# 21cmfast/21cmFAST

Measured on AMD Instinct MI355X. Metric: IonizeBox cells/sec (512^3 HII_DIM, 40 filter radii), higher is better.
Workload: dtype f32; 1 GPU; ComputeIonizedBox single-z, HII_DIM=512, 40 filter steps, G=2 (delta tophat + n_ion exp-MFP), first snapshot, device-resident inputs; hii_dim=512, n_radii=40, filtered_grids=2, parallelism=single GPU, fft=native

## Files before the change

21cmfast_amd/csrc/hip/c21hip.h:

```cpp
#ifndef C21HIP_H
#define C21HIP_H

#include <stddef.h>

#include "ws_slots.h"

#ifdef __cplusplus
extern "C" {
#endif

int c21hip_device_count(void);
int c21hip_current_device(void);
int c21hip_use_device(int device);
int c21hip_is_device_ptr(const void *p);
void *c21hip_ws(int slot, size_t bytes);
__attribute__((visibility("hidden"))) const void *c21_stage_in(int slot, const void *p, size_t bytes, void *stream, int *status);
void *c21hip_ws_peek(int slot, size_t *bytes);
int c21hip_ws_adopt(int slot, void *ptr, size_t bytes);
void *c21hip_raw_alloc(size_t bytes);
void *c21hip_vmm_chunk(size_t phys_bytes, size_t map_bytes, void **va_out);
void c21hip_vmm_chunk_free(void *chunk);
int c21hip_ws_adopt_vmm(int slot, void *chunk, size_t bytes);
void c21hip_raw_free(void *p);
size_t c21hip_free_bytes(void);
// ... 23 lines not shown
float c21hip_event_elapsed_ms(void *start, void *stop);
void c21hip_set_error(const char *fmt, ...);
const char *c21hip_get_error(void);

int c21hip_fft_r2c(float *padded, int nx, int ny, int nz, void *stream);
int c21hip_fft_c2r(float *padded, int nx, int ny, int nz, void *stream);
int c21hip_fft_r2c_batched(float *padded, int nx, int ny, int nz, int n_batch, void *stream);
void c21hip_fft_release(void);
int c21hip_fft_is_native(int nx, int ny, int nz);
int c21hip_pair_sweep_supported(int nx);

size_t c21hip_split_floats(int nx, int ny, int nz);
int c21hip_padded_to_split(const float *padded_c, float *split, int nx, int ny, int nz,
                           void *stream);
int c21hip_split_filter_c2r(const float *split_src, float *split_work, float *real_out,
                            long out_zstride, int nx, int ny, int nz, double box_len,
                            double box_len_z, int filter_type, float R, float R_param, int apply,
                            void *stream);

int c21hip_split_r2c(const float *real_in, long in_zstride, float *split_out, int nx, int ny,
                     int nz, double factor, double lo, double hi, float out_scale, void *stream);
int c21hip_split_filter_xy(const float *split_src, float *split_work, int nx, int ny, int nz,
                           double box_len, double box_len_z, int filter_type, float R,
                           float R_param, int apply, void *stream);
int c21hip_split_filter_xy2(const float *src_a, float *work_a, int filter_a, float R_param_a,
                            const float *src_b, float *work_b, int filter_b, float R_param_b,
                            int nx, int ny, int nz, double box_len, double box_len_z, float R,
                            int apply, int table_slot, int tables_ready, void *stream);
int c21hip_split_filter_shell(const float *src_a, float *work_a, int filter_a, const float *src_b,
                              float *work_b, int filter_b, int n_grids, int nx, int ny, int nz,
                              double box_len, double box_len_z, float R_inner, float R_outer,
                              float R_star, int apply, void *stream);
int c21hip_split_filter_xy2_pair(const float *src_a, float *work_a, float *work_a2, int filter_a,
                                 float R_param_a, const float *src_b, float *work_b,
                                 float *work_b2, int filter_b, float R_param_b, int nx, int ny,
                                 int nz, double box_len, double box_len_z, float R, float R2,
                                 int table_slot, int table_slot2, int phases, void *stream);
int c21hip_split_filter_x_pair1(const float *src, float *work, float *work2, int filter_type, int nx, int ny,
                                int nz, double box_len, double box_len_z, float R, float R2, int phases,
                                void *stream);
int c21hip_split_filter_xy2_pair_eval(const float *src_a, float *work_a, float *work_a2, int filter_a,
                                      const float *src_b, float *work_b, float *work_b2, int filter_b, int nx,
                                      int ny, int nz, double box_len, double box_len_z, float R, float R2,
                                      int phases, void *stream);
int c21hip_split_filter_xy_shared_pair(const float *src, float *work, float *work2,
                                       int filter_type, int nx, int ny, int nz, double box_len,
                                       double box_len_z, float R, float R2, int table_slot,
                                       int table_slot2, int phases, void *stream);
int c21hip_wev_prepare(int filter_a, float R_param_a, int filter_b, float R_param_b, int n_grids,
                       const float *R, int n_R, int nx, int ny, int nz, double box_len,
                       double box_len_z, int pair, int *enabled, void *stream);
void c21hip_wev_release(void);
int c21hip_wev_applicable(int filter_a, int filter_b, int n_grids, int nx, int ny, int nz);
int c21hip_split_filter_xy_single_pair(const float *src, float *work, float *work2, int filter_type,
                                       float R_param, int nx, int ny, int nz, double box_len,
                                       double box_len_z, float R, float R2, int phases, void *stream);
int c21hip_z_ionise_recomb_xe_supported(int nx, int ny, int nz);
int c21hip_split_z_ionise_recomb_xe(const float *delta_work, const float *stars_work, const float *xe_work,
                                    const float *nrec, double rec0, float *g12, unsigned char *first_cross,
                                    double *partials, int nx, int ny, int nz, int r_index,
                                    double rhocrit_omb, double ion_eff, int mass_dep_zeta, double f_limit,
                                    void *stream);
int c21hip_split_z_ionise_recomb_nrec(const float *delta_work, const float *stars_work, const float *nrec_work,
                                      float *g12, unsigned char *first_cross, double *partials, int nx,
                                      int ny, int nz, int r_index, double rhocrit_omb, double ion_eff,
                                      int mass_dep_zeta, double f_limit, void *stream);
int c21hip_z_ionise_recomb_xe_nrec_supported(int nx, int ny, int nz);
int c21hip_split_z_ionise_recomb_xe_nrec(const float *delta_work, const float *stars_work, const float *xe_work,
                                         const float *nrec_work, float *g12, unsigned char *first_cross,
                                         double *partials, int nx, int ny, int nz, int r_index,
                                         double rhocrit_omb, double ion_eff, int mass_dep_zeta, double f_limit,
                                         void *stream);
int c21hip_split_z_ionise_recomb(const float *delta_work, const float *stars_work, const float *nrec,
                                 double rec0, float *g12, unsigned char *first_cross,
                                 double *partials, int nx, int ny, int nz, int r_index,
                                 double rhocrit_omb, double ion_eff, int mass_dep_zeta,
                                 double f_limit, void *stream);
int c21hip_split_z_sfr_gamma12(const float *sfr_work, const unsigned char *first_cross, float *g12,
                               int nx, int ny, int nz, int r_index, double g12_scale, void *stream);
int c21hip_z_ionise_recomb_supported(int nx, int ny, int nz);
int c21hip_z_xe_mask_supported(int nx, int ny, int nz);
int c21hip_split_z_xe_mask(const float *xe_work, const float *nion_dense, const double *mean_dev,
                           unsigned char *first_cross, int nx, int ny, int nz, int r_index,
                           double mean_f_coll, int fix_mean, int mass_dep_zeta, double f_limit,
                           double ion_eff, void *stream);
int c21hip_apply_first_cross_recomb(const unsigned char *first_cross, const float *R_dev,
                                    const float *prev_z_reion, int first_snapshot, double redshift,
                                    float *xH, float *z_reion, float *mfp, size_t ntot, void *stream);
int c21hip_window_tables(int table_slot, int filter_a, float R_param_a, int filter_b,
                         float R_param_b, int nx, int ny, int nz, double box_len,
                         double box_len_z, float R, void *stream);
int c21hip_split_z_c2r_minmax(const float *split_work, float *real_out, long out_zstride, int nx,
                              int ny, int nz, double *partials, double *minmax_out, void *stream);
int c21hip_z_table_band_supported(int nx, int ny, int nz);
int c21hip_split_z_minmax_only(const float *split_work, int nx, int ny, int nz, double *partials,
                               double *minmax_out, void *stream);
int c21hip_split_z_fcoll_table_band(const float *split_work, float *f_pend, const double *band_dev,
                                    const double *thr_prev_dev, unsigned char *first_cross, int r_index,
                                    int r_prev, int nx, int ny, int nz, int mode, double tab_min, double tab_width,
                                    const float *table_dev, double *partials, void *stream);
int c21hip_split_z_fcoll_erfc(const float *split_work, float *nion_dense, int nx, int ny, int nz,
                              double growthf, double sigma_min, double sigma_max, double delta_c,
                              double *partials, double *sum_out, void *stream);
int c21hip_split_z_c2r_stats(const float *split_work, float *real_out, long out_zstride, int nx,
                             int ny, int nz, double min_value, double const_factor,
                             double *partials, double *stats_out, void *stream);
int c21hip_batched_stats(const double *partials, long stride, int nb, int count,
                         double *stats_out, void *stream);
int c21hip_floor_scale_stats(const float *in, long in_zstride, float *out, int nx, int ny, int nz,
                             double min_value, double const_factor, double *partials,
                             double *stats_out, void *stream);
int c21hip_split_z_c2r_div(const float *split_work, float *real_out, long out_zstride, int nx,
                           int ny, int nz, float divisor, void *stream);
int c21hip_split_z_c2r_out(const float *split_work, float *real_out, long out_zstride, int nx,
                           int ny, int nz, float scale, float divisor, int floor_density,
                           void *stream);
int c21hip_split_xblock_log2(int nx);
int c21hip_split_kop(const float *in_split, float *out_split, int nx, int ny, int nz,
                     double box_len, double box_len_z, int axis0, int axis1, void *stream);
int c21hip_split_sepop_xy(const float *split_src, float *split_work, int nx, int ny, int nz,
                          double box_len, double box_len_z, int axis0, int axis1, void *stream);
int c21hip_split_fold(const float *hi_split, float *lo_split, int nx, int ny, int nz, int f,
                      double box_len, double box_len_z, int axis0, int axis1, void *stream);
int c21hip_split_fold_multi(const float *hi_split, float *const lo_split[4], const int ops[4], int n_out, int nx,
                            int ny, int nz, int f, double box_len, double box_len_z, float tophat_R, void *stream);
int c21hip_lpt2_source(const float *const diag[3], const float *const off[3], float *out, size_t n,
                       float norm, void *stream);
int c21hip_copy_filter_split(const float *src_split, float *dst_split, int nx, int ny, int nz,
                             double box_len, double box_len_z, int filter_type, float R,
                             float R_param, int apply, void *stream);
int c21hip_split_z_c2r(const float *split_work, float *real_out, long out_zstride, int nx, int ny,
                       int nz, void *stream);
int c21hip_split_z_ionise_stars(const float *delta_work, const float *stars_work,
                                unsigned char *first_cross, double *partials, double *sum_out,
                                int nx, int ny, int nz, int r_index, double rhocrit_omb,
                                double ion_eff, int mass_dep_zeta, double f_limit, void *stream);
int c21hip_z_ionise_partials(int nx, int ny, int nz);
int c21hip_batched_means(const double *partials, long stride, int n_partials, int first, int step,
                         int count, double ntot, int mass_dep_zeta, double f_limit, double *sums,
                         double *means, void *stream);
int c21hip_split_z_ionise_stars_xe(const float *delta_work, const float *stars_work,
                                   const float *xe_work, unsigned char *first_cross,
                                   double *partials, double *sum_out, int nx, int ny, int nz,
                                   int r_index, double rhocrit_omb, double ion_eff,
                                   int mass_dep_zeta, double f_limit, void *stream);
int c21hip_z_ionise_xe_supported(int nx, int ny, int nz);
int c21hip_z_cross_bits_supported(int nx, int ny, int nz);
int c21hip_split_z_ionise_stars_bits(const float *delta_work, const float *stars_work,
                                     unsigned *cross_plane, double *partials, double *sum_out, int nx,
                                     int ny, int nz, int r_index, double rhocrit_omb, double ion_eff,
                                     int mass_dep_zeta, double f_limit, void *stream);
int c21hip_resolve_crossings(const unsigned *bits, int r_hi, int r_lo, unsigned char *first_cross,
                             size_t nlines, void *stream);
int c21hip_split_filter_xy_shared(const float *src, float *work, int filter_type, int nx, int ny,
                                  int nz, double box_len, double box_len_z, float R, int apply,
                                  int table_slot, void *stream);
int c21hip_bench_pass(int kind, int n, int filter_a, int filter_b, float R, float R_param_b,
                      double box_len, int reps, void *stream, float *ms_out);
int c21hip_reduce_sum(const double *partials, int n, double *out, void *stream);
int c21hip_reduce_op(const double *partials, int n, int op, double *stage, double *out,
                     void *stream);

int c21hip_pack_clip(const float *dense, float *padded, int nx, int ny, int nz, double factor,
                     double lo, double hi, void *stream);
int c21hip_unpack_scale(const float *padded, float *dense, int nx, int ny, int nz, float scale,
                        void *stream);
int c21hip_divide_inplace(float *buf, size_t n, float divisor, void *stream);
int c21hip_divide_inplace_f64(float *buf, size_t n, double divisor, void *stream);
int c21hip_fill(float *buf, size_t n, float value, void *stream);
int c21hip_add_scalar(float *buf, size_t n, float value, void *stream);
int c21hip_widen(const float *in, double *out, size_t n, void *stream);

int c21hip_copy_filter(const float *src_c, float *dst_c, int nx, int ny, int nz, double box_len,
                       double box_len_z, int filter_type, float R, float R_param, int apply,
                       void *stream);
int c21hip_copy_filter_star(const float *src_c, float *dst_c, int nx, int ny, int nz,
                            double box_len, double box_len_z, int filter_type, float R,
                            float R_param, float R_star, int apply, void *stream);

int c21hip_gsl_words_to_deviates(void *buf, size_t n_deviates, const unsigned char *row_kind_dev,
                                 size_t deviates_per_row, void *stream);

int c21hip_cic_scatter(const float *hires_density, const int dens_dim[3], const float *const vel[3],
                       const float *const vel2[3], const int vel_dim[3], double *out,
                       const int out_dim[3], double box_len, double box_len_z, double growth,
                       double init_growth, int lpt2, int *fixed_out, void *stream);
int c21hip_cic_fixed_status(int *bad, void *stream);
int c21hip_cic_last_path(void);
int c21hip_halobox_scatter(const float *src_density, const int dens_dim[3],
                           const float *const vel[3], const float *const vel2[3],
                           const int vel_dim[3], double *out_nion, double *out_sfr,
                           double *out_xray , const int out_dim[3],
                           double box_len, double box_len_z, double growth, double init_growth,
                           int lpt2, const float *tables_dev ,
                           double tab_min, double tab_width, double pref_nion, double pref_sfr,
                           double pref_xray, void *stream);
int c21hip_halobox_turnovers(size_t ntot, int n_chunks, int below_z_heat_max, double redshift,
                             double mturn_a_nofb, double m_turn, double vcb_const, double A_LW,
                             double BETA_LW, double A_VCB, double BETA_VCB, double sigma_vcb,
                             const float *prev_G12, const float *prev_z_reion, const float *J_21_LW,
                             const float *vcb, float *out_a, float *out_m, double *sums_dev,
                             void *stream);
int c21hip_halobox_scatter_mini(const float *src_density, const int dim[3],
                                const float *const vel[3], const float *const vel2[3],
                                const float *mturn_a, const float *mturn_m, double *out_nion,
                                double *out_sfr, double *out_sfr_mini, double *out_xray,
                                double box_len, double box_len_z, double growth, double init_growth,
                                int lpt2, const float *tab_sfrd, const float *tab_nion_a,
                                const float *tab_nion_m, const float *tab_sfrd_m,
                                const float *tab_xray, const double *ranges,
                                const double *prefactors, void *stream);
struct c21cm_halo_consts;
size_t c21hip_halo_deposit_scratch_ints(unsigned long long n_halos, const int out_dim[3]);
int c21hip_halo_props(const struct c21cm_halo_consts *consts, unsigned long long n_halos,
                      const float *masses, const float *coords, const float *star_rng,
                      const float *sfr_rng, const float *xray_rng, const int dim[3],
                      double cell_length, double redshift, int below_z_heat_max, int vcb_flucts,
                      const double lw[7], const float *vcb, const float *J21, const float *z_re,
                      const float *G12, float *out, void *stream);
int c21hip_halo_deposit(const struct c21cm_halo_consts *consts, unsigned long long n_halos,
                        const float *masses, const float *coords, const float *star_rng,
                        const float *sfr_rng, const float *xray_rng, const float *const vel[3],
                        const float *const vel2[3], const int vel_dim[3], const int out_dim[3],
                        double box_len, double box_len_z, double growth, double init_growth, int lpt2,
                        const float *mturn_a, const float *mturn_m, double *out_nion, double *out_sfr,
                        double *out_sfr_mini, double *out_xray, double *out_wsfr, int *scratch,
                        void *stream);
int c21hip_halo_catalog(const struct c21cm_halo_consts *consts, unsigned long long n_halos,
                        const float *masses, const float *coords, const float *star_rng,
                        const float *sfr_rng, const float *xray_rng, const float *const vel[3],
                        const float *const vel2[3], const int vel_dim[3], const int lo_dim[3],
                        double box_len, double box_len_z, double vdf, double vdf2, int lpt2,
                        double box_to_lores, const float *mturn_a, const float *mturn_m,
                        float *const out[9], void *stream);
int c21hip_narrow(const double *in, float *out, float *out_scaled, double scale, size_t n,
                  void *stream);
int c21hip_minmax_dense(const float *a, size_t n, double *partials, double *out2, void *stream);
int c21hip_widen_normalise(const double *in, float *padded, int nx, int ny, int nz, int normalise,
                           double mass_factor, int fixed, void *stream);
int c21hip_scale_pack(const float *dense, float *padded, int nx, int ny, int nz, double factor,
                      void *stream);
int c21hip_gather(const float *src_padded, const int src_dim[3], float *dst, const int lo_dim[3],
                  int dst_padded, float divisor, int clip, void *stream);
int c21hip_velocity_kspace(const float *saved_c, float *grid_c, int nx, int ny, int nz,
                           double box_len, double box_len_z, int axis, double dDdt_over_D,
                           void *stream);

int c21hip_vcb_op(const float *in_c, float *out_c, int nx, int ny, int nz, double box_len,
                  double box_len_z, int axis, const double *h_by_m_dev, void *stream);
int c21hip_vcb_accumulate(const float *src_padded, const int hi_dim[3], float *dst,
                          const int lo_dim[3], int first, int last, float volume, void *stream);
int c21hip_sample_modes(float *cbox, int nx, int ny, int nz, const double *pk_by_m_dev,
                        float volume, unsigned long long seed, const double *deviates_dev,
                        void *stream);
int c21hip_sample_modes_split(float *split, int nx, int ny, int nz, const double *pk_by_m_dev, float volume,
                              unsigned long long seed, const double *deviates_dev, void *stream);
int c21hip_kspace_op(const float *in_c, float *out_c, int nx, int ny, int nz, double box_len,
                     double box_len_z, int axis0, int axis1, void *stream);
int c21hip_pack_density(const float *dense, float *padded, int nx, int ny, int nz, float volume,
                        void *stream);
int c21hip_lpt2_accumulate(float *box, const float *phi_ij_padded, const float *diag_i,
                           const float *diag_j, int nx, int ny, int nz, void *stream);

typedef struct c21hip_ionize_args {
    int nx, ny, nz;
    int r_index;
    int lagrangian;
    int mass_dep_zeta;
    int use_ts_fluct;
    int minimize_memory;
    int first_snapshot;
    int fix_mean;
    double mean_f_coll;
    double f_limit;
    double ion_eff_factor;
    double rhocrit_omb;
    double photoncons_factor;
    double redshift;
    double TK_nofluct, adia_TK_term, T_re;
} c21hip_ionize_args;

#define C21HIP_PARTIALS 4096

int c21hip_clip_minmax(float *delta_fil, int nx, int ny, int nz, double *partials,
                       double *minmax_out, void *stream);
int c21hip_fcoll_eulerian(const float *delta_fil, float *nion_dense, int nx, int ny, int nz,
                          int mode, double growthf, double sigma_min, double sigma_max,
                          double delta_c, double tab_min, double tab_width,
                          const float *table_dev, double *partials, double *sum_out,
                          void *stream);
int c21hip_fcoll_eulerian_zs(const float *delta_fil, long zstride, float *nion_dense, int nx, int ny, int nz,
                             int mode, double growthf, double sigma_min, double sigma_max, double delta_c,
                             double tab_min, double tab_width, const float *table_dev, double *partials,
                             double *sum_out, void *stream);
int c21hip_ionise_stars(const c21hip_ionize_args *a, const float *delta_fil,
                        const float *stars_fil, const float *xe_fil, const float *density,
                        const float *prev_z_reion, const float *kinetic_temp_neutral, float *xH,
                        float *z_reion, float *kinetic_temperature, unsigned char *first_cross,
                        double *partials, double *sum_out, void *stream);
int c21hip_ionise_eulerian(const c21hip_ionize_args *a, const float *nion_dense,
                           const float *xe_fil, const float *density, const float *prev_z_reion,
                           const float *kinetic_temp_neutral, const double *mean_dev, float *xH,
                           float *z_reion, float *kinetic_temperature,
                           unsigned char *first_cross, void *stream);
int c21hip_finish_mean(const double *sum_dev, double ntot, int mass_dep_zeta, double f_limit,
                       double *mean_dev, void *stream);
// ... 247 lines not shown
```

21cmfast_amd/csrc/hip/fft_native.hip:

```cpp
#include <hip/hip_runtime.h>

#include <cmath>
#include <map>
#include <mutex>
#include <vector>

#include "c21hip.h"
#include "fcoll_device.h"
#include "ms_window.h"
#include "c21cm_abi.h"
#include "c21cm_grid.h"

#ifndef C21X_XPAIR_THREADS
#define C21X_XPAIR_THREADS 512
#endif
#ifndef C21X_FUSE512
#define C21X_FUSE512 1
#endif
#ifndef C21X_FUSE1024
#define C21X_FUSE1024 1
#endif
#ifndef C21X_F512_MERGE
#define C21X_F512_MERGE 1
#endif
// ... 301 lines not shown
        const float ksq = __fadd_rn(__fadd_rn(__fmul_rn(kx[i], kx[i]), __fmul_rn(ky[i], ky[i])),
                                    __fmul_rn(kz[i], kz[i]));
        const double k = sqrt((double)ksq);
        x0[i] = (double)(float)(k * (double)pa.R);
        x3[i] = k * pb.mfp.R;
    }
#pragma unroll
    for (int i = 0; i < NE; i++) fast_sincos(x0[i], &sn[i], &cs[i]);
#pragma unroll
    for (int i = 0; i < NE; i++) {
        wa[i] = w_tophat(x0[i], sn[i], cs[i]);
        const double d = x3[i] - x0[i], d3 = d * (1.0 / 3.0);
        const double s3 = sn[i] + d * (cs[i] - 0.5 * d * (sn[i] + d3 * cs[i]));
        const double c3 = cs[i] - d * (sn[i] + 0.5 * d * (cs[i] - d3 * sn[i]));
        wb[i] = w_expmfp(pb.mfp, x3[i], s3, c3);
    }
}

using wtab_t = float;
struct WTableArgs {
    FilterParams pa, pb;
    int dual;
    int nx, ny, nz;
    wtab_t *main_a, *nyq_a, *main_b, *nyq_b;
    MsConsts ms_a, ms_b;
};

template <int NE>
__device__ __forceinline__ void window_batch_ms(const FilterParams &p, const MsConsts &ms,
                                                const float (&kx)[NE], const float (&ky)[NE],
                                                const float (&kz)[NE], double (&w)[NE]) {
    if (p.type != 5) {
        window_batch<NE>(p, kx, ky, kz, w);
        return;
    }
#pragma unroll
    for (int i = 0; i < NE; i++) {
        const float ksq = __fadd_rn(__fadd_rn(__fmul_rn(kx[i], kx[i]), __fmul_rn(ky[i], ky[i])),
                                    __fmul_rn(kz[i], kz[i]));
        w[i] = ms_window(sqrt((double)ksq), ms);
    }
}

template <bool MS>
__global__ void __launch_bounds__(kBlock)
window_table_kernel(WTableArgs t) {
    const int nxh = t.nx / 2 + 1, nyh = t.ny / 2 + 1, H = t.nz / 2, H4 = H / 4;
    const long n4 = (long)nyh * nxh * H4;
    const long id = (long)blockIdx.x * kBlock + threadIdx.x;
    const bool sym = (t.nx == t.ny);
    if (id < n4) {
        const int l4 = (int)(id % H4);
        const long r = id / H4;
        const int i = (int)(r % nxh), j = (int)(r / nxh);
        if (sym && i > j) return;
        const long rT = (long)i * nxh + j;
        float kx[4], ky[4], kz[4];
#pragma unroll
        for (int e = 0; e < 4; e++) {
            kx[e] = k_of(i, t.nx, t.pa.dkx);
            ky[e] = k_of(j, t.ny, t.pa.dky);
            kz[e] = (float)((double)(4 * l4 + e) * t.pa.dkz);
        }
        double wa[4], wb[4];
        if (MS) {
            window_batch_ms<4>(t.pa, t.ms_a, kx, ky, kz, wa);
            if (t.dual) window_batch_ms<4>(t.pb, t.ms_b, kx, ky, kz, wb);
        } else if (t.dual)
            window_batch_dual<4>(t.pa, t.pb, kx, ky, kz, wa, wb);
        else
            window_batch<4>(t.pa, kx, ky, kz, wa);
        for (int rep = 0; rep < ((sym && i != j) ? 2 : 1); rep++) {
            const long rr = rep ? rT : r;
            *reinterpret_cast<float4 *>(t.main_a + rr * H + 4 * l4) =
                make_float4((float)wa[0], (float)wa[1], (float)wa[2], (float)wa[3]);
            if (t.dual)
                *reinterpret_cast<float4 *>(t.main_b + rr * H + 4 * l4) =
                    make_float4((float)wb[0], (float)wb[1], (float)wb[2], (float)wb[3]);
        }
    } else if (id - n4 < (long)nxh * nyh) {
        const long q = id - n4;
        const int i = (int)(q / nyh), j = (int)(q % nyh);
        if (sym && i > j) return;
        float kx[1] = {k_of(i, t.nx, t.pa.dkx)}, ky[1] = {k_of(j, t.ny, t.pa.dky)};
        float kz[1] = {(float)((double)(t.nz / 2) * t.pa.dkz)};
        double wa[1], wb[1];
        if (MS) {
            window_batch_ms<1>(t.pa, t.ms_a, kx, ky, kz, wa);
            if (t.dual) window_batch_ms<1>(t.pb, t.ms_b, kx, ky, kz, wb);
        } else if (t.dual)
            window_batch_dual<1>(t.pa, t.pb, kx, ky, kz, wa, wb);
        else
            window_batch<1>(t.pa, kx, ky, kz, wa);
        t.nyq_a[q] = (wtab_t)wa[0];
        if (t.dual) t.nyq_b[q] = (wtab_t)wb[0];
        if (sym && i != j) {
            t.nyq_a[(long)j * nyh + i] = (wtab_t)wa[0];
            if (t.dual) t.nyq_b[(long)j * nyh + i] = (wtab_t)wb[0];
        }
    }
}

struct WNodeArgs {
    float *out;
    int n_nodes, n_tabs;
    int first_type;
    const ExpMfpConsts *mfp;
};
__device__ __forceinline__ double wnode_value(int type, const ExpMfpConsts &c, double x) {
    x = fabs(x);
    double sn, cs;
    sincos(x, &sn, &cs);
    return type == 0 ? w_tophat(x, sn, cs) : w_expmfp(c, x, sn, cs);
}
__global__ void __launch_bounds__(kBlock)
window_nodes_kernel(WNodeArgs a) {
    const int id = blockIdx.x * kBlock + threadIdx.x;
    if (id >= a.n_nodes * a.n_tabs) return;
    const int tab = id / a.n_nodes, n = id - tab * a.n_nodes;
    const int type = (tab == 0) ? a.first_type : 3;
    ExpMfpConsts c{};
    if (type == 3) c = a.mfp[a.first_type == 3 ? tab : tab - 1];
    const double h = 0.25, s = h / 16., x = h * (double)n;
    const double c1[4] = {4. / 5., -1. / 5., 4. / 105., -1. / 280.};
    const double c2[4] = {8. / 5., -1. / 5., 8. / 315., -1. / 560.};
    const double f0 = wnode_value(type, c, x);
    double d1 = 0., d2 = -205. / 72. * f0;
#pragma unroll
    for (int k = 1; k <= 4; k++) {
        const double fp = wnode_value(type, c, x + k * s), fm = wnode_value(type, c, x - k * s);
        d1 += c1[k - 1] * (fp - fm);
        d2 += c2[k - 1] * (fp + fm);
    }
    float *o = a.out + 3 * (size_t)id;
    o[0] = (float)f0;
    o[1] = (float)(d1 / s * h);
    o[2] = (float)(d2 / (s * s) * h * h * 0.5);
}

struct LineGeo {
    const float2 *src[2];
    float2 *dst[2];
    float2 *dst2[2];
    long line_stride, line_bstride;
    long outer_stride, outer_bstride;
    int line_lb, outer_lb;
    long col_stride;
    int n_outer;
    int n_ctiles;
    int pair_outer;
    int filter_axis;
};

struct LinePassArgs {
    LineGeo g0, g1;
    int n_geo;
    int g1_strided;
    int n_grids;
    int n_y, n_z;
    float out_scale;
    const wtab_t *wt_main[2];
    const wtab_t *wt_nyq[2];
    int dual;
    const wtab_t *wt2_main[2];
    const wtab_t *wt2_nyq[2];
    FilterParams fp;
    int op_ex, op_ey, op_ez, op_imag;
    double op_sign, op_dkx, op_dky, op_dkz;
    const float *wev_src[3];
    int wev_n_tabs, wev_n_nodes;
    int wev_tab[2][2];
    int wev_type[2];
    float wev_R[2];
    float wev_mfp[2][4];
    double wev_dkx, wev_dky, wev_dkz;
    int item_order;
};

static inline int geo_items(const LineGeo &g) {
    return (g.pair_outer ? (g.n_outer / 2 + 1) : g.n_outer) * g.n_ctiles;
}

template <int N>
__device__ __forceinline__ int mirror_row(int row_a) {
    return row_a == 0 ? N / 2 : N - row_a;
}

template <int N, int FMODE = 0>
struct LineThreads {
    static constexpr int value =
        ((FMODE == 5 || FMODE == 7 || FMODE == 9) && N == 512) ? C21X_XPAIR_THREADS
                                                 : ((N >= 128 && N != 192) ? 512 : 256);
};

struct LineItemSecond {
    float2 *dst0b, *dst1b;
    const wtab_t *wt0b, *wt1b;
};
struct LineItemNone {};
template <bool PAIR>
struct LineItemT : std::conditional_t<PAIR, LineItemSecond, LineItemNone> {
    const float2 *src0, *src1;
    float2 *dst0, *dst1;
    long line_stride, line_bstride, outer_stride, outer_bstride, col_stride;
    int line_lb, outer_lb;
    int n_outer, filter_axis;
    int og, ct, npair;
    const wtab_t *wt0, *wt1;
};

template <int N, int SIGN, int FMODE>
__global__ void __launch_bounds__((LineThreads<N, FMODE>::value), (LineThreads<N, FMODE>::value / 256))
line_pass_kernel(LinePassArgs a, const float2 *__restrict__ tw_global) {
    static_assert(N >= 64, "tile loader needs N >= 64");
    constexpr int kBlock = LineThreads<N, FMODE>::value;
    constexpr int TZ = line_tile_cols(N);
    constexpr int CPAIR = TZ / 2;
    constexpr int RSTEP = kBlock / CPAIR;
    constexpr bool WEVAL = (FMODE >= 6 && FMODE <= 9);
    constexpr bool WDIRECT = (FMODE == 8 || FMODE == 9);
    constexpr bool WIN = (FMODE == 3 || (FMODE == 5 && !C21X_XPAIR_NOWIN) || WEVAL);
    constexpr bool PAIR = (FMODE == 5 || FMODE == 7 || FMODE == 9);
    constexpr int NR = PAIR ? 2 : 1;
    using LineItem = LineItemT<PAIR>;
    extern __shared__ float4 lds_raw[];
    float2 *tile = reinterpret_cast<float2 *>(lds_raw);
    float2 *tw = tile + NR * N * TZ;
    float2 *tw_half = tw + N;
    float *wnodes = reinterpret_cast<float *>(tw_half + (N >= 1024 ? N / 2 : 0));
    for (int t = threadIdx.x; t < N; t += kBlock) tw[t] = tw_global[t];
    if (N >= 1024)
        for (int t = threadIdx.x; t < N / 2; t += kBlock) tw_half[t] = tw_global[2 * t];
    if constexpr (WEVAL) {
        const int per = 3 * a.wev_n_nodes;
        for (int t = threadIdx.x; t < per; t += kBlock) {
            wnodes[t] = a.wev_src[0][t];
            if (a.wev_n_tabs > 1) wnodes[per + t] = a.wev_src[1][t];
            if (a.wev_n_tabs > 2) wnodes[2 * per + t] = a.wev_src[2][t];
        }
    }
#ifndef C21X_NO_TW_BARRIER
#define C21X_NO_TW_BARRIER 0
#endif
    if (!C21X_NO_TW_BARRIER || WEVAL) __syncthreads();

    constexpr int NP = (N / 2) / RSTEP;
    const int r0 = threadIdx.x / CPAIR, c4 = threadIdx.x % CPAIR;
    constexpr bool F512_ = C21X_FUSE512 && N == 512 && kBlock == 512 && (FMODE == 0 || WEVAL);
    float2 twd1[F512_ ? 8 : 1], twd2[F512_ ? 8 : 1];
    if constexpr (F512_) {
        __syncthreads();
        auto fill = [&](float2(&t)[8], int ps) {
            t[0] = make_float2(1.f, 0.f);
            t[1] = tw[ps];
            t[2] = tw[2 * ps];
            t[4] = tw[4 * ps];
            t[3] = cmul(t[1], t[2]);
            t[5] = cmul(t[1], t[4]);
            t[6] = cmul(t[2], t[4]);
            t[7] = cmul(t[3], t[4]);
            if (SIGN > 0)
#pragma unroll
                for (int j = 1; j < 8; j++) t[j].y = -t[j].y;
        };
        fill(twd1, r0);
        if (C21X_F512_HOIST2) fill(twd2, r0 & ~7);
    }
    const int n_work0 = (a.g0.pair_outer ? (a.g0.n_outer / 2 + 1) : a.g0.n_outer) * a.g0.n_ctiles;
    const int n_work1 =
        (a.n_geo > 1) ? (a.g1.pair_outer ? (a.g1.n_outer / 2 + 1) : a.g1.n_outer) * a.g1.n_ctiles : 0;
    const int n_work = n_work0 + (a.g1_strided ? 0 : n_work1);

    auto decode = [&](int w) {
        LineItem it;
        const bool s = w >= n_work0;
        int ww = s ? w - n_work0 : w;
        if (WIN && !s && ww < (n_work0 & ~15) && a.item_order == 0) {
            const int r = ww & 15;
            ww = (ww & ~15) + 2 * (r & 7) + (r >> 3);
        }
        it.src0 = s ? a.g1.src[0] : a.g0.src[0];
        it.src1 = s ? a.g1.src[1] : a.g0.src[1];
        it.dst0 = s ? a.g1.dst[0] : a.g0.dst[0];
        it.dst1 = s ? a.g1.dst[1] : a.g0.dst[1];
        it.line_stride = s ? a.g1.line_stride : a.g0.line_stride;
        it.line_bstride = s ? a.g1.line_bstride : a.g0.line_bstride;
        it.line_lb = s ? a.g1.line_lb : a.g0.line_lb;
        it.outer_stride = s ? a.g1.outer_stride : a.g0.outer_stride;
        it.outer_bstride = s ? a.g1.outer_bstride : a.g0.outer_bstride;
        it.outer_lb = s ? a.g1.outer_lb : a.g0.outer_lb;
        it.col_stride = s ? a.g1.col_stride : a.g0.col_stride;
        it.n_outer = s ? a.g1.n_outer : a.g0.n_outer;
        it.filter_axis = s ? a.g1.filter_axis : a.g0.filter_axis;
        it.wt0 = (it.filter_axis == 1) ? a.wt_nyq[0] : a.wt_main[0];
        it.wt1 = (it.filter_axis == 1) ? a.wt_nyq[1] : a.wt_main[1];
        if constexpr (PAIR) {
            it.dst0b = s ? a.g1.dst2[0] : a.g0.dst2[0];
            it.dst1b = s ? a.g1.dst2[1] : a.g0.dst2[1];
            it.wt0b = (it.filter_axis == 1) ? a.wt2_nyq[0] : a.wt2_main[0];
            it.wt1b = (it.filter_axis == 1) ? a.wt2_nyq[1] : a.wt2_main[1];
        }
        const int nct = s ? a.g1.n_ctiles : a.g0.n_ctiles;
        const int po = s ? a.g1.pair_outer : a.g0.pair_outer;
        it.og = ww / nct;
        it.ct = ww - it.og * nct;
        if (a.item_order == 3 || a.item_order == -1) {
            if (!s && (int)gridDim.x % nct == 0)
                it.ct = (it.ct + w / (int)gridDim.x) % nct;
        } else if (a.item_order != 0 && !s) {
            const int nog = n_work0 / nct;
            if (FMODE != 0) {
                it.ct = ww / nog;
                it.og = ww - it.ct * nog;
            } else {
                const int k = a.item_order < nct ? a.item_order : nct;
                const int head = k * nog;
                if (ww < head) {
                    const int c = ww / nog;
                    it.ct = nct - 1 - c;
                    it.og = ww - c * nog;
                } else {
                    const int v = ww - head, m = nct - k;
                    it.og = v / m;
                    it.ct = v - it.og * m;
                }
            }
        }
        it.npair = (po && it.og != 0 && 2 * it.og != it.n_outer) ? 2 : 1;
        return it;
    };
    auto member_grid = [](const LineItem &it, int m) { return it.npair == 2 ? (m >> 1) : m; };
    auto member_base = [](const LineItem &it, int m) {
        const int mi = it.npair == 2 ? (m & 1) : 0;
        const int outer = mi == 0 ? it.og : it.n_outer - it.og;
        return (long)(outer >> it.outer_lb) * it.outer_bstride +
               (long)(outer & ((1 << it.outer_lb) - 1)) * it.outer_stride +
               (long)it.ct * TZ * it.col_stride;
    };
    auto row_off = [](const LineItem &it, int r) {
        return (unsigned)(r >> it.line_lb) * (unsigned)it.line_bstride +
               (unsigned)(r & ((1 << it.line_lb) - 1)) * (unsigned)it.line_stride;
    };

    constexpr bool TWO_SETS = (N < 1024) && (!PAIR || C21X_XPAIR_TWO_SETS);
    float4 reg_a[2 * NP], reg_b[2 * NP];
    constexpr bool F512 = C21X_FUSE512 && N == 512 && kBlock == 512 && (FMODE == 0 || WEVAL);
    constexpr bool F1024 = C21X_FUSE1024 && N == 1024 && kBlock == 512 && (FMODE == 0 || FMODE == 3 || WEVAL);
    constexpr bool FUSED = F512 || F1024;
    constexpr int NW = FUSED ? 2 * NP : NP;
    constexpr bool WPRE = (N >= 512) && !FUSED;
    float2 wpre[NR][WPRE ? NP : 1], wcur[NR][NW], wpre_half[NR], wcur_half[NR];
    auto w_reload = [&](const LineItem &it, int m) {
        const int mi = it.npair == 2 ? (m & 1) : 0;
        return m == 0 || (a.dual && mi == 0);
    };
    struct KAbs {
        float kh, kl;
    };
    auto k_abs = [](float kx, float ky, float kz) -> KAbs {
        const float ksq = __fadd_rn(__fadd_rn(__fmul_rn(kx, kx), __fmul_rn(ky, ky)), __fmul_rn(kz, kz));
        KAbs k;
        k.kh = __builtin_amdgcn_sqrtf(ksq);
        const float r = __fmaf_rn(-k.kh, k.kh, ksq);
        k.kl = (k.kh > 0.f) ? __fmul_rn(r, __fmul_rn(0.5f, __builtin_amdgcn_rcpf(k.kh))) : 0.f;
        return k;
    };
    auto weval_direct = [&](float x0, float d, int type, int rr) -> float {
        const float n = rintf(x0 * 0.6366197723675814f);
        float r = __fmaf_rn(-n, 1.5707963705062866f, x0);
        r = __fmaf_rn(-n, -4.371138828673793e-08f, r);
        const float z = r * r;
        const float s = fmaf(fmaf(fmaf(-1.9515295891e-4f, z, 8.3321608736e-3f), z, -1.6666654611e-1f) * z, r, r);
        const float c = fmaf(fmaf(fmaf(2.443315711809948e-5f, z, -1.388731625493765e-3f), z,
                                  4.166664568298827e-2f) * z, z, fmaf(-0.5f, z, 1.0f));
        const int q = (int)n & 3;
        const float ss = (q & 1) ? c : s, cc = (q & 1) ? s : c;
        float sn = (q & 2) ? -ss : ss, cs = ((q + 1) & 2) ? -cc : cc;
        const float inv = __builtin_amdgcn_rcpf(x0);
        if (type == 0) return 3.f * (sn - x0 * cs) * (inv * inv) * inv;
        const float s0 = sn, c0 = cs;
        sn = fmaf(d, c0, s0);
        cs = fmaf(-d, s0, c0);
        const float ra = rr ? a.wev_mfp[1][0] : a.wev_mfp[0][0], r2 = rr ? a.wev_mfp[1][1] : a.wev_mfp[0][1],
                    r3 = rr ? a.wev_mfp[1][2] : a.wev_mfp[0][2], et = rr ? a.wev_mfp[1][3] : a.wev_mfp[0][3];
        const float xx = fmaf(2.f * x0, d, x0 * x0);
        float f = fmaf(xx, r2, fmaf(2.f, ra, 1.f)) * ra * cs;
        f = fmaf(fmaf(xx, r2 - r3, ra + 1.f) * sn, __builtin_amdgcn_rcpf(x0 + d), f);
        f = fmaf(f, et, -2.f * r2);
        const float dd = fmaf(xx, r2, 1.f);
        return f * (-3.f * ra * __builtin_amdgcn_rcpf(dd * dd));
    };
    auto weval_one = [&](const KAbs &k, float R, int type, const float *tab, int rr) -> float {
        const float ph = __fmul_rn(k.kh, R);
        const float e = __fmaf_rn(k.kl, R, __fmaf_rn(k.kh, R, -ph));
        const float x0 = __fadd_rn(ph, e);
        if (type == 1) return ((double)x0 * 0.413566994 > 1) ? 0.f : 1.f;
        const float u = x0 * 4.0f;
        if constexpr (WDIRECT)
            if (u >= (float)(a.wev_n_nodes - 2))
                return weval_direct(x0, __fadd_rn(__fsub_rn(ph, x0), e), type, rr);
        const int n = WDIRECT ? (int)u : min((int)u, a.wev_n_nodes - 2);
        const float t = u - (float)n;
        const float *nd = tab + 3 * n;
        const float f0 = nd[0], g0 = nd[1], q0 = nd[2], f1 = nd[3], g1 = nd[4], q1 = nd[5];
        const float A = ((f1 - f0) - g0) - q0, B = (g1 - g0) - 2.f * q0, C = q1 - q0;
        const float a3 = 10.f * A - 4.f * B + C, a4 = -15.f * A + 7.f * B - 2.f * C,
                    a5 = 6.f * A - 3.f * B + C;
        float p = fmaf(fmaf(fmaf(fmaf(fmaf(a5, t, a4), t, a3), t, q0), t, g0), t, f0);
        if (type == 3) {
            const float d = __fadd_rn(__fsub_rn(ph, x0), e);
            const float dp = fmaf(fmaf(fmaf(fmaf(5.f * a5, t, 4.f * a4), t, 3.f * a3), t, 2.f * q0), t, g0);
            p = fmaf(d * 4.0f, dp, p);
        }
        return p;
    };
    float wev_kx[WEVAL ? NW : 1];
    float wev_kx_half = 0.f;
    if constexpr (WEVAL) {
#pragma unroll
        for (int u = 0; u < NW; u++) {
            const int row = r0 + RSTEP * u;
            wev_kx[u] = (float)((double)(FUSED ? min(row, N - row) : row) * a.wev_dkx);
        }
        wev_kx_half = (float)((double)(N / 2) * a.wev_dkx);
    }
    auto eval_windows = [&](const LineItem &it, int m) {
        const int wsel = (a.dual && member_grid(it, m)) ? 1 : 0;
        const int type = wsel ? a.wev_type[1] : a.wev_type[0];
        const int per = 3 * a.wev_n_nodes;
        float kyc[2], kzc[2];
        if (it.filter_axis == 0) {
            kyc[0] = kyc[1] = (float)((double)it.og * a.wev_dky);
            const int l0 = it.ct * TZ + 2 * c4;
            kzc[0] = (float)((double)l0 * a.wev_dkz);
            kzc[1] = (float)((double)(l0 + 1) * a.wev_dkz);
        } else {
            const int c0 = it.ct * TZ + 2 * c4;
            kyc[0] = (float)((double)min(c0, a.n_y - c0) * a.wev_dky);
            kyc[1] = (float)((double)min(c0 + 1, a.n_y - c0 - 1) * a.wev_dky);
            kzc[0] = kzc[1] = (float)((double)(a.n_z / 2) * a.wev_dkz);
        }
        const float *tab0 = wnodes + max(wsel ? a.wev_tab[0][1] : a.wev_tab[0][0], 0) * per;
        const float *tab1 = wnodes + max(wsel ? a.wev_tab[1][1] : a.wev_tab[1][0], 0) * per;
#pragma unroll
        for (int u = 0; u < NW; u++) {
            if (FUSED && u >= NP && !(u == NP && r0 == 0)) continue;
            const KAbs k0 = k_abs(wev_kx[WEVAL ? u : 0], kyc[0], kzc[0]);
            const KAbs k1 = k_abs(wev_kx[WEVAL ? u : 0], kyc[1], kzc[1]);
#pragma unroll
            for (int rr = 0; rr < NR; rr++) {
                const float R = rr ? a.wev_R[1] : a.wev_R[0];
                const float *tab = rr ? tab1 : tab0;
                (WPRE ? wpre[rr][WPRE ? u : 0] : wcur[rr][u]) =
                    make_float2(weval_one(k0, R, type, tab, rr), weval_one(k1, R, type, tab, rr));
            }
        }
        if (!FUSED && r0 == 0) {
            const KAbs k0 = k_abs(wev_kx_half, kyc[0], kzc[0]), k1 = k_abs(wev_kx_half, kyc[1], kzc[1]);
#pragma unroll
            for (int rr = 0; rr < NR; rr++) {
                const float R = rr ? a.wev_R[1] : a.wev_R[0];
                const float *tab = rr ? tab1 : tab0;
                (WPRE ? wpre_half[rr] : wcur_half[rr]) =
                    make_float2(weval_one(k0, R, type, tab, rr), weval_one(k1, R, type, tab, rr));
            }
        }
        if constexpr (FUSED) {
            float2 *const exch = tile;
            __syncthreads();
#pragma unroll
            for (int rr = 0; rr < NR; rr++)
#pragma unroll
                for (int u = 0; u < NP; u++) exch[((int)threadIdx.x * NP + u) * NR + rr] = wcur[rr][u];
            __syncthreads();
            const int src = (((RSTEP - r0) & (RSTEP - 1)) * CPAIR + c4) * NP;
#pragma unroll
            for (int rr = 0; rr < NR; rr++)
#pragma unroll
                for (int u = NP; u < NW; u++)
                    if (!(u == NP && r0 == 0))
                        wcur[rr][u] = exch[(src + (NW - (r0 == 0 ? 0 : 1) - u)) * NR + rr];
            __syncthreads();
        }
    };
    auto issue_wloads = [&](const LineItem &it, int m) {
        if constexpr (WEVAL) {
            eval_windows(it, m);
            return;
        }
        const bool second = a.dual && member_grid(it, m);
#pragma unroll
        for (int rr = 0; rr < NR; rr++) {
            const wtab_t *t = second ? it.wt1 : it.wt0;
            if constexpr (PAIR)
                if (rr) t = second ? it.wt1b : it.wt0b;
            if (it.filter_axis == 0) {
                const unsigned wc = (unsigned)(a.n_z / 2);
                const wtab_t *b = t + (long)it.og * (N / 2 + 1) * wc + (it.ct * TZ + 2 * c4);
                if constexpr (FUSED) {
#pragma unroll
                    for (int u = 0; u < NW; u++) {
                        const int row = r0 + RSTEP * u;
                        wcur[rr][u] = *reinterpret_cast<const float2 *>(b + (unsigned)min(row, N - row) * wc);
                    }
                    continue;
                }
#pragma unroll
                for (int u = 0; u < NP; u++)
                    (WPRE ? wpre[rr][WPRE ? u : 0] : wcur[rr][u]) =
                        *reinterpret_cast<const float2 *>(b + (unsigned)(r0 + RSTEP * u) * wc);
                (WPRE ? wpre_half[rr] : wcur_half[rr]) =
                    *reinterpret_cast<const float2 *>(b + (unsigned)(N / 2) * wc);
            } else {
                const int c0 = it.ct * TZ + 2 * c4;
                const unsigned nyh = (unsigned)(a.n_y / 2 + 1);
                const unsigned j0 = (unsigned)min(c0, a.n_y - c0),
                               j1 = (unsigned)min(c0 + 1, a.n_y - c0 - 1);
                if constexpr (FUSED) {
#pragma unroll
                    for (int u = 0; u < NW; u++) {
                        const int row = r0 + RSTEP * u;
                        const wtab_t *r = t + (unsigned)min(row, N - row) * nyh;
                        wcur[rr][u] = make_float2(r[j0], r[j1]);
                    }
                    continue;
                }
#pragma unroll
                for (int u = 0; u < NP; u++) {
                    const wtab_t *r = t + (unsigned)(r0 + RSTEP * u) * nyh;
                    (WPRE ? wpre[rr][WPRE ? u : 0] : wcur[rr][u]) = make_float2(r[j0], r[j1]);
                }
                {
                    const wtab_t *r = t + (unsigned)(N / 2) * nyh;
                    (WPRE ? wpre_half[rr] : wcur_half[rr]) = make_float2(r[j0], r[j1]);
                }
            }
        }
    };
    auto issue_loads = [&](float4(&reg)[2 * NP], const LineItem &it, int m) {
        const float2 *lo = (member_grid(it, m) ? it.src1 : it.src0) + member_base(it, m);
        const float2 *hi = lo + (long)((N / 2) >> it.line_lb) * it.line_bstride;
#pragma unroll
        for (int u = 0; u < 2 * NP; u++) {
            if constexpr (FUSED) {
                const int row = r0 + RSTEP * u;
                const unsigned roff = row_off(it, row < N / 2 ? row : row - N / 2);
                reg[u] = *reinterpret_cast<const float4 *>((row < N / 2 ? lo : hi) + (roff + 2u * c4));
                continue;
            }
            const int row_a = r0 + RSTEP * (u >> 1);
            const unsigned roff = (u & 1) ? (row_a == 0 ? 0u : row_off(it, N / 2 - row_a))
                                          : row_off(it, row_a);
            const float2 *p = (u & 1) ? hi : lo;
            reg[u] = *reinterpret_cast<const float4 *>(p + (roff + 2u * c4));
        }
    };

    struct TileRef {
        LineItem it;
        int m, work, valid;
    };
    auto next_tile = [&](const TileRef &t) {
        TileRef n = t;
        if (!t.valid) return n;
        if (t.m + 1 < t.it.npair * a.n_grids) {
            n.m = t.m + 1;
        } else {
            n.work = t.work + (int)gridDim.x;
            n.valid = n.work < n_work;
            if (n.valid) {
                n.m = 0;
                n.it = decode(n.work);
            }
        }
        return n;
    };

    bool first = true;
    auto process = [&](float4(&reg)[2 * NP], const TileRef &cur, const TileRef &nxt,
                       const TileRef &refill) {
        const LineItem &it = cur.it;
        const int m = cur.m;
        const long st_half = (long)((N / 2) >> it.line_lb) * it.line_bstride;
        if (!first) __syncthreads();
        first = false;
        if (WIN && WPRE && w_reload(it, m)) {
#pragma unroll
            for (int rr = 0; rr < NR; rr++) {
#pragma unroll
                for (int u = 0; u < NP; u++) wcur[rr][u] = wpre[rr][WPRE ? u : 0];
                wcur_half[rr] = wpre_half[rr];
            }
        }
        double op_c0 = 1., op_c1 = 1.;
        if (FMODE == 4) {
            const int c0 = it.ct * TZ + 2 * c4;
            int kyi0, kyi1, kzi0, kzi1;
            if (it.filter_axis == 0) {
                const int mi = it.npair == 2 ? (m & 1) : 0;
                const int outer = mi == 0 ? it.og : it.n_outer - it.og;
                kyi0 = kyi1 = (outer <= a.n_y / 2) ? outer : outer - a.n_y;
                kzi0 = c0;
                kzi1 = c0 + 1;
            } else {
                kyi0 = (c0 <= a.n_y / 2) ? c0 : c0 - a.n_y;
                kyi1 = (c0 + 1 <= a.n_y / 2) ? c0 + 1 : c0 + 1 - a.n_y;
                kzi0 = kzi1 = a.n_z / 2;
            }
            const double ky0 = (double)kyi0 * a.op_dky, ky1 = (double)kyi1 * a.op_dky;
            const double kz0 = (double)kzi0 * a.op_dkz, kz1 = (double)kzi1 * a.op_dkz;
            const double fy0 = a.op_ey == 0 ? 1. : (a.op_ey == 1 ? ky0 : ky0 * ky0);
            const double fy1 = a.op_ey == 0 ? 1. : (a.op_ey == 1 ? ky1 : ky1 * ky1);
            const double fz0 = a.op_ez == 0 ? 1. : (a.op_ez == 1 ? kz0 : kz0 * kz0);
            const double fz1 = a.op_ez == 0 ? 1. : (a.op_ez == 1 ? kz1 : kz1 * kz1);
// ... 85 lines not shown
                }
                continue;
            }
            if (!(PAIR && C21X_XPAIR_SKIP_FFT)) {
                Dft<8, SIGN>::run(c0);
                Dft<8, SIGN>::run(c1);
            }
#pragma unroll
            for (int j = 0; j < 8; j++) {
                float2 o0 = c0[j], o1 = c1[j];
                if (j > 0 && !(PAIR && C21X_XPAIR_SKIP_FFT)) {
                    o0 = cmul(o0, twd1[F512_ ? j : 0]);
                    o1 = cmul(o1, twd1[F512_ ? j : 0]);
                }
                *reinterpret_cast<float4 *>(tile_r + (8 * r0 + j) * TZ + 2 * c4) =
                    make_float4(o0.x, o0.y, o1.x, o1.y);
            }
            continue;
        }
#pragma unroll
        for (int u = 0; u < 2 * NP; u++) {
            const int row_a = r0 + RSTEP * (u >> 1);
            const int row = (u & 1) ? mirror_row<N>(row_a) : row_a;
            const bool half = (u & 1) && row_a == 0;
            float4 v = reg[u];
            if (FMODE == 4) {
                const int kxi = (row <= N / 2) ? row : row - N;
                const double kx = (double)kxi * a.op_dkx;
                const double fr = a.op_ex == 0 ? 1. : (a.op_ex == 1 ? kx : kx * kx);
                const double f0 = fr * op_c0, f1 = fr * op_c1;
                if (a.op_imag) {
                    const float4 t = v;
                    v.x = (float)(-(double)t.y * f0);
                    v.y = (float)((double)t.x * f0);
                    v.z = (float)(-(double)t.w * f1);
                    v.w = (float)((double)t.z * f1);
                } else {
                    v.x = (float)((double)v.x * f0);
                    v.y = (float)((double)v.y * f0);
                    v.z = (float)((double)v.z * f1);
                    v.w = (float)((double)v.w * f1);
                }
            }
            if (WIN) {
                const float2 wv = half ? wcur_half[rr] : wcur[rr][u >> 1];
                v.x = __fmul_rn(v.x, wv.x);
                v.y = __fmul_rn(v.y, wv.x);
                v.z = __fmul_rn(v.z, wv.y);
                v.w = __fmul_rn(v.w, wv.y);
            }
            *reinterpret_cast<float4 *>(tile_r + row * TZ + 2 * c4) = v;
        }
      }
        __syncthreads();
        if (WIN && !WEVAL && w_reload(nxt.it, nxt.m)) issue_wloads(nxt.it, nxt.m);
        issue_loads(reg, refill.it, refill.m);
        if (WEVAL && !FUSED && w_reload(nxt.it, nxt.m)) issue_wloads(nxt.it, nxt.m);

        if constexpr (F1024) {
            const int obase = (r0 & 7) + 64 * (r0 >> 3);
            float2 s0[2][8], s1[2][8];
#pragma unroll
            for (int h = 0; h < 2; h++)
#pragma unroll
                for (int k = 0; k < 8; k++) {
                    const float4 t = *reinterpret_cast<const float4 *>(tile + (h * (N / 2) + r0 + RSTEP * k) * TZ + 2 * c4);
                    s0[h][k] = make_float2(t.x, t.y);
                    s1[h][k] = make_float2(t.z, t.w);
                }
            __syncthreads();
            float2 w2[8];
            {
                const int ps = r0 & ~7;
                w2[1] = tw_half[ps];
                w2[2] = tw_half[2 * ps];
                w2[4] = tw_half[4 * ps];
                w2[3] = cmul(w2[1], w2[2]);
                w2[5] = cmul(w2[1], w2[4]);
                w2[6] = cmul(w2[2], w2[4]);
                w2[7] = cmul(w2[3], w2[4]);
                if (SIGN > 0)
#pragma unroll
                    for (int j = 1; j < 8; j++) w2[j].y = -w2[j].y;
            }
#pragma unroll
            for (int h = 0; h < 2; h++) {
                Dft<8, SIGN>::run(s0[h]);
                Dft<8, SIGN>::run(s1[h]);
#pragma unroll
                for (int j = 0; j < 8; j++) {
                    float2 o0 = s0[h][j], o1 = s1[h][j];
                    if (j > 0) {
                        o0 = cmul(o0, w2[j]);
                        o1 = cmul(o1, w2[j]);
                    }
                    *reinterpret_cast<float4 *>(tile + (h * (N / 2) + obase + 8 * j) * TZ + 2 * c4) =
                        make_float4(o0.x, o0.y, o1.x, o1.y);
                }
            }
            __syncthreads();
        }
        if constexpr (F512 && !(PAIR && C21X_XPAIR_SKIP_FFT)) {
            constexpr int GRP = C21X_F512_MERGE ? NR : 1;
            const int obase = (r0 & 7) + 64 * (r0 >> 3);
#pragma unroll
            for (int g = 0; g < NR; g += GRP) {
                float2 s0[GRP][8], s1[GRP][8];
#pragma unroll
                for (int rr = 0; rr < GRP; rr++)
#pragma unroll
                    for (int k = 0; k < 8; k++) {
                        const float4 t = *reinterpret_cast<const float4 *>(tile + (g + rr) * N * TZ +
                                                                           (r0 + RSTEP * k) * TZ + 2 * c4);
                        s0[rr][k] = make_float2(t.x, t.y);
                        s1[rr][k] = make_float2(t.z, t.w);
                    }
                __syncthreads();
                float2 w2[8];
                if (!C21X_F512_HOIST2) {
                    const int ps = r0 & ~7;
                    w2[1] = tw[ps];
                    w2[2] = tw[2 * ps];
                    w2[4] = tw[4 * ps];
                    w2[3] = cmul(w2[1], w2[2]);
                    w2[5] = cmul(w2[1], w2[4]);
                    w2[6] = cmul(w2[2], w2[4]);
                    w2[7] = cmul(w2[3], w2[4]);
                    if (SIGN > 0)
#pragma unroll
                        for (int j = 1; j < 8; j++) w2[j].y = -w2[j].y;
                }
#pragma unroll
                for (int rr = 0; rr < GRP; rr++) {
                    Dft<8, SIGN>::run(s0[rr]);
                    Dft<8, SIGN>::run(s1[rr]);
#pragma unroll
                    for (int j = 0; j < 8; j++) {
                        float2 o0 = s0[rr][j], o1 = s1[rr][j];
                        if (j > 0) {
                            const float2 w = C21X_F512_HOIST2 ? twd2[F512_ ? j : 0] : w2[j];
                            o0 = cmul(o0, w);
                            o1 = cmul(o1, w);
                        }
                        *reinterpret_cast<float4 *>(tile + (g + rr) * N * TZ + (obase + 8 * j) * TZ + 2 * c4) =
                            make_float4(o0.x, o0.y, o1.x, o1.y);
                    }
                }
                __syncthreads();
            }
        }
#pragma unroll
      for (int rr = 0; rr < NR; rr++) {
        float2 *const tile_r = tile + rr * N * TZ;
        float2 *st_lo = member_grid(it, m) ? it.dst1 : it.dst0;
        if constexpr (PAIR)
            if (rr) st_lo = member_grid(it, m) ? it.dst1b : it.dst0b;
        st_lo += member_base(it, m);
        if constexpr (F1024) {
#pragma unroll
            for (int h = 0; h < 2; h++) {
                float2 c0[8], c1[8];
#pragma unroll
                for (int k = 0; k < 8; k++) {
                    const float4 t = *reinterpret_cast<const float4 *>(tile_r + (h * (N / 2) + r0 + RSTEP * k) * TZ + 2 * c4);
                    c0[k] = make_float2(t.x, t.y);
                    c1[k] = make_float2(t.z, t.w);
                }
                Dft<8, SIGN>::run(c0);
                Dft<8, SIGN>::run(c1);
#pragma unroll
                for (int j = 0; j < 8; j++) {
                    float4 v = make_float4(c0[j].x, c0[j].y, c1[j].x, c1[j].y);
                    if (a.out_scale != 1.0f) {
                        v.x *= a.out_scale;
                        v.y *= a.out_scale;
                        v.z *= a.out_scale;
                        v.w *= a.out_scale;
                    }
                    const int row = 2 * (r0 + RSTEP * j) + h;
                    const unsigned roff = row_off(it, row < N / 2 ? row : row - N / 2);
                    float2 *p = st_lo + (row < N / 2 ? 0 : st_half);
                    *reinterpret_cast<float4 *>(p + (roff + 2u * c4)) = v;
                }
            }
            continue;
        }
        if constexpr (F512) {
            if constexpr (PAIR && C21X_XPAIR_SKIP_FFT == 3) continue;
            float2 c0[8], c1[8];
#pragma unroll
            for (int k = 0; k < 8; k++) {
                const float4 t = *reinterpret_cast<const float4 *>(tile_r + (r0 + RSTEP * k) * TZ + 2 * c4);
                c0[k] = make_float2(t.x, t.y);
                c1[k] = make_float2(t.z, t.w);
            }
            if (!(PAIR && C21X_XPAIR_SKIP_FFT)) {
                Dft<8, SIGN>::run(c0);
                Dft<8, SIGN>::run(c1);
            }
#pragma unroll
            for (int j = 0; j < 8; j++) {
                float4 v = make_float4(c0[j].x, c0[j].y, c1[j].x, c1[j].y);
                if (a.out_scale != 1.0f) {
                    v.x *= a.out_scale;
                    v.y *= a.out_scale;
                    v.z *= a.out_scale;
                    v.w *= a.out_scale;
                }
                const int row = r0 + RSTEP * j;
                const unsigned roff = row_off(it, row < N / 2 ? row : row - N / 2);
                float2 *p = st_lo + (row < N / 2 ? 0 : st_half);
                *reinterpret_cast<float4 *>(p + (roff + 2u * c4)) = v;
            }
            continue;
        }
        if (!(PAIR && C21X_XPAIR_SKIP_FFT)) line_fft<N, TZ, SIGN, kBlock>(tile_r, tw, tw_half);
        if (PAIR && C21X_XPAIR_SKIP_FFT == 2 && rr == 1) continue;
#pragma unroll
        for (int u = 0; u < 2 * NP; u++) {
            const int row_a = r0 + RSTEP * (u >> 1);
            const int row = (u & 1) ? mirror_row<N>(row_a) : row_a;
            float4 v = *reinterpret_cast<const float4 *>(tile_r + fft_out_row<N>(row) * TZ + 2 * c4);
            if (a.out_scale != 1.0f) {
                v.x *= a.out_scale;
                v.y *= a.out_scale;
                v.z *= a.out_scale;
                v.w *= a.out_scale;
            }
            const unsigned roff = (u & 1) ? (row_a == 0 ? 0u : row_off(it, N / 2 - row_a))
                                          : row_off(it, row_a);
            float2 *p = st_lo + ((u & 1) ? st_half : 0);
            *reinterpret_cast<float4 *>(p + (roff + 2u * c4)) = v;
        }
      }
        if (WEVAL && FUSED && w_reload(nxt.it, nxt.m)) issue_wloads(nxt.it, nxt.m);
    };

    if ((int)blockIdx.x < n_work) {
        TileRef ta;
        ta.work = blockIdx.x;
        ta.valid = 1;
        ta.m = 0;
        ta.it = decode(ta.work);
        if (WIN && !WEVAL) issue_wloads(ta.it, 0);
        issue_loads(reg_a, ta.it, 0);
        if (WEVAL) issue_wloads(ta.it, 0);
        TileRef tb = next_tile(ta);
        if (!TWO_SETS) {
            process(reg_a, ta, tb, tb);
            while (tb.valid) {
                ta = tb;
                tb = next_tile(ta);
                process(reg_a, ta, tb, tb);
            }
            goto main_done;
        }
        issue_loads(reg_b, tb.it, tb.m);
        TileRef tc = next_tile(tb);
        process(reg_a, ta, tb, tc);
        while (tb.valid) {
            const TileRef td = next_tile(tc);
            process(reg_b, tb, tc, td);
            if (!tc.valid) break;
            const TileRef te = next_tile(td);
            process(reg_a, tc, td, te);
            tb = td;
            tc = te;
        }
    }
main_done:
    if (!(a.n_geo > 1 && a.g1_strided)) return;
    for (int w = (int)(gridDim.x - 1 - blockIdx.x); w < n_work1; w += (int)gridDim.x) {
        const unsigned ls = (unsigned)a.g1.line_bstride, cs = (unsigned)a.g1.col_stride;
        const int nct = a.g1.n_ctiles;
        const int og = w / nct, ct = w - og * nct;
        const long base = (long)og * a.g1.outer_bstride + (long)ct * TZ * a.g1.col_stride;
        for (int g = 0; g < a.n_grids; g++) {
            const float2 *src = (g ? a.g1.src[1] : a.g1.src[0]) + base;
            float2 *dst = (g ? a.g1.dst[1] : a.g1.dst[0]) + base;
            __syncthreads();
#pragma unroll
            for (int u = 0; u < 2 * NP; u++) {
                const int row_a = r0 + RSTEP * (u >> 1);
                const int row = (u & 1) ? mirror_row<N>(row_a) : row_a;
                const float2 e0 = src[(unsigned)row * ls + (unsigned)(2 * c4) * cs];
                const float2 e1 = src[(unsigned)row * ls + (unsigned)(2 * c4 + 1) * cs];
                *reinterpret_cast<float4 *>(tile + row * TZ + 2 * c4) =
                    make_float4(e0.x, e0.y, e1.x, e1.y);
            }
            __syncthreads();
            line_fft<N, TZ, SIGN, kBlock>(tile, tw, tw_half);
#pragma unroll
            for (int u = 0; u < 2 * NP; u++) {
                const int row_a = r0 + RSTEP * (u >> 1);
                const int row = (u & 1) ? mirror_row<N>(row_a) : row_a;
                float4 v = *reinterpret_cast<const float4 *>(tile + fft_out_row<N>(row) * TZ + 2 * c4);
                if (a.out_scale != 1.0f) {
                    v.x *= a.out_scale;
                    v.y *= a.out_scale;
                    v.z *= a.out_scale;
                    v.w *= a.out_scale;
                }
                dst[(unsigned)row * ls + (unsigned)(2 * c4) * cs] = make_float2(v.x, v.y);
                dst[(unsigned)row * ls + (unsigned)(2 * c4 + 1) * cs] = make_float2(v.z, v.w);
            }
        }
// ... 304 lines not shown
    const float dmin = (float)(-1. + 1e-7);
    double acc = 0.;
#pragma unroll
    for (int u = 0; u < NOUT; u++) {
        const int f = threadIdx.x + kBlock * u;
        const int li = f / H, j = f % H;
        const float2 st = tile[j * ZROW + li];
        const float s0 = fmaxf(st.x, 0.f), s1 = fmaxf(st.y, 0.f);
        acc += (double)s0;
        acc += (double)s1;
        const double D0 = a.rhocrit_omb * (1. + (double)fmaxf(dens[u].x, dmin));
        const double D1 = a.rhocrit_omb * (1. + (double)fmaxf(dens[u].y, dmin));
        const bool i0 = floor_ionises || ((double)s0 * a.ion_eff > D0);
        const bool i1 = floor_ionises || ((double)s1 * a.ion_eff > D1);
        uchar2 m = old[u];
        const bool n0 = i0 && m.x == 0, n1 = i1 && m.y == 0;
        if (n0) m.x = (unsigned char)a.r_index;
        if (n1) m.y = (unsigned char)a.r_index;
        if (n0 || n1 || a.store_all)
            reinterpret_cast<uchar2 *>(a.first_cross + logical_line(l0 + li, a.ny, a.lb) * NZ)[j] = m;
    }
    __shared__ double red[kBlock / 64];
#pragma unroll
    for (int off = 32; off > 0; off >>= 1) acc += __shfl_down(acc, off, 64);
    if ((threadIdx.x & 63) == 0) red[threadIdx.x >> 6] = acc;
    __syncthreads();
    if (threadIdx.x == 0) {
        double sum = 0.;
#pragma unroll
        for (int w = 0; w < kBlock / 64; w++) sum += red[w];
        a.partials[blockIdx.x] = sum;
    }
}

__global__ void __launch_bounds__(kBlock)
padded_to_split_kernel(const float2 *__restrict__ padded, float2 *__restrict__ main,
                       float2 *__restrict__ nyq, long nlines, int H, int ny, int lb) {
    const long total = nlines * (long)(H + 1);
    for (long i = (long)blockIdx.x * kBlock + threadIdx.x; i < total;
         i += (long)gridDim.x * kBlock) {
        const long line = i / (H + 1);
        const int k = (int)(i - line * (H + 1));
        const float2 v = padded[i];
        if (k < H) {
            const long x = line / ny, y = line - x * ny;
            const long m = lb ? (((x >> lb) * ny + y) << lb) + (x & ((1 << lb) - 1)) : line;
            main[m * H + k] = v;
        } else {
            nyq[line] = v;
        }
    }
}

struct Twiddles {
    float2 *dev = nullptr;
};
std::map<int, Twiddles> g_tw;
std::mutex g_tw_mutex;

const float2 *twiddles(int n) {
    std::lock_guard<std::mutex> lock(g_tw_mutex);
    auto it = g_tw.find(n);
    if (it != g_tw.end()) return it->second.dev;
    std::vector<float2> host(n);
    for (int t = 0; t < n; t++) {
        const double ang = -2.0 * M_PI * (double)t / (double)n;
        host[t] = make_float2((float)cos(ang), (float)sin(ang));
    }
    Twiddles tw;
    if (hipMalloc(&tw.dev, sizeof(float2) * n) != hipSuccess) return nullptr;
    if (hipMemcpy(tw.dev, host.data(), sizeof(float2) * n, hipMemcpyHostToDevice) != hipSuccess)
        return nullptr;
    g_tw[n] = tw;
    return tw.dev;
}

bool pow2(int n) { return n > 0 && (n & (n - 1)) == 0; }

void geo_ptrs(LineGeo &g, int grid, const float2 *src, float2 *dst) {
    g.src[grid] = src;
    g.dst[grid] = dst;
}
void geo_axes(LineGeo &g, int line_lb, long line_stride, long line_bstride, int outer_lb,
              long outer_stride, long outer_bstride) {
    g.line_lb = line_lb;
    g.line_stride = line_stride;
    g.line_bstride = line_bstride;
    g.outer_lb = outer_lb;
    g.outer_stride = outer_stride;
    g.outer_bstride = outer_bstride;
}
LineGeo geo_x_main(int ny, int H, int tz, int lb) {
    LineGeo g{};
    const long xb = 1L << lb;
    geo_axes(g, lb, H, (long)ny * xb * H, 0, 0, xb * H);
    g.col_stride = 1;
    g.n_outer = ny;
    g.n_ctiles = H / tz;
    g.pair_outer = 1;
    g.filter_axis = 0;
    return g;
}
LineGeo geo_x_nyq(int ny, int tz) {
    LineGeo g{};
    geo_axes(g, 0, 0, ny, 0, 0, 0);
    g.col_stride = 1;
    g.n_outer = 1;
    g.n_ctiles = ny / tz;
    g.pair_outer = 0;
    g.filter_axis = 1;
    return g;
}
LineGeo geo_y_main(int nx, int ny, int H, int tz, int lb) {
    LineGeo g{};
    const long xb = 1L << lb;
    geo_axes(g, 0, 0, xb * H, lb, H, (long)ny * xb * H);
    g.col_stride = 1;
    g.n_outer = nx;
    g.n_ctiles = H / tz;
    return g;
}
LineGeo geo_y_nyq(int nx, int ny, int tz) {
    LineGeo g{};
    geo_axes(g, 0, 0, 1, 0, 0, 0);
    g.col_stride = ny;
    g.n_outer = 1;
    g.n_ctiles = nx / tz;
    return g;
}

struct KTimeRec {
    int kind;
    hipEvent_t e0, e1;
};
std::vector<KTimeRec> g_ktime;
int g_ktime_on = 0;
struct KTimeScope {
    KTimeRec r{-1, nullptr, nullptr};
    hipStream_t stream;
    KTimeScope(int kind, hipStream_t s) : stream(s) {
        if (!g_ktime_on) return;
        if (hipEventCreate(&r.e0) != hipSuccess || hipEventCreate(&r.e1) != hipSuccess) return;
        r.kind = kind;
        (void)hipEventRecord(r.e0, stream);
    }
    ~KTimeScope() {
        if (r.kind < 0) return;
        (void)hipEventRecord(r.e1, stream);
        g_ktime.push_back(r);
    }
};
constexpr int ktime_kind(int sign, int fmode) {
    return sign < 0 ? 9 : (fmode == 0 ? 1 : fmode == 3 ? 0 : fmode == 5 ? 6 : (fmode == 6 || fmode == 8) ? 7
                                                              : (fmode == 7 || fmode == 9) ? 8 : 10);
}

#ifndef C21X_XORDER_DEFAULT
#define C21X_XORDER_DEFAULT 3
#endif
template <int N, int SIGN, int FMODE>
int launch_line_pass_mode(const LinePassArgs &a, hipStream_t stream) {
    const float2 *tw = twiddles(N);
    if (!tw) {
        c21hip_set_error("native FFT: twiddle table allocation failed");
        return C21CM_MEMORY_ALLOC_ERROR;
    }
    const size_t lds = sizeof(float2) * ((size_t)((FMODE == 5 || FMODE == 7 || FMODE == 9) ? 2 : 1) * N *
                                             line_tile_cols(N) + N + (N >= 1024 ? N / 2 : 0)) +
                       ((FMODE >= 6 && FMODE <= 9) ? sizeof(float) * 3 * (size_t)a.wev_n_nodes * a.wev_n_tabs : 0);
    if (lds > 160 * 1024) {
        c21hip_set_error("native FFT: %zu bytes of LDS for a %d-point line pass (mode %d)", lds, N, FMODE);
        return C21CM_VALUE_ERROR;
    }
    const int n_work = geo_items(a.g0) + (a.n_geo > 1 ? geo_items(a.g1) : 0);
    int per_cu = (int)((160 * 1024) / lds) > 0 ? (int)((160 * 1024) / lds) : 1;
    const int by_waves = (LineThreads<N, FMODE>::value >= 512 && N > 256) ? 1 : 2;
    if (per_cu > by_waves) per_cu = by_waves;
    int nblocks = 256 * per_cu;
    if (nblocks > n_work) nblocks = n_work;
    static size_t attr_lds = 0;
    if (lds > attr_lds) {
        (void)hipFuncSetAttribute((const void *)line_pass_kernel<N, SIGN, FMODE>,
                                  hipFuncAttributeMaxDynamicSharedMemorySize, (int)lds);
        attr_lds = lds;
    }
    LinePassArgs ao = a;
    {
        static int xo = -99, yo = -99;
        if (xo == -99) {
            const char *ex = getenv("C21CM_XORDER"), *ey = getenv("C21CM_YORDER");
            xo = ex ? atoi(ex) : C21X_XORDER_DEFAULT;
            yo = ey ? atoi(ey) : -1;
        }
        ao.item_order = (FMODE == 0) ? yo : xo;
    }
    KTimeScope kt(ktime_kind(SIGN, FMODE), stream);
    hipLaunchKernelGGL((line_pass_kernel<N, SIGN, FMODE>), dim3((unsigned)nblocks),
                       dim3(LineThreads<N, FMODE>::value), lds, stream, ao, tw);
    LAUNCH_CHECK();
    return 0;
}

template <int N, int SIGN>
int launch_line_pass(const LinePassArgs &a, int fmode, hipStream_t stream) {
    if (SIGN > 0 && fmode == 3) return launch_line_pass_mode<N, +1, 3>(a, stream);
    if (SIGN > 0 && fmode == 4) return launch_line_pass_mode<N, +1, 4>(a, stream);
    if constexpr (N <= 512)
        if (SIGN > 0 && fmode == 5) return launch_line_pass_mode<N, +1, 5>(a, stream);
    if constexpr (N >= 128 && (N & (N - 1)) == 0) {
        if (SIGN > 0 && fmode == 6) return launch_line_pass_mode<N, +1, 6>(a, stream);
        if (SIGN > 0 && fmode == 8) return launch_line_pass_mode<N, +1, 8>(a, stream);
        if constexpr (N <= 512) {
            if (SIGN > 0 && fmode == 7) return launch_line_pass_mode<N, +1, 7>(a, stream);
            if (SIGN > 0 && fmode == 9) return launch_line_pass_mode<N, +1, 9>(a, stream);
        }
    }
    if (fmode >= 6 && fmode <= 9) {
        c21hip_set_error("native FFT: evaluated windows are not built for %d-point lines", N);
        return C21CM_VALUE_ERROR;
    }
    return launch_line_pass_mode<N, SIGN, 0>(a, stream);
}

template <int SIGN>
int dispatch_line_pass(int n, const LinePassArgs &a, int fmode, hipStream_t stream) {
    switch (n) {
        case 64: return launch_line_pass<64, SIGN>(a, fmode, stream);
        case 128: return launch_line_pass<128, SIGN>(a, fmode, stream);
        case 192: return launch_line_pass<192, SIGN>(a, fmode, stream);
        case 256: return launch_line_pass<256, SIGN>(a, fmode, stream);
        case 384: return launch_line_pass<384, SIGN>(a, fmode, stream);
        case 512: return launch_line_pass<512, SIGN>(a, fmode, stream);
        case 768: return launch_line_pass<768, SIGN>(a, fmode, stream);
        case 1024: return launch_line_pass<1024, SIGN>(a, fmode, stream);
        case 1536: return launch_line_pass<1536, SIGN>(a, fmode, stream);
        default:
            c21hip_set_error("native FFT: unsupported line length %d", n);
            return C21CM_VALUE_ERROR;
    }
}

template <int NZ, int EPI = 0>
int launch_z_c2r(const ZPassArgs &a, long nlines, hipStream_t stream) {
    constexpr int H = NZ / 2;
    const float2 *twH = twiddles(H);
    const float2 *twN = twiddles(NZ);
    if (!twH || !twN) return C21CM_MEMORY_ALLOC_ERROR;
    const size_t lds = sizeof(float2) * ((size_t)H * (LZ_PLAIN + 1) + H + H / 2 + 1);
    static bool attr_done = false;
    if (!attr_done) {
        (void)hipFuncSetAttribute((const void *)z_c2r_kernel<NZ, EPI>,
                                  hipFuncAttributeMaxDynamicSharedMemorySize, (int)lds);
        attr_done = true;
    }
    hipLaunchKernelGGL((z_c2r_kernel<NZ, EPI>), dim3((unsigned)(nlines / LZ_PLAIN)), dim3(kBlock),
                       lds, stream, a, twH, twN);
    LAUNCH_CHECK();
    return 0;
}

constexpr int ZW_LINES = 16;
constexpr int zw_lines(int P) { return kBlock / P; }

template <int A, bool TS, int P = 16, bool RC = false, bool CB = false>
__global__ void
#if C21X_ZW_OCC
__launch_bounds__(kBlock, (A == 16 && !TS) ? C21X_ZW_OCC : 1)
#else
__launch_bounds__((A == 16 && P == 16) ? C21X_ZW_BLOCK : kBlock, (TS && RC && A == 16 && P == 16) ? C21X_ZW_TSRC_OCC : 1)
#endif
zw_ionise_kernel(ZFusedArgs a, const float2 *__restrict__ twH_global,
                 const float2 *__restrict__ twN_global) {
    constexpr int ZBLK = (A == 16 && P == 16) ? C21X_ZW_BLOCK : kBlock;
    constexpr int H = P * A, NZ = 2 * H, ZWL = ZBLK / P;
    constexpr int LINE_LDS = A * (P + 1) + 4;
    static_assert(LINE_LDS % 2 == 0, "16-byte aligned line regions (mask rows)");
    __shared__ __attribute__((aligned(16))) float2 lines[ZWL * LINE_LDS];
    __shared__ float2 twH[H], twN[H];
    __shared__ double red[ZBLK / 64];
    for (int t = threadIdx.x; t < H; t += ZBLK) {
        twH[t] = twH_global[t];
        twN[t] = twN_global[t];
    }
    const int lane = threadIdx.x & 63, wave = threadIdx.x >> 6;
    const int g = lane / P, b = lane % P;
    const int lw = wave * (64 / P) + g;
    const unsigned blk = a.reverse ? gridDim.x - 1 - blockIdx.x : blockIdx.x;
    const long line = (long)blk * ZWL + lw;
    float2 *L = lines + lw * LINE_LDS;
    const float2 *dm = a.d_main + line * H, *sm = a.s_main + line * H;
    constexpr bool EARLY = (A == 16) && !C21X_ZW_LATE;
    static_assert(!CB || (A == 16 && P == 16 && !TS && !RC), "crossing bits: the two-grid kernel on 512-point lines");
    float2 xd[A], xs[A];
#pragma unroll
    for (int q = 0; q < A; q++) xd[q] = dm[P * q + b];
    if (EARLY) {
#pragma unroll
        for (int q = 0; q < A; q++) xs[q] = sm[P * q + b];
    }
    const long lline = logical_line(line, a.ny, a.lb);
    const float dh = a.d_nyq[lline].x, sh = a.s_nyq[lline].x;
    unsigned char *mrow = nullptr;
    if constexpr (!CB) mrow = a.first_cross + lline * NZ;
    constexpr bool MASK16 = !CB && EARLY && (C21X_ZW_MASK16 || (TS && RC && C21X_ZW_TSRC_LEAN));
    constexpr int MV = MASK16 ? A / 8 : 1;
    uint4 mreg[MV];
    uchar2 old[(EARLY && !MASK16) ? A : 1];
    if constexpr (MASK16) {
#pragma unroll
        for (int v = 0; v < MV; v++) mreg[v] = reinterpret_cast<const uint4 *>(mrow)[b * MV + v];
    } else if (EARLY && !CB) {
#pragma unroll
        for (int q = 0; q < A; q++)
            old[q] = reinterpret_cast<const uchar2 *>(mrow)[(b + P * (q / P)) + A * (q % P)];
    }
    constexpr bool STASH = TS && RC && A == 16 && P == 16 && C21X_ZW_TSRC_LEAN;
    constexpr int NRH = (RC && A == 16 && !STASH) ? A / 2 : 1;
    float2 nr_lo[NRH], nr_hi[NRH];
    __shared__ __attribute__((aligned(16))) float nstash[STASH ? ZWL * NZ : 4];
    uint4 nreg[STASH ? NZ / (4 * P) : 1];
    if constexpr (STASH) {
#pragma unroll
        for (int v = 0; v < NZ / (4 * P); v++) nreg[v] = make_uint4(0u, 0u, 0u, 0u);
        if (a.nrec) {
#pragma unroll
            for (int v = 0; v < NZ / (4 * P); v++)
                nreg[v] = reinterpret_cast<const uint4 *>(a.nrec + lline * NZ)[v * P + b];
        }
    } else if constexpr (RC && A == 16) {
        if (a.nrec) {
#pragma unroll
            for (int q = 0; q < NRH; q++)
                nr_lo[q] = reinterpret_cast<const float2 *>(a.nrec + lline * NZ)[(b + P * (q / P)) + A * (q % P)];
        }
    }
    __syncthreads();
    if constexpr (STASH) {
        if (a.n_main) {
            float2 xn[A];
            const float2 *nm = a.n_main + line * H;
#pragma unroll
            for (int q = 0; q < A; q++) xn[q] = nm[P * q + b];
            wave_c2r<A, P>(xn, a.n_nyq[lline].x, L, twH, twN, b);
#pragma unroll
            for (int q = 0; q < A; q++) {
                const int j = (b + P * (q / P)) + A * (q % P);
                reinterpret_cast<float2 *>(nstash + lw * NZ)[j] =
                    make_float2(fmaxf(xn[q].x, 0.f), fmaxf(xn[q].y, 0.f));
            }
            wave_fence();
        }
    }
    wave_c2r<A, P>(xd, dh, L, twH, twN, b);
    if constexpr (STASH) {
        if (a.nrec) {
#pragma unroll
            for (int v = 0; v < NZ / (4 * P); v++)
                reinterpret_cast<uint4 *>(nstash + lw * NZ)[v * P + b] = nreg[v];
        }
    }
    if (!EARLY) {
#pragma unroll
        for (int q = 0; q < A; q++) xs[q] = sm[P * q + b];
    }
    wave_fence();
    wave_c2r<A, P>(xs, sh, L, twH, twN, b);
    static_assert(!(TS && RC) || A == 16, "x_e + recombinations: 16 points per lane only (registers)");
    float2 xx[TS ? A : 1];
    if constexpr (TS) {
        const float2 *xm = a.x_main + line * H;
// ... 1204 lines not shown
        const dim3 tgrid((unsigned)((n_threads + kBlock - 1) / kBlock));
        if (ms)
            hipLaunchKernelGGL(window_table_kernel<true>, tgrid, dim3(kBlock), 0, stream, t);
        else
            hipLaunchKernelGGL(window_table_kernel<false>, tgrid, dim3(kBlock), 0, stream, t);
        LAUNCH_CHECK();
    }
    w.main[0] = t.main_a;
    w.nyq[0] = t.nyq_a;
    w.main[1] = t.main_b;
    w.nyq[1] = t.nyq_b;
    w.dual = t.dual;
    return 0;
}

struct WevSet {
    bool active = false;
    int filter[2] = {-1, -1};
    float R_param[2] = {0.f, 0.f};
    int nx = 0, ny = 0, nz = 0;
    double box_len = 0, box_len_z = 0;
    std::vector<float> R;
    float *nodes = nullptr;
    int n_nodes = 0, n_tabs = 0;
    bool covers = true;
    int first_type = 0;
    int table(int w, int r) const {
        const int t = filter[w];
        if (t == 1) return -1;
        if (t == 0) return 0;
        int base = (first_type == 0) ? 1 : 0;
        if (w == 1 && filter[0] == 3) base += (int)R.size();
        return base + r;
    }
    int find(float radius) const {
        for (size_t i = 0; i < R.size(); i++)
            if (R[i] == radius) return (int)i;
        return -1;
    }
};
WevSet g_wev;

static bool wev_type_ok(int t) { return t == 0 || t == 1 || t == 3; }
static size_t wev_lds(int n, bool pair, int n_tabs, int n_nodes) {
    return sizeof(float2) * ((size_t)(pair ? 2 : 1) * n * TZ + n + (n >= 1024 ? n / 2 : 0)) +
           sizeof(float) * 3 * (size_t)n_nodes * n_tabs;
}
static bool wev_use(LinePassArgs &a, int n_grids, const int filter_type[2], const float R_param[2],
                    float R, float R2, bool pair, int nx, int ny, int nz, double box_len,
                    double box_len_z) {
    const WevSet &w = g_wev;
    if (!w.active || w.nx != nx || w.ny != ny || w.nz != nz || w.box_len != box_len ||
        w.box_len_z != box_len_z)
        return false;
    int win0 = 0;
    auto matches = [&](int g, int win) {
        return filter_type[g] == w.filter[win] && (filter_type[g] != 3 || R_param[g] == w.R_param[win]);
    };
    if (n_grids == 2) {
        if (!matches(0, 0) || !matches(1, 1)) return false;
    } else if (!matches(0, 0)) {
        if (!matches(0, 1)) return false;
        win0 = 1;
    }
    const int ra = w.find(R), rb = pair ? w.find(R2) : ra;
    if (ra < 0 || rb < 0) return false;
    int ids[4], n_ids = 0;
    auto slot = [&](int id) {
        if (id < 0) return -1;
        for (int i = 0; i < n_ids; i++)
            if (ids[i] == id) return i;
        ids[n_ids] = id;
        return n_ids++;
    };
    const int rr[2] = {ra, rb};
    for (int m = 0; m < 2; m++)
        for (int win = 0; win < 2; win++)
            a.wev_tab[m][win] =
                (win < n_grids && (m == 0 || pair)) ? slot(w.table(win == 0 ? win0 : win, rr[m])) : -1;
    if (n_ids > 3) return false;
    if (wev_lds(nx, pair, n_ids, w.n_nodes) > 160 * 1024) return false;
    for (int i = 0; i < 3; i++)
        a.wev_src[i] = w.nodes + 3 * (size_t)w.n_nodes * (i < n_ids ? ids[i] : ids[0 < n_ids ? 0 : 0]);
    a.wev_n_tabs = n_ids > 0 ? n_ids : 1;
    if (n_ids == 0) a.wev_src[0] = a.wev_src[1] = a.wev_src[2] = w.nodes;
    a.wev_n_nodes = w.n_nodes;
    a.wev_type[0] = filter_type[0];
    a.wev_type[1] = n_grids == 2 ? filter_type[1] : filter_type[0];
    a.wev_R[0] = R;
    a.wev_R[1] = pair ? R2 : R;
    for (int m = 0; m < 2; m++) {
        const int win = (filter_type[0] == 3) ? 0 : ((n_grids == 2 && filter_type[1] == 3) ? 1 : -1);
        if (win < 0) break;
        const float Rm = m ? a.wev_R[1] : a.wev_R[0];
        const double ratio = (double)R_param[win] / (double)Rm;
        a.wev_mfp[m][0] = (float)ratio;
        a.wev_mfp[m][1] = (float)(ratio * ratio);
        a.wev_mfp[m][2] = (float)(ratio * ratio * ratio);
        a.wev_mfp[m][3] = (float)exp((double)(-Rm / R_param[win]));
    }
    a.wev_dkx = 2.0 * M_PI / box_len;
    a.wev_dky = 2.0 * M_PI / box_len;
    a.wev_dkz = 2.0 * M_PI / box_len_z;
    a.dual = (n_grids == 2 && (filter_type[0] != filter_type[1] ||
                               (filter_type[0] >= 3 && R_param[0] != R_param[1])))
                 ? 1 : 0;
    return true;
}

static int check_filter_request(int n_grids, int nx, int ny, int nz, const int filter_type[2],
                                int apply) {
    if (!c21hip_native_fft_supported(nx, ny, nz)) {
        c21hip_set_error("native FFT does not support %dx%dx%d", nx, ny, nz);
        return C21CM_VALUE_ERROR;
    }
    for (int g = 0; g < n_grids; g++)
        if (apply && (filter_type[g] < 0 || filter_type[g] > 5)) {
            c21hip_set_error("filter type %d is not implemented on the device", filter_type[g]);
            return C21CM_VALUE_ERROR;
        }
    return 0;
}

static int filter_xy(const float *const split_src[2], float *const split_work[2], int n_grids,
                     int nx, int ny, int nz, double box_len, double box_len_z,
                     const int filter_type[2], float R, const float R_param[2], int apply,
                     void *stream_, int phases = 7, int table_slot = 0, float R_star = 0.f) {
    int st = check_filter_request(n_grids, nx, ny, nz, filter_type, apply);
    if (st) return st;
    hipStream_t stream = (hipStream_t)stream_;
    const int H = nz / 2;
    const long nlines = (long)nx * ny;
    LinePassArgs a{};
    fill_filter(a.fp, apply ? filter_type[0] : -1, R, R_param[0], box_len, box_len_z);
    a.n_y = ny;
    a.n_z = nz;
    a.out_scale = 1.0f;
    int fmode = apply ? 3 : 0;
    if (fmode == 3 && filter_type[0] != 5 && wev_use(a, n_grids, filter_type, R_param, R, R, false, nx,
                                                      ny, nz, box_len, box_len_z))
        fmode = g_wev.covers ? 6 : 8;
    if (fmode == 3) {
        WinTables w;
        if ((st = win_tables(table_slot, n_grids, filter_type, R, R_param, R_star, nx, ny, nz,
                             box_len, box_len_z, (phases & 1) != 0, stream, w)))
            return st;
        for (int i = 0; i < 2; i++) {
            a.wt_main[i] = w.main[i];
            a.wt_nyq[i] = w.nyq[i];
        }
        a.dual = w.dual;
    }
    if (!(phases & 6)) return 0;
    a.n_geo = 2;
    a.n_grids = n_grids;
    a.g0 = geo_x_main(ny, H, line_tile_cols(nx), split_xb_log2(nx));
    a.g1 = geo_x_nyq(ny, line_tile_cols(nx));
    for (int g = 0; g < n_grids; g++) {
        const float2 *src = reinterpret_cast<const float2 *>(split_src[g]);
        float2 *work = reinterpret_cast<float2 *>(split_work[g]);
        geo_ptrs(a.g0, g, src, work);
        geo_ptrs(a.g1, g, src + nlines * H, work + nlines * H);
    }
    if ((phases & 2) && (st = dispatch_line_pass<+1>(nx, a, fmode, stream))) return st;
    if (!(phases & 4)) return 0;
    a.fp.type = -1;
    a.g0 = geo_y_main(nx, ny, H, line_tile_cols(ny), split_xb_log2(nx));
    a.g1 = geo_y_nyq(nx, ny, line_tile_cols(ny));
    a.g1_strided = 1;
    for (int g = 0; g < n_grids; g++) {
        float2 *work = reinterpret_cast<float2 *>(split_work[g]);
        geo_ptrs(a.g0, g, work, work);
        geo_ptrs(a.g1, g, work + nlines * H, work + nlines * H);
    }
    return dispatch_line_pass<+1>(ny, a, 0, stream);
}

extern "C" int c21hip_split_filter_xy(const float *split_src, float *split_work, int nx, int ny,
                                      int nz, double box_len, double box_len_z, int filter_type,
                                      float R, float R_param, int apply, void *stream_) {
    const float *src[2] = {split_src, nullptr};
    float *work[2] = {split_work, nullptr};
    const int ft[2] = {filter_type, 0};
    const float rp[2] = {R_param, 0.f};
    return filter_xy(src, work, 1, nx, ny, nz, box_len, box_len_z, ft, R, rp, apply, stream_);
}

extern "C" int c21hip_split_filter_xy2(const float *src_a, float *work_a, int filter_a,
                                       float R_param_a, const float *src_b, float *work_b,
                                       int filter_b, float R_param_b, int nx, int ny, int nz,
                                       double box_len, double box_len_z, float R, int apply,
                                       int table_slot, int tables_ready, void *stream_) {
    const float *src[2] = {src_a, src_b};
    float *work[2] = {work_a, work_b};
    const int ft[2] = {filter_a, filter_b};
    const float rp[2] = {R_param_a, R_param_b};
    return filter_xy(src, work, 2, nx, ny, nz, box_len, box_len_z, ft, R, rp, apply, stream_,
                     tables_ready ? 6 : 7, table_slot);
}

static int filter_xy_pair(const float *src_a, float *work_a, float *work_a2, int filter_a,
                          float R_param_a, const float *src_b, float *work_b, float *work_b2,
                          int filter_b, float R_param_b, int nx, int ny, int nz, double box_len,
                          double box_len_z, float R, float R2, int table_slot, int table_slot2,
                          int phases, void *stream_, int n_grids = 2, bool must_eval = false) {
    const int tables_ready = !(phases & 1);
    const int ft[2] = {filter_a, filter_b};
    const float rp[2] = {R_param_a, R_param_b};
    int st = check_filter_request(n_grids, nx, ny, nz, ft, 1);
    if (st) return st;
    if (nx >= 1024 || table_slot == table_slot2 || (n_grids != 2 && !tables_ready)) {
        c21hip_set_error("two-radius sweep: nx = %d / table slots %d, %d not supported", nx,
                         table_slot, table_slot2);
        return C21CM_VALUE_ERROR;
    }
    hipStream_t stream = (hipStream_t)stream_;
    const int H = nz / 2;
    const long nlines = (long)nx * ny;
    LinePassArgs a{};
    a.fp.type = -1;
    a.n_y = ny;
    a.n_z = nz;
    a.out_scale = 1.0f;
    const bool evaluated = (must_eval && !(phases & 2))
                               ? true
                               : wev_use(a, n_grids, ft, rp, R, R2, true, nx, ny, nz, box_len, box_len_z);
    if (must_eval && !evaluated) {
        c21hip_set_error("two-radius sweep of one grid: the evaluated windows do not cover radii %g, %g", (double)R,
                         (double)R2);
        return C21CM_VALUE_ERROR;
    }
    if (!evaluated) {
        WinTables w, w2;
        if ((st = win_tables(table_slot, n_grids, ft, R, rp, 0.f, nx, ny, nz, box_len, box_len_z,
                             !tables_ready, stream, w)))
            return st;
        if ((st = win_tables(table_slot2, n_grids, ft, R2, rp, 0.f, nx, ny, nz, box_len, box_len_z,
                             !tables_ready, stream, w2)))
            return st;
        for (int i = 0; i < 2; i++) {
            a.wt_main[i] = w.main[i];
            a.wt_nyq[i] = w.nyq[i];
            a.wt2_main[i] = w2.main[i];
            a.wt2_nyq[i] = w2.nyq[i];
        }
        a.dual = w.dual;
    }
    a.n_geo = 2;
    a.n_grids = n_grids;
    a.g0 = geo_x_main(ny, H, line_tile_cols(nx), split_xb_log2(nx));
    a.g1 = geo_x_nyq(ny, line_tile_cols(nx));
    const float2 *src[2] = {reinterpret_cast<const float2 *>(src_a),
                            reinterpret_cast<const float2 *>(src_b)};
    float2 *work[2] = {reinterpret_cast<float2 *>(work_a), reinterpret_cast<float2 *>(work_b)};
    float2 *work2[2] = {reinterpret_cast<float2 *>(work_a2), reinterpret_cast<float2 *>(work_b2)};
    for (int g = 0; g < n_grids && (phases & 2); g++) {
        geo_ptrs(a.g0, g, src[g], work[g]);
        geo_ptrs(a.g1, g, src[g] + nlines * H, work[g] + nlines * H);
        a.g0.dst2[g] = work2[g];
        a.g1.dst2[g] = work2[g] + nlines * H;
    }
    if ((phases & 2) &&
        (st = dispatch_line_pass<+1>(nx, a, evaluated ? (g_wev.covers ? 7 : 9) : 5, stream)))
        return st;
    if (!(phases & 12)) return 0;
    for (int r = 0; r < 2; r++) {
        if (!(phases & (4 << r))) continue;
        float2 *const *wk = r ? work2 : work;
        a.g0 = geo_y_main(nx, ny, H, line_tile_cols(ny), split_xb_log2(nx));
        a.g1 = geo_y_nyq(nx, ny, line_tile_cols(ny));
        a.g1_strided = 1;
        for (int g = 0; g < n_grids; g++) {
            geo_ptrs(a.g0, g, wk[g], wk[g]);
            geo_ptrs(a.g1, g, wk[g] + nlines * H, wk[g] + nlines * H);
        }
        if ((st = dispatch_line_pass<+1>(ny, a, 0, stream))) return st;
    }
    return 0;
}

extern "C" int c21hip_split_filter_xy2_pair(const float *src_a, float *work_a, float *work_a2,
                                            int filter_a, float R_param_a, const float *src_b,
                                            float *work_b, float *work_b2, int filter_b,
                                            float R_param_b, int nx, int ny, int nz,
                                            double box_len, double box_len_z, float R, float R2,
                                            int table_slot, int table_slot2, int phases,
                                            void *stream_) {
    return filter_xy_pair(src_a, work_a, work_a2, filter_a, R_param_a, src_b, work_b, work_b2,
                          filter_b, R_param_b, nx, ny, nz, box_len, box_len_z, R, R2, table_slot,
                          table_slot2, phases, stream_);
}

extern "C" int c21hip_split_filter_xy_shared_pair(const float *src, float *work, float *work2,
                                                  int filter_type, int nx, int ny, int nz,
                                                  double box_len, double box_len_z, float R,
                                                  float R2, int table_slot, int table_slot2,
                                                  int phases, void *stream_) {
    return filter_xy_pair(src, work, work2, filter_type, 0.f, nullptr, nullptr, nullptr, 0, 0.f,
                          nx, ny, nz, box_len, box_len_z, R, R2, table_slot, table_slot2, phases,
                          stream_, 1);
}

extern "C" int c21hip_split_filter_x_pair1(const float *src, float *work, float *work2, int filter_type,
                                           int nx, int ny, int nz, double box_len, double box_len_z, float R,
                                           float R2, int phases, void *stream_) {
    return filter_xy_pair(src, work, work2, filter_type, 0.f, nullptr, nullptr, nullptr, 0, 0.f, nx, ny, nz,
                          box_len, box_len_z, R, R2, 0, 1, phases & ~1, stream_, 1, true);
}

extern "C" int c21hip_split_filter_xy2_pair_eval(const float *src_a, float *work_a, float *work_a2, int filter_a,
                                                 const float *src_b, float *work_b, float *work_b2, int filter_b,
                                                 int nx, int ny, int nz, double box_len, double box_len_z, float R,
                                                 float R2, int phases, void *stream_) {
    return filter_xy_pair(src_a, work_a, work_a2, filter_a, 0.f, src_b, work_b, work_b2, filter_b, 0.f, nx, ny, nz,
                          box_len, box_len_z, R, R2, 0, 1, phases & ~1, stream_, 2, true);
}

extern "C" int c21hip_split_filter_shell(const float *src_a, float *work_a, int filter_a,
                                         const float *src_b, float *work_b, int filter_b,
                                         int n_grids, int nx, int ny, int nz, double box_len,
                                         double box_len_z, float R_inner, float R_outer,
                                         float R_star, int apply, void *stream_) {
    const float *src[2] = {src_a, src_b};
    float *work[2] = {work_a, work_b};
    const int ft[2] = {filter_a, filter_b};
    const float rp[2] = {R_outer, R_outer};
    return filter_xy(src, work, n_grids, nx, ny, nz, box_len, box_len_z, ft, R_inner, rp, apply,
                     stream_, 7, 0, R_star);
}

extern "C" int c21hip_split_sepop_xy(const float *split_src, float *split_work, int nx, int ny,
                                     int nz, double box_len, double box_len_z, int axis0,
                                     int axis1, void *stream_) {
    if (!c21hip_native_fft_supported(nx, ny, nz)) {
        c21hip_set_error("native FFT does not support %dx%dx%d", nx, ny, nz);
        return C21CM_VALUE_ERROR;
    }
    if (axis0 < 0 || axis0 > 2 || axis1 > 2) return C21CM_VALUE_ERROR;
    hipStream_t stream = (hipStream_t)stream_;
    const int H = nz / 2;
    const long nlines = (long)nx * ny;
    LinePassArgs a{};
    a.fp.type = -1;
    a.n_y = ny;
    a.n_z = nz;
    a.out_scale = 1.0f;
    int e[3] = {0, 0, 0};
    e[axis0]++;
    if (axis1 >= 0) e[axis1]++;
    a.op_ex = e[0];
    a.op_ey = e[1];
    a.op_ez = e[2];
    a.op_imag = axis1 < 0;
    a.op_sign = axis1 < 0 ? 1. : -1.;
    a.op_dkx = 2.0 * M_PI / box_len;
    a.op_dky = 2.0 * M_PI / box_len;
    a.op_dkz = 2.0 * M_PI / box_len_z;
    a.n_geo = 2;
    a.n_grids = 1;
    a.g0 = geo_x_main(ny, H, line_tile_cols(nx), split_xb_log2(nx));
    a.g1 = geo_x_nyq(ny, line_tile_cols(nx));
    const float2 *src = reinterpret_cast<const float2 *>(split_src);
    float2 *work = reinterpret_cast<float2 *>(split_work);
    geo_ptrs(a.g0, 0, src, work);
    geo_ptrs(a.g1, 0, src + nlines * H, work + nlines * H);
    int st = dispatch_line_pass<+1>(nx, a, 4, stream);
    if (st) return st;
    a.g0 = geo_y_main(nx, ny, H, line_tile_cols(ny), split_xb_log2(nx));
    a.g1 = geo_y_nyq(nx, ny, line_tile_cols(ny));
    a.g1_strided = 1;
    geo_ptrs(a.g0, 0, work, work);
    geo_ptrs(a.g1, 0, work + nlines * H, work + nlines * H);
    return dispatch_line_pass<+1>(ny, a, 0, stream);
}

extern "C" int c21hip_window_tables(int table_slot, int filter_a, float R_param_a, int filter_b,
                                    float R_param_b, int nx, int ny, int nz, double box_len,
                                    double box_len_z, float R, void *stream_) {
    const float *src[2] = {nullptr, nullptr};
    float *work[2] = {nullptr, nullptr};
    const int ft[2] = {filter_a, filter_b};
    const float rp[2] = {R_param_a, R_param_b};
    return filter_xy(src, work, 2, nx, ny, nz, box_len, box_len_z, ft, R, rp, 1, stream_, 1,
                     table_slot);
}

static bool wev_static_ok(int filter_a, int filter_b, int n_grids, int nx, int ny, int nz, int pair,
                          int *worst_out, int *cap_out) {
    if (!wev_type_ok(filter_a) || (n_grids == 2 && !wev_type_ok(filter_b))) return false;
    if (nx < 128 || (nx & (nx - 1)) || nx > 1024 || !c21hip_native_fft_supported(nx, ny, nz))
        return false;
    const int f1 = n_grids == 2 ? filter_b : filter_a;
    const bool any_tophat = (filter_a == 0) || (n_grids == 2 && f1 == 0);
    const int n_mfp_windows = (filter_a == 3 ? 1 : 0) + (n_grids == 2 && f1 == 3 ? 1 : 0);
    const int worst = (any_tophat ? 1 : 0) + n_mfp_windows * (pair && nx <= 512 ? 2 : 1);
    if (worst > 3 || n_mfp_windows > 1) return false;
    const size_t fixed = wev_lds(nx, pair && nx <= 512, 0, 0);
    const size_t room = fixed < 158 * 1024 ? 158 * 1024 - fixed : 0;
    const int cap = (int)(room / (sizeof(float) * 3 * (size_t)(worst > 0 ? worst : 1)));
    if (cap < 32 * 4 + 3) return false;
    if (worst_out) *worst_out = worst;
    if (cap_out) *cap_out = cap;
    return true;
}

extern "C" int c21hip_wev_prepare(int filter_a, float R_param_a, int filter_b, float R_param_b,
                                  int n_grids, const float *R, int n_R, int nx, int ny, int nz,
                                  double box_len, double box_len_z, int pair, int *enabled,
                                  void *stream_) {
    *enabled = 0;
    g_wev.active = false;
    const char *env = getenv("C21CM_WINDOWS");
    const int by_table = (env && env[0] == 't') ? 1 : 0;
    int worst = 0, cap = 0;
    if (by_table || n_R < 1 || !wev_static_ok(filter_a, filter_b, n_grids, nx, ny, nz, pair, &worst, &cap))
        return 0;
    WevSet &w = g_wev;
    w.filter[0] = filter_a;
    w.filter[1] = n_grids == 2 ? filter_b : filter_a;
    w.R_param[0] = R_param_a;
    w.R_param[1] = n_grids == 2 ? R_param_b : R_param_a;
    w.nx = nx, w.ny = ny, w.nz = nz;
    w.box_len = box_len, w.box_len_z = box_len_z;
    w.R.assign(R, R + n_R);
    float R_max = 0.f;
    for (int i = 0; i < n_R; i++) R_max = R[i] > R_max ? R[i] : R_max;
    const double kx = M_PI * nx / box_len, ky = M_PI * ny / box_len, kz = M_PI * nz / box_len_z;
    const double x_max = sqrt(kx * kx + ky * ky + kz * kz) * R_max * (1. + 1e-6);
    w.n_nodes = (int)(x_max * 4.) + 3;
    const bool any_tophat = (w.filter[0] == 0) || (n_grids == 2 && w.filter[1] == 0);
    const int n_mfp_windows = (w.filter[0] == 3 ? 1 : 0) + (n_grids == 2 && w.filter[1] == 3 ? 1 : 0);
    w.first_type = any_tophat ? 0 : 3;
    w.n_tabs = (any_tophat ? 1 : 0) + n_mfp_windows * n_R;
    {
        const int need = w.n_nodes;
        if (w.n_nodes > cap) w.n_nodes = cap;
        if (w.n_nodes > 4096) w.n_nodes = 4096;
        w.covers = (w.n_nodes == need);
    }
    if (w.n_tabs == 0) {
        w.n_tabs = 1;
        w.first_type = 0;
    }
// ... 251 lines not shown
}

extern "C" int c21hip_split_z_fcoll_erfc(const float *split_work, float *nion_dense, int nx,
                                         int ny, int nz, double growthf, double sigma_min,
                                         double sigma_max, double delta_c, double *partials,
                                         double *sum_out, void *stream) {
    const long nlines = (long)nx * ny;
    ZPassArgs z{};
    z.ny = ny;
    z.lb = split_xb_log2(nx);
    z.main = reinterpret_cast<const float2 *>(split_work);
    z.nyq = z.main + nlines * (nz / 2);
    z.out_scale = 1.0f;
    z.f_out = nion_dense;
    z.p0 = partials;
    z.delta_c = delta_c;
    z.sig = -1.;
    {
        const float ss = (float)sigma_min, sl = (float)sigma_max;
        if (sl > ss) {
            c21hip_set_error("FgtrM requested in a region where M_min > M_max (sigma %g > %g)",
                             (double)sl, (double)ss);
            return C21CM_VALUE_ERROR;
        }
        if (sl != ss)
            z.sig = 1.0 / ((double)(float)growthf * (sqrt(2.) * sqrt((double)(ss * ss - sl * sl))));
    }
    int st;
    {
        KTimeScope kt(12, (hipStream_t)stream);
        st = dispatch_z_c2r<2>(nz, z, nlines, (hipStream_t)stream);
    }
    if (st || !sum_out) return st;
    return c21hip_reduce_sum(partials, (int)(nlines / LZ_PLAIN), sum_out, stream);
}

extern "C" int c21hip_z_fcoll_erfc_mask_supported(int nx, int ny, int nz) {
    return (nz == 512 || nz == 1024) && zw_lines_of(nz, (long)nx * ny) != 0;
}
extern "C" int c21hip_split_z_fcoll_erfc_mask(const float *split_work, float *nion_dense,
                                              const float *nion_prev, const double *mean_prev_dev,
                                              unsigned char *first_cross, int r_index_prev, int fix_mean,
                                              double mean_f_coll, int mass_dep_zeta, double f_limit,
                                              double ion_eff, int nx, int ny, int nz, double growthf,
                                              double sigma_min, double sigma_max, double delta_c,
                                              double *partials, double *sum_out, void *stream) {
    if (!c21hip_z_fcoll_erfc_mask_supported(nx, ny, nz) || nion_prev == nion_dense) {
        c21hip_set_error("pass Z with the deferred barrier: unsupported box or aliased f_coll grids");
        return C21CM_VALUE_ERROR;
    }
    const long nlines = (long)nx * ny;
    ZPassArgs z{};
    z.ny = ny;
    z.lb = split_xb_log2(nx);
    z.main = reinterpret_cast<const float2 *>(split_work);
    z.nyq = z.main + nlines * (nz / 2);
    z.out_scale = 1.0f;
    z.f_out = nion_dense;
    z.f_prev = nion_prev;
    z.mean_dev = mean_prev_dev;
    z.mask_rw = first_cross;
    z.r_index = r_index_prev;
    z.fix_mean = fix_mean;
    z.mean_f_coll = mean_f_coll;
    z.mass_dep_zeta = mass_dep_zeta;
    z.f_limit = f_limit;
    z.ion_eff = ion_eff;
    z.p0 = partials;
    z.delta_c = delta_c;
    z.sig = -1.;
    {
        const float ss = (float)sigma_min, sl = (float)sigma_max;
        if (sl > ss) {
            c21hip_set_error("FgtrM requested in a region where M_min > M_max (sigma %g > %g)",
                             (double)sl, (double)ss);
            return C21CM_VALUE_ERROR;
        }
        if (sl != ss)
            z.sig = 1.0 / ((double)(float)growthf * (sqrt(2.) * sqrt((double)(ss * ss - sl * sl))));
    }
    int st = dispatch_z_c2r<6>(nz, z, nlines, (hipStream_t)stream);
    if (st) return st;
    return c21hip_reduce_sum(partials, (int)(nlines / LZ_PLAIN), sum_out, stream);
}

extern "C" int c21hip_split_z_fcoll_erfc_band(const float *split_work, float *f_pend,
                                              const double *band_dev, const double *thr_prev_dev,
                                              unsigned char *first_cross, int r_index, int r_prev, int nx,
                                              int ny, int nz, double growthf, double sigma_min,
                                              double sigma_max, double delta_c, double *partials,
                                              double *sum_out, void *stream) {
    if (!c21hip_z_fcoll_erfc_mask_supported(nx, ny, nz) || r_index <= 0 || r_index >= 255 || r_prev >= 255) {
        c21hip_set_error("pass Z with the banded barrier: unsupported box or radius index");
        return C21CM_VALUE_ERROR;
    }
    const long nlines = (long)nx * ny;
    ZPassArgs z{};
    z.ny = ny;
    z.lb = split_xb_log2(nx);
    z.main = reinterpret_cast<const float2 *>(split_work);
    z.nyq = z.main + nlines * (nz / 2);
    z.out_scale = 1.0f;
    z.f_out = f_pend;
    z.band = band_dev;
    z.mean_dev = thr_prev_dev;
    z.mask_rw = first_cross;
    z.r_index = r_index;
    z.r_prev = r_prev;
    z.p0 = partials;
    z.delta_c = delta_c;
    z.sig = -1.;
    {
        const float ss = (float)sigma_min, sl = (float)sigma_max;
        if (sl > ss) {
            c21hip_set_error("FgtrM requested in a region where M_min > M_max (sigma %g > %g)",
                             (double)sl, (double)ss);
            return C21CM_VALUE_ERROR;
        }
        if (sl != ss)
            z.sig = 1.0 / ((double)(float)growthf * (sqrt(2.) * sqrt((double)(ss * ss - sl * sl))));
    }
    int st;
    {
        KTimeScope kt(12, (hipStream_t)stream);
        st = dispatch_z_c2r<7>(nz, z, nlines, (hipStream_t)stream);
    }
    if (st || !sum_out) return st;
    return c21hip_reduce_sum(partials, (int)(nlines / LZ_PLAIN), sum_out, stream);
}

extern "C" int c21hip_split_filter_c2r(const float *split_src, float *split_work, float *real_out,
                                       long out_zstride, int nx, int ny, int nz, double box_len,
                                       double box_len_z, int filter_type, float R, float R_param,
                                       int apply, void *stream) {
    int st = c21hip_split_filter_xy(split_src, split_work, nx, ny, nz, box_len, box_len_z,
                                    filter_type, R, R_param, apply, stream);
    if (st) return st;
    return c21hip_split_z_c2r(split_work, real_out, out_zstride, nx, ny, nz, stream);
}

extern "C" int c21hip_split_z_ionise_stars(const float *delta_work, const float *stars_work,
                                           unsigned char *first_cross, double *partials,
                                           double *sum_out, int nx, int ny, int nz, int r_index,
                                           double rhocrit_omb, double ion_eff, int mass_dep_zeta,
                                           double f_limit, void *stream) {
    return c21hip_split_z_ionise_stars_xe(delta_work, stars_work, NULL, first_cross, partials,
                                          sum_out, nx, ny, nz, r_index, rhocrit_omb, ion_eff,
                                          mass_dep_zeta, f_limit, stream);
}

static int z_ionise_stars(const float *delta_work, const float *stars_work, const float *xe_work,
                          unsigned char *first_cross, unsigned *cross_bits, double *partials,
                          double *sum_out, int nx, int ny, int nz, int r_index, double rhocrit_omb,
                          double ion_eff, int mass_dep_zeta, double f_limit, void *stream) {
    const long nlines = (long)nx * ny;
    ZFusedArgs a{};
    a.ny = ny;
    a.lb = split_xb_log2(nx);
    a.d_main = reinterpret_cast<const float2 *>(delta_work);
    a.d_nyq = a.d_main + nlines * (nz / 2);
    a.s_main = reinterpret_cast<const float2 *>(stars_work);
    a.s_nyq = a.s_main + nlines * (nz / 2);
    if (xe_work) {
        a.x_main = reinterpret_cast<const float2 *>(xe_work);
        a.x_nyq = a.x_main + nlines * (nz / 2);
    }
    a.first_cross = first_cross;
    a.cross_bits = cross_bits;
    a.partials = partials;
    a.rhocrit_omb = rhocrit_omb;
    a.ion_eff = ion_eff;
    a.f_limit = f_limit;
    a.mass_dep_zeta = mass_dep_zeta;
    a.r_index = r_index;
    static const int store_all = [] {
        const char *e = getenv("C21CM_MASK_STORE_ALL");
        return (e && e[0] == '1') ? 1 : 0;
    }();
    a.store_all = store_all;
    static const int reverse = [] {
        const char *e = getenv("C21CM_ZREV");
        return (e && e[0] == '0') ? 0 : 1;
    }();
    a.reverse = reverse;
    int n_partials = 0;
    int st = dispatch_z_fused(nz, a, nlines, (hipStream_t)stream, &n_partials);
    if (st) return st;
    if (!sum_out) return 0;
    return c21hip_reduce_sum(partials, n_partials, sum_out, stream);
}

extern "C" int c21hip_split_z_ionise_stars_xe(const float *delta_work, const float *stars_work,
                                              const float *xe_work, unsigned char *first_cross,
                                              double *partials, double *sum_out, int nx, int ny,
                                              int nz, int r_index, double rhocrit_omb,
                                              double ion_eff, int mass_dep_zeta, double f_limit,
                                              void *stream) {
    return z_ionise_stars(delta_work, stars_work, xe_work, first_cross, nullptr, partials, sum_out, nx,
                          ny, nz, r_index, rhocrit_omb, ion_eff, mass_dep_zeta, f_limit, stream);
}

extern "C" int c21hip_z_cross_bits_supported(int nx, int ny, int nz) {
    static const int on = [] {
        const char *e = getenv("C21CM_CROSS_BITS");
        return (e && e[0] == '0') ? 0 : 1;
    }();
    return on && nz == 512 && zw_lines_of(nz, (long)nx * ny) != 0;
}

extern "C" int c21hip_split_z_ionise_stars_bits(const float *delta_work, const float *stars_work,
                                                unsigned *cross_plane, double *partials,
                                                double *sum_out, int nx, int ny, int nz, int r_index,
                                                double rhocrit_omb, double ion_eff,
                                                int mass_dep_zeta, double f_limit, void *stream) {
    if (!cross_plane || !c21hip_z_cross_bits_supported(nx, ny, nz)) {
        c21hip_set_error("fused pass Z: crossing bits are not available for this grid");
        return C21CM_VALUE_ERROR;
    }
    return z_ionise_stars(delta_work, stars_work, nullptr, nullptr, cross_plane, partials, sum_out, nx,
                          ny, nz, r_index, rhocrit_omb, ion_eff, mass_dep_zeta, f_limit, stream);
}

extern "C" int c21hip_split_z_ionise_recomb_xe(const float *delta_work, const float *stars_work,
                                               const float *xe_work, const float *nrec, double rec0,
                                               float *g12, unsigned char *first_cross, double *partials,
                                               int nx, int ny, int nz, int r_index, double rhocrit_omb,
                                               double ion_eff, int mass_dep_zeta, double f_limit,
                                               void *stream);
extern "C" int c21hip_split_z_ionise_recomb(const float *delta_work, const float *stars_work,
                                            const float *nrec, double rec0, float *g12,
                                            unsigned char *first_cross,
                                            double *partials, int nx, int ny, int nz, int r_index,
                                            double rhocrit_omb, double ion_eff, int mass_dep_zeta,
                                            double f_limit, void *stream) {
    return c21hip_split_z_ionise_recomb_xe(delta_work, stars_work, nullptr, nrec, rec0, g12, first_cross,
                                           partials, nx, ny, nz, r_index, rhocrit_omb, ion_eff,
                                           mass_dep_zeta, f_limit, stream);
}
extern "C" int c21hip_split_z_ionise_recomb_xe(const float *delta_work, const float *stars_work,
                                               const float *xe_work, const float *nrec, double rec0,
                                               float *g12, unsigned char *first_cross, double *partials,
                                               int nx, int ny, int nz, int r_index, double rhocrit_omb,
                                               double ion_eff, int mass_dep_zeta, double f_limit,
                                               void *stream) {
    const long nlines = (long)nx * ny;
    ZFusedArgs a{};
    if (xe_work) {
        a.x_main = reinterpret_cast<const float2 *>(xe_work);
        a.x_nyq = a.x_main + nlines * (nz / 2);
    }
    a.ny = ny;
    a.lb = split_xb_log2(nx);
    a.d_main = reinterpret_cast<const float2 *>(delta_work);
    a.d_nyq = a.d_main + nlines * (nz / 2);
    a.s_main = reinterpret_cast<const float2 *>(stars_work);
    a.s_nyq = a.s_main + nlines * (nz / 2);
    a.first_cross = first_cross;
    a.partials = partials;
    a.rhocrit_omb = rhocrit_omb;
    a.ion_eff = ion_eff;
    a.f_limit = f_limit;
    a.mass_dep_zeta = mass_dep_zeta;
    a.r_index = r_index;
#ifdef C21CM_DIAG_BUILD
    a.rc = getenv("C21CM_DIAG_RC_NOSTORE") ? 2 : 1;
#else
    a.rc = 1;
#endif
    a.nrec = nrec;
    a.rec0 = rec0;
    a.g12 = g12;
    a.reverse = 1;
    int n_partials = 0;
    return dispatch_z_fused(nz, a, nlines, (hipStream_t)stream, &n_partials);
}
extern "C" int c21hip_split_z_ionise_recomb_nrec(const float *delta_work, const float *stars_work,
                                                 const float *nrec_work, float *g12,
                                                 unsigned char *first_cross, double *partials, int nx,
                                                 int ny, int nz, int r_index, double rhocrit_omb,
                                                 double ion_eff, int mass_dep_zeta, double f_limit,
                                                 void *stream) {
    const long nlines = (long)nx * ny;
    ZFusedArgs a{};
    a.x_main = reinterpret_cast<const float2 *>(nrec_work);
    a.x_nyq = a.x_main + nlines * (nz / 2);
    a.x_is_nrec = 1;
    a.ny = ny;
    a.lb = split_xb_log2(nx);
    a.d_main = reinterpret_cast<const float2 *>(delta_work);
    a.d_nyq = a.d_main + nlines * (nz / 2);
    a.s_main = reinterpret_cast<const float2 *>(stars_work);
    a.s_nyq = a.s_main + nlines * (nz / 2);
    a.first_cross = first_cross;
    a.partials = partials;
    a.rhocrit_omb = rhocrit_omb;
    a.ion_eff = ion_eff;
    a.f_limit = f_limit;
    a.mass_dep_zeta = mass_dep_zeta;
    a.r_index = r_index;
    a.rc = 1;
    a.g12 = g12;
    a.reverse = 1;
    int n_partials = 0;
    return dispatch_z_fused(nz, a, nlines, (hipStream_t)stream, &n_partials);
}
extern "C" int c21hip_split_z_sfr_gamma12(const float *sfr_work, const unsigned char *first_cross,
                                          float *g12, int nx, int ny, int nz, int r_index,
                                          double g12_scale, void *stream) {
    const long nlines = (long)nx * ny;
    const int zwl = zw_lines_of(nz, nlines);
    if (!zwl || zw3_selected(nz, nlines) || nz > 512) return C21CM_VALUE_ERROR;
    const float2 *twH = twiddles(nz / 2);
    const float2 *twN = twiddles(nz);
    if (!twH || !twN) return C21CM_MEMORY_ALLOC_ERROR;
    ZPassArgs z{};
    z.ny = ny;
    z.lb = split_xb_log2(nx);
    z.main = reinterpret_cast<const float2 *>(sfr_work);
    z.nyq = z.main + nlines * (nz / 2);
    z.out = g12;
    z.out_zstride = nz;
    z.out_scale = 1.0f;
    z.const_factor = g12_scale;
    z.mask = first_cross;
    z.r_index = r_index;
    const dim3 grid((unsigned)(nlines / zwl));
    if (nz == 256)
        hipLaunchKernelGGL((zw_c2r_kernel<16, 4, 8>), grid, dim3(kBlock), 0, (hipStream_t)stream, z, twH, twN);
    else
        hipLaunchKernelGGL((zw_c2r_kernel<16, 4, 16>), grid, dim3(kBlock), 0, (hipStream_t)stream, z, twH, twN);
    LAUNCH_CHECK();
    return 0;
}
extern "C" int c21hip_z_xe_mask_supported(int nx, int ny, int nz) {
    const long nlines = (long)nx * ny;
    return zw_lines_of(nz, nlines) != 0 && !zw3_selected(nz, nlines) && (nz == 256 || nz == 512);
}
extern "C" int c21hip_split_z_xe_mask(const float *xe_work, const float *nion_dense, const double *mean_dev,
                                      unsigned char *first_cross, int nx, int ny, int nz, int r_index,
                                      double mean_f_coll, int fix_mean, int mass_dep_zeta, double f_limit,
                                      double ion_eff, void *stream) {
    if (!c21hip_z_xe_mask_supported(nx, ny, nz)) return C21CM_VALUE_ERROR;
    const long nlines = (long)nx * ny;
    const int zwl = zw_lines_of(nz, nlines);
    const float2 *twH = twiddles(nz / 2);
    const float2 *twN = twiddles(nz);
    if (!twH || !twN) return C21CM_MEMORY_ALLOC_ERROR;
    ZPassArgs z{};
    z.ny = ny;
    z.lb = split_xb_log2(nx);
    z.main = reinterpret_cast<const float2 *>(xe_work);
    z.nyq = z.main + nlines * (nz / 2);
    z.out_zstride = nz;
    z.out_scale = 1.0f;
    z.f_out = const_cast<float *>(nion_dense);
    z.mask_rw = first_cross;
    z.mean_dev = mean_dev;
    z.mean_f_coll = mean_f_coll;
    z.fix_mean = fix_mean;
    z.mass_dep_zeta = mass_dep_zeta;
    z.f_limit = f_limit;
    z.ion_eff = ion_eff;
    z.r_index = r_index;
    KTimeScope kt(11, (hipStream_t)stream);
    const dim3 grid((unsigned)(nlines / zwl));
    if (nz == 256)
        hipLaunchKernelGGL((zw_c2r_kernel<16, 5, 8>), grid, dim3(kBlock), 0, (hipStream_t)stream, z, twH, twN);
    else if (nz == 512)
        hipLaunchKernelGGL((zw_c2r_kernel<16, 5, 16>), grid, dim3(kBlock), 0, (hipStream_t)stream, z, twH, twN);
    else
        return C21CM_VALUE_ERROR;
    LAUNCH_CHECK();
    return 0;
// ... 321 lines not shown
```

21cmfast_amd/csrc/hip/ws_slots.h:

```cpp
#ifndef C21_WS_SLOTS_H
#define C21_WS_SLOTS_H

enum c21_ws_slot {
    WS_DELTA_UNF,
    WS_DELTA_FIL,
    WS_STARS_UNF,
    WS_STARS_FIL,
    WS_XE_UNF,
    WS_XE_FIL,
    WS_DENSITY,
    WS_NION,
    WS_XE_DENSE,
    WS_TNEUTRAL,
    WS_PREV_ZRE,
    WS_XH,
    WS_ZRE,
    WS_TK,
    WS_NION_DENSE,
    WS_SCALARS,
    WS_TABLE,
    WS_FIRST_CROSS,
    WS_CROSS_BITS,
    WS_DELTA_WORK,
    WS_STARS_WORK,
// ... 102 lines not shown
    WS_WSFR,
    WS_PREV_NREC,
    WS_G12,
    WS_MFP,
    WS_NREC_OUT,
    WS_RR_TABLES,
    WS_SH_XH,
    WS_SH_ZRE,
    WS_SH_G12,
    WS_SH_MFP,

    WS_SHARD_GRID,
    WS_SHARD_STAGE,
    WS_SHARD_SCALARS,
    WS_SHARD_BITS,

    WS_TS_DENS,
    WS_TS_PTS,
    WS_TS_PTK,
    WS_TS_PXE,
    WS_TS_GRID_A,
    WS_TS_GRID_B,
    WS_TS_TAB,
    WS_TS_SFRDTAB,
    WS_TS_LYA_C,
    WS_TS_LYA_I,
    WS_TS_OTS,
    WS_TS_OTK,
    WS_TS_OXE,
    WS_TS_PART,
    WS_TS_SMALL,
    WS_TS_MEANSFR,
    WS_TS_SFRDTAB2,
    WS_TS_SUMS,

    WS_ABI_TS_FILTERED,
    WS_ABI_MEAN_PART,
    WS_ABI_TS_MCRIT,
    WS_ABI_TS_MCRIT_R,

    WS_MINI_PD_UNF,
    WS_MINI_PD_WORK,
    WS_MINI_PD_FIL,
    WS_MINI_MTA_UNF,
    WS_MINI_MTA_WORK,
    WS_MINI_MTA_FIL,
    WS_MINI_MTM_UNF,
    WS_MINI_MTM_WORK,
    WS_MINI_MTM_FIL,
    WS_MINI_PDENS,
    WS_MINI_MTA,
    WS_MINI_MTM,
    WS_MINI_TABLES,
    WS_MINI_HIST_A,
    WS_MINI_HIST_M,
    WS_MINI_OUT_A,
    WS_MINI_OUT_M,
    WS_MT_G12,
    WS_MT_ZRE,
    WS_MT_J21,
    WS_MT_VCB,
    WS_MT_OUT_A,
    WS_MT_OUT_M,
    WS_MT_SC,
    WS_MT_PART,

    WS_ABI_ION_MTA,
    WS_ABI_ION_MTM,

    WS_TS_MINI_TAB,
    WS_TS_MINI_MCRIT,
    WS_TS_MINI_SHELL,
    WS_TS_MINI_J21,
    WS_TS_MINI_MEAN,
    WS_TS_MCRIT_J21,
    WS_TS_MCRIT_VCB,
    WS_TS_MCRIT_OUT,

    WS_SPHERE_RSQ,

    WS_HBM_MTA,
    WS_HBM_MTM,
    WS_HBM_TAB,
    WS_HBM_ACC3,
    WS_HBM_OUT4,
    WS_HBM_G12,
    WS_HBM_ZRE,
    WS_HBM_J21,
    WS_HBM_VCB,
    WS_HBM_OUTA,
    WS_HBM_OUTM,
    WS_HBM_SUMS,
    WS_ABI_HB_MTA,
    WS_ABI_HB_MTM,
    WS_HC_MASS,
    WS_HC_COORD,
    WS_HC_RNG0,
    WS_HC_RNG1,
    WS_HC_RNG2,
    WS_HC_WSFR,
    WS_HC_BINS,

    WS_HP0,
    WS_HP_LAST = WS_HP0 + 9,
    WS_WEV_NODES = WS_HP0 + 2,
    WS_WEV_MFP = WS_HP0 + 3,
    WS_TSS_SUMS = WS_HP0 + 4,
    WS_TSS_SEND = WS_HP0 + 5,
    WS_TSS_RECV = WS_HP0 + 6,
    WS_TSS_SLAB = WS_HP0 + 7,
    WS_SFR_WORK2 = WS_HP0 + 8,
    WS_R_DEV = WS_HP_LAST,

    WS_SHARD_RC_MASK,
    WS_SHARD_RC_G12,

    WS_EUL_XEPEND,
    WS_NION_DENSE2,
    WS_GSL_ROW_KIND,
    WS_SHARD_STATUS,
    WS_SHARD_SLABBITS,
    WS_ARENA,
    WS_NREC_WORK2,
    WS_TSS_ROWMAX,
    WS_EUL_WORK3,
    WS_EUL_WORK4,

    WS_LC_TAB,
    WS_LC_BOXES,
    WS_LC_SLAB,
    WS_LC_HUBBLE,
    WS_LC_DVDR,
    WS_RSD_SCALE,
    WS_RSD_IN,
    WS_RSD_OUT,
    WS_RSD_FLAG,
    WS_RSD_VEL,
    WS_ANG_NHAT,
    WS_ANG_TAB,
    WS_ANG_BOXES,
    WS_ANG_SLAB,
    WS_ANG_FLAG,
    WS_PREFILTER_IN,
    WS_PREFILTER_OUT,
    WS_PW_TAB,
    WS_PW_IN,
    WS_PW_PAD,
    WS_PW_SUMS,
    WS_PW_FLAG,
    WS_PH_IN,
    WS_PH_OUT,
    WS_PH_GRIDS,

    WS_COUNT
};

#endif
```

21cmfast_amd/csrc/host/ionize_driver.c:

```c
#include <math.h>
#include <stdio.h>
#include <stdlib.h>
#include <string.h>

#include "../hip/c21hip.h"
#include "c21cm_grid.h"

#define MAX_COPYBACK 12
typedef struct {
    void *host[MAX_COPYBACK];
    void *dev[MAX_COPYBACK];
    size_t bytes[MAX_COPYBACK];
    int n;
} copyback_list;

#define SC_SUMS 0
#define SC_MEANS (SC_SUMS + C21CM_MAX_RADII)
#define SC_MINMAX (SC_MEANS + C21CM_MAX_RADII)
#define SC_XHSUM (SC_MINMAX + 4)
#define SC_FLAG (SC_XHSUM + 1)
#define SC_G12SUM (SC_FLAG + 1)
#define SC_SUMS_M (SC_G12SUM + 1)
#define SC_MEANS_M (SC_SUMS_M + C21CM_MAX_RADII)
#define SC_MINMAX_M (SC_MEANS_M + C21CM_MAX_RADII)
// ... 57 lines not shown
    if (s->recomb_model != C21CM_RECOMB_NONE) {
        if (s->recomb_model != C21CM_RECOMB_HOMOGENEOUS &&
            s->recomb_model != C21CM_RECOMB_INHOMOGENEOUS) {
            c21hip_set_error("ionize: unknown recomb_model %d", s->recomb_model);
            return C21CM_VALUE_ERROR;
        }
        if (!s->rr_y || !s->rr_c) {
            c21hip_set_error("ionize: a recombination model needs the rr_y / rr_c rate tables");
            return C21CM_VALUE_ERROR;
        }
        if (!box->ionisation_rate_G12 || !box->cumulative_recombinations) {
            c21hip_set_error("ionize: a recombination model needs ionisation_rate_G12 and "
                             "cumulative_recombinations");
            return C21CM_VALUE_ERROR;
        }
        if (s->recomb_model == C21CM_RECOMB_HOMOGENEOUS && !s->cell_recomb) {
            c21hip_set_error("ionize: RECOMB_MODEL = homogeneous needs CELL_RECOMB");
            return C21CM_VALUE_ERROR;
        }
        if (s->fcoll_mode == C21CM_FCOLL_STARS_GRID && (!halos || !halos->whalo_sfr)) {
            c21hip_set_error("ionize: Lagrangian sources with recombinations need HaloBox.whalo_sfr");
            return C21CM_VALUE_ERROR;
        }
    }
    if (s->fcoll_mode < C21CM_FCOLL_STARS_GRID || s->fcoll_mode > C21CM_FCOLL_NODES) {
        c21hip_set_error("ionize: unknown fcoll_mode %d", s->fcoll_mode);
        return C21CM_VALUE_ERROR;
    }
    if (s->use_mini_halos && s->fcoll_mode == C21CM_FCOLL_STARS_GRID) {
    } else if (s->use_mini_halos) {
        if (s->fcoll_mode != C21CM_FCOLL_TABLE_EXP || !s->table2d_fn) {
            c21hip_set_error("ionize: USE_MINI_HALOS runs on the E-INTEGRAL tables (fcoll_mode "
                             "TABLE_EXP) and needs table2d_fn");
            return C21CM_VALUE_ERROR;
        }
        if (!s->prev_density || !s->log10_mturn_acg || !s->log10_mturn_mcg ||
            !box->unnormalised_nion_mini) {
            c21hip_set_error("ionize: USE_MINI_HALOS needs prev_density, the two log10 M_turn "
                             "grids and IonizedBox.unnormalised_nion_mini");
            return C21CM_VALUE_ERROR;
        }
    } else if (s->fcoll_mode >= C21CM_FCOLL_TABLE_LINEAR && !s->table_fn) {
        c21hip_set_error("ionize: TABLE fcoll_mode needs table_fn");
        return C21CM_VALUE_ERROR;
    }
    if (s->ionise_entire_sphere) {
        if (s->recomb_model != C21CM_RECOMB_NONE || s->use_mini_halos) {
            c21hip_set_error("ionize: IONISE_ENTIRE_SPHERE with a recombination model or mini-halos "
                             "is not built (upstream's result depends on its thread order there)");
            return C21CM_VALUE_ERROR;
        }
        if (sphere_rsq(s, 0) > 1.f) {
            c21hip_set_error("ionize: IONISE_ENTIRE_SPHERE needs a cell-scale radius below one cell");
            return C21CM_VALUE_ERROR;
        }
    }
    if (!pf->density || !box->neutral_fraction || !box->z_reion) {
        c21hip_set_error("ionize: density / neutral_fraction / z_reion arrays are required");
        return C21CM_VALUE_ERROR;
    }
    if (s->fcoll_mode == C21CM_FCOLL_STARS_GRID && (!halos || !halos->n_ion)) {
        c21hip_set_error("ionize: Lagrangian source model needs HaloBox.n_ion");
        return C21CM_VALUE_ERROR;
    }
    if (s->fcoll_mode != C21CM_FCOLL_STARS_GRID && !box->unnormalised_nion) {
        c21hip_set_error("ionize: Eulerian source model needs IonizedBox.unnormalised_nion");
        return C21CM_VALUE_ERROR;
    }
    if (s->use_ts_fluct &&
        (!ts || !ts->xray_ionised_fraction || (!s->minimize_memory && !ts->kinetic_temp_neutral))) {
        c21hip_set_error("ionize: USE_TS_FLUCT needs the TsBox arrays");
        return C21CM_VALUE_ERROR;
    }
    if (!s->minimize_memory && !box->kinetic_temperature) {
        c21hip_set_error("ionize: kinetic_temperature is required unless MINIMIZE_MEMORY");
        return C21CM_VALUE_ERROR;
    }
    return 0;
}

static void fill_args(c21hip_ionize_args *a, const c21cm_ionize_spec *s, int r_index) {
    memset(a, 0, sizeof(*a));
    a->nx = s->hii_dim;
    a->ny = s->hii_dim;
    a->nz = s->hii_dim_z;
    a->r_index = r_index;
    a->lagrangian = (s->fcoll_mode == C21CM_FCOLL_STARS_GRID);
    a->mass_dep_zeta = s->mass_dep_zeta;
    a->use_ts_fluct = s->use_ts_fluct;
    a->minimize_memory = s->minimize_memory;
    a->first_snapshot = s->first_snapshot;
    a->fix_mean = s->fix_mean;
    a->mean_f_coll = s->mean_f_coll;
    a->f_limit = s->f_limit_acg;
    a->ion_eff_factor = s->ion_eff_factor;
    a->rhocrit_omb = s->rhocrit_omb;
    a->photoncons_factor = s->photoncons_adjustment_factor;
    a->redshift = s->redshift;
    a->TK_nofluct = s->TK_nofluct;
    a->adia_TK_term = s->adia_TK_term;
    a->T_re = s->T_re;
}

typedef struct {
    const c21cm_ionize_spec *s;
    void *stream;
    int nx, ny, nz;
    size_t ntot, npad;
    int lagrangian;
    int native;
    float *delta_unf, *delta_fil, *stars_unf, *stars_fil, *xe_unf, *xe_fil;
    float *delta_work, *stars_work, *xe_work;
    float *delta_work2, *stars_work2, *xe_work2;
    int recomb, inhomo, filter_rec;
    float *sfr_unf, *sfr_fil, *sfr_work, *nrec_unf, *nrec_fil, *nrec_work;
    const float *whalo_sfr, *prev_nrec;
    float *G12, *mfp, *nrec_out;
    double *rr_dev;
    int pair_radii;
    const float *density, *n_ion, *xe_dense, *Tneutral, *prev_zre;
    float *xH, *zre, *Tk, *nion_dense;
    double *scalars;
    double *partials;
    float *table_dev;
    int fused;
    double *def_partials;
    long def_stride;
    int def_first, def_step, def_count;
    int tab_seq;
    int wev;
    int fused_rc;
    int eul_pend, eul_pend_buf;
    unsigned char *eul_pend_mask;
    float *nion_dense2;
    int band_off;
    int band_used;
    int band_next;
    int band_pend;
    int band_h1, band_h2, band_hn;
    unsigned char *band_mask;
    const unsigned char *r0_mask;
    int r0_slab, r0_cb, r0_ce;
    int band_mf;
    int band_skip;
    short band_hist[C21CM_MAX_RADII][3];
    float *band_xe_pend;
    const float *cur_xe;
    int x3_on, x3_nrec;
    float *x3_unf, *x3_work, *x3_work2;
    int x4_on;
    float *x4_unf, *x4_work, *x4_work2;
    const float *cur_x4;
    unsigned *cross_bits;
    float *sfr_work2;
    double rec0;
    int finalised;
    float *eul_xe[2];
    int wev_pair, pairx_R;
    float *pairx_buf;
    int sphere;
    int mini, lag_mini;
    float *pd_unf, *pd_work, *pd_fil, *mta_unf, *mta_work, *mta_fil, *mtm_unf, *mtm_work, *mtm_fil;
    const float *prev_density, *mta_dense, *mtm_dense, *hist_a, *hist_m;
    float *mini_tables, *nion_all, *mini_all;
    int eul_mask;
    copyback_list cb;
    size_t cb_cell0, cb_ncell;
} ion_ctx;

static int r0_direct(void);

static int g_loop_flags;
int c21cm_ionize_last_loop_flags(void) { return g_loop_flags; }

static int ctx_setup(ion_ctx *c, const c21cm_ionize_spec *s, const PerturbedField *pf,
                     const IonizedBox *prev, const TsBox *ts, const HaloBox *halos,
                     IonizedBox *box, int need_outputs, int fused_rc_ok, void *stream) {
    int status = 0;
    memset(c, 0, sizeof(*c));
    c->s = s;
    c->stream = stream;
    c->nx = s->hii_dim;
    c->ny = s->hii_dim;
    c->nz = s->hii_dim_z;
    c->ntot = (size_t)c->nx * c->ny * c->nz;
    c->npad = (size_t)c->nx * c->ny * 2 * (size_t)(c->nz / 2 + 1);
    c->lagrangian = (s->fcoll_mode == C21CM_FCOLL_STARS_GRID);
    const size_t gbytes = c->npad * sizeof(float), dbytes = c->ntot * sizeof(float);

    c->native = c21hip_fft_is_native(c->nx, c->ny, c->nz);
    char *arena = NULL;
    size_t astep = 0;
    {
        const char *e = getenv("C21CM_ARENA");
        if (e && c->lagrangian) {
            const size_t skew = (size_t)atol(e);
            astep = ((gbytes + ((size_t)2 << 20) - 1) & ~(((size_t)2 << 20) - 1)) + skew;
            arena = (char *)c21hip_ws(WS_ARENA, 4 * astep);
            if (!arena) return C21CM_MEMORY_ALLOC_ERROR;
        }
    }
    c->delta_unf = arena ? (float *)arena : (float *)c21hip_ws(WS_DELTA_UNF, gbytes);
    c->delta_fil = (float *)c21hip_ws(WS_DELTA_FIL, gbytes);
    if (!c->delta_unf || !c->delta_fil) return C21CM_MEMORY_ALLOC_ERROR;
    if (c->native && !(c->delta_work = arena ? (float *)(arena + 2 * astep) : (float *)c21hip_ws(WS_DELTA_WORK, gbytes)))
        return C21CM_MEMORY_ALLOC_ERROR;
    if (c->lagrangian) {
        c->stars_unf = arena ? (float *)(arena + astep) : (float *)c21hip_ws(WS_STARS_UNF, gbytes);
        c->stars_fil = (float *)c21hip_ws(WS_STARS_FIL, gbytes);
        if (!c->stars_unf || !c->stars_fil) return C21CM_MEMORY_ALLOC_ERROR;
        if (c->native && !(c->stars_work = arena ? (float *)(arena + 3 * astep)
                                                 : c21_place_work_partner(WS_DELTA_WORK, WS_STARS_WORK, gbytes, c->nx, c->ny,
                                                                      c->nz, stream)))
            return C21CM_MEMORY_ALLOC_ERROR;
    }
    if (s->use_ts_fluct) {
        c->xe_unf = (float *)c21hip_ws(WS_XE_UNF, gbytes);
        c->xe_fil = (float *)c21hip_ws(WS_XE_FIL, gbytes);
        if (!c->xe_unf || !c->xe_fil) return C21CM_MEMORY_ALLOC_ERROR;
        if (c->native && !(c->xe_work = !c->lagrangian ? c21_place_work_partner(WS_DELTA_WORK, WS_XE_WORK, gbytes, c->nx,
                                                                                c->ny, c->nz, stream)
                                                       : (float *)c21hip_ws(WS_XE_WORK, gbytes)))
            return C21CM_MEMORY_ALLOC_ERROR;
    }
    {
        size_t np = (size_t)c->nx * c->ny / 4;
        np += np / 512 + 16;
        if (np < C21HIP_PARTIALS) np = C21HIP_PARTIALS;
        c->partials = (double *)c21hip_ws(WS_PARTIALS, np * sizeof(double));
        if (!c->partials) return C21CM_MEMORY_ALLOC_ERROR;
    }
    c->recomb = (s->recomb_model != C21CM_RECOMB_NONE);
    c->inhomo = (s->recomb_model == C21CM_RECOMB_INHOMOGENEOUS);
    c->filter_rec = c->recomb && !s->cell_recomb;
    c->fused = c->native && c->lagrangian && !c->recomb &&
               (!s->use_ts_fluct ||
                (c21hip_z_ionise_xe_supported(c->nx, c->ny, c->nz) && r0_direct()));
    c->fused_rc = 0;
    const char *e_nr = getenv("C21CM_RECOMB_FUSED_NREC");
    const int nrec_ok = s->cell_recomb ||
                        (c->inhomo && fused_rc_ok && !(e_nr && e_nr[0] == '0') &&
                         (s->use_ts_fluct ? c21hip_z_ionise_recomb_xe_nrec_supported(c->nx, c->ny, c->nz)
                                          : c21hip_z_ionise_recomb_xe_supported(c->nx, c->ny, c->nz)));
    c->x3_on = c->x3_nrec = 0;
    c->x3_unf = c->x3_work = c->x3_work2 = NULL;
    c->x4_on = 0;
    c->x4_unf = c->x4_work = c->x4_work2 = NULL;
    c->cur_x4 = NULL;
    if (c->native && c->lagrangian && c->recomb && nrec_ok &&
        !s->use_mini_halos && !s->ionise_entire_sphere && s->r_lowest == 0 &&
        fused_rc_ok) {
        const char *e = getenv("C21CM_RECOMB_FUSED"), *et = getenv("C21CM_RECOMB_FUSED_TS");
        const int ts_ok = !s->use_ts_fluct ||
                          (!(et && et[0] == '0') && r0_direct() &&
                           c21hip_z_ionise_recomb_xe_supported(c->nx, c->ny, c->nz));
        if (!(e && e[0] == '0') && ts_ok && c21hip_z_ionise_recomb_supported(c->nx, c->ny, c->nz) &&
            c21hip_wev_applicable(s->hii_filter, s->stars_filter, 2, c->nx, c->ny, c->nz))
            c->fused_rc = c->fused = 1;
    }
    c->eul_pend = -1;
    c->eul_pend_buf = 0;
    c->eul_pend_mask = NULL;
    c->wev_pair = 0;
    c->pairx_R = -1;
    c->pairx_buf = NULL;
    c->nion_dense2 = NULL;
    c->band_off = c->band_used = 0;
    c->band_next = c->band_pend = c->band_h1 = c->band_h2 = -1;
    c->band_hn = 0;
    c->band_mask = NULL;
    c->band_mf = 0;
    c->r0_mask = NULL;
    c->band_skip = -1;
    c->band_xe_pend = NULL;
    c->sphere = s->ionise_entire_sphere;
    c->mini = s->use_mini_halos && !c->lagrangian;
    c->lag_mini = s->use_mini_halos && c->lagrangian;
    if (c->lag_mini) c->fused = 0;
    c->eul_mask = c->native && !c->lagrangian && !c->recomb && !c->mini;
    if (c->mini) {
        const int slots[9] = {WS_MINI_PD_UNF, WS_MINI_PD_WORK, WS_MINI_PD_FIL,
                              WS_MINI_MTA_UNF, WS_MINI_MTA_WORK, WS_MINI_MTA_FIL,
                              WS_MINI_MTM_UNF, WS_MINI_MTM_WORK, WS_MINI_MTM_FIL};
        float **dst[9] = {&c->pd_unf, &c->pd_work, &c->pd_fil, &c->mta_unf, &c->mta_work,
                          &c->mta_fil, &c->mtm_unf, &c->mtm_work, &c->mtm_fil};
        for (int i = 0; i < 9; i++) {
            if (!c->native && i % 3 == 1) continue;
            if (!(*dst[i] = (float *)c21hip_ws(slots[i], gbytes))) return C21CM_MEMORY_ALLOC_ERROR;
        }
        c->mini_tables = (float *)c21hip_ws(
            WS_MINI_TABLES, 4 * sizeof(float) * C21CM_NDELTA_TABLE * C21CM_NMTURN_TABLE);
        if (!c->mini_tables) return C21CM_MEMORY_ALLOC_ERROR;
    }
    if (c->filter_rec) {
        c->nrec_unf = (float *)c21hip_ws(WS_NREC_UNF, gbytes);
        c->nrec_fil = (float *)c21hip_ws(WS_NREC_FIL, gbytes);
        if (!c->nrec_unf || !c->nrec_fil) return C21CM_MEMORY_ALLOC_ERROR;
        if (c->native && !(c->nrec_work = (float *)c21hip_ws(WS_NREC_WORK, gbytes)))
            return C21CM_MEMORY_ALLOC_ERROR;
    }
    if (c->recomb && c->lagrangian) {
        c->sfr_unf = (float *)c21hip_ws(WS_SFR_UNF, gbytes);
        c->sfr_fil = (float *)c21hip_ws(WS_SFR_FIL, gbytes);
        if (!c->sfr_unf || !c->sfr_fil) return C21CM_MEMORY_ALLOC_ERROR;
        const int x3_slot = s->use_ts_fluct ? WS_XE_WORK : (c->filter_rec ? WS_NREC_WORK : -1);
        if (c->native &&
// ... 127 lines not shown

static struct {
    int valid, nx, nz, ts;
    int stars_r0_ready;
    const void *density, *n_ion, *xe;
    double factor;
} g_spectra;

static int spectra_match(const ion_ctx *c, const PerturbedField *pf, const HaloBox *halos,
                         const TsBox *ts) {
    return g_spectra.valid && g_spectra.nx == c->nx && g_spectra.nz == c->nz &&
           g_spectra.ts == c->s->use_ts_fluct && g_spectra.density == (const void *)pf->density &&
           g_spectra.n_ion == (const void *)(c->lagrangian ? halos->n_ion : NULL) &&
           g_spectra.xe == (const void *)(c->s->use_ts_fluct ? ts->xray_ionised_fraction : NULL) &&
           g_spectra.factor == c->s->photoncons_adjustment_factor;
}

static void spectra_remember(const ion_ctx *c, const PerturbedField *pf, const HaloBox *halos,
                             const TsBox *ts) {
    g_spectra.valid = 1;
    g_spectra.stars_r0_ready = 0;
    g_spectra.nx = c->nx;
    g_spectra.nz = c->nz;
    g_spectra.ts = c->s->use_ts_fluct;
    g_spectra.density = pf->density;
    g_spectra.n_ion = c->lagrangian ? halos->n_ion : NULL;
    g_spectra.xe = c->s->use_ts_fluct ? ts->xray_ionised_fraction : NULL;
    g_spectra.factor = c->s->photoncons_adjustment_factor;
}

static int prepare_grid(ion_ctx *c, const float *dense, float *cgrid, float *scratch,
                        double factor, double lo, double hi) {
    int status = 0;
    (void)scratch;
    if (c->native) {
        TRY(c21hip_split_r2c(dense, c->nz, cgrid, c->nx, c->ny, c->nz, factor, lo, hi,
                             1.0f / (float)c->ntot, c->stream));
        goto done;
    }
    float *padded = cgrid;
    TRY(c21hip_pack_clip(dense, padded, c->nx, c->ny, c->nz, factor, lo, hi, c->stream));
    TRY(c21hip_fft_r2c(padded, c->nx, c->ny, c->nz, c->stream));
    TRY(c21hip_divide_inplace(padded, c->npad, (float)c->ntot, c->stream));
done:
    return status;
}

static int filter_to_real(ion_ctx *c, const float *unf, float *work, float *fil, int filter_type,
                          float R, float R_param, int apply) {
    int status = 0;
    const c21cm_ionize_spec *s = c->s;
    if (c->native) {
        TRY(c21hip_split_filter_c2r(unf, work, fil, 2 * (long)(c->nz / 2 + 1), c->nx, c->ny, c->nz,
                                    s->box_len, s->box_len_z, filter_type, R, R_param, apply,
                                    c->stream));
    } else {
        TRY(c21hip_copy_filter(unf, fil, c->nx, c->ny, c->nz, s->box_len, s->box_len_z,
                               filter_type, R, R_param, apply, c->stream));
        TRY(c21hip_fft_c2r(fil, c->nx, c->ny, c->nz, c->stream));
    }
done:
    return status;
}

static int preloop(ion_ctx *c) {
    int status = 0;
    const c21cm_ionize_spec *s = c->s;
    TRY(prepare_grid(c, c->density, c->delta_unf, c->delta_fil, s->photoncons_adjustment_factor,
                     -1., 1e6));
    if (c->lagrangian) TRY(prepare_grid(c, c->n_ion, c->stars_unf, c->stars_fil, 1., 0., 1e20));
    if (s->use_ts_fluct) TRY(prepare_grid(c, c->xe_dense, c->xe_unf, c->xe_fil, 1., 0., 1.));
    if (c->recomb && c->lagrangian)
        TRY(prepare_grid(c, c->whalo_sfr, c->sfr_unf, c->sfr_fil, 1., 0., 1e20));
    if (c->filter_rec) TRY(prepare_grid(c, c->prev_nrec, c->nrec_unf, c->nrec_fil, 1., 0., 1e20));
    if (c->mini) {
        TRY(prepare_grid(c, c->prev_density, c->pd_unf, c->pd_fil, 1., -1., 1e6));
        TRY(prepare_grid(c, c->mtm_dense, c->mtm_unf, c->mtm_fil, 1., -INFINITY, INFINITY));
        TRY(prepare_grid(c, c->mta_dense, c->mta_unf, c->mta_fil, 1., -INFINITY, INFINITY));
    }
done:
    return status;
}

static struct {
    int init, enabled;
    void *aux, *ev_table[4], *ev_used[4], *ev_sync;
} g_tab;

static void tab_init(void) {
    if (g_tab.init) return;
    g_tab.init = 1;
    const char *e = getenv("C21CM_ASYNC_TABLES");
    if (e && e[0] == '0') return;
    g_tab.aux = c21hip_aux_stream();
    g_tab.ev_sync = c21hip_event_create();
    g_tab.enabled = g_tab.aux && g_tab.ev_sync;
    for (int b = 0; b < 4; b++) {
        g_tab.ev_table[b] = c21hip_event_create();
        g_tab.ev_used[b] = c21hip_event_create();
        g_tab.enabled = g_tab.enabled && g_tab.ev_table[b] && g_tab.ev_used[b];
    }
}

static int tab_build_async(ion_ctx *c, int R_ct, int buf) {
    int status = 0;
    const c21cm_ionize_spec *s = c->s;
    TRY(c21hip_stream_wait_event(g_tab.aux, g_tab.ev_used[buf]));
#ifdef C21CM_DIAG_BUILD
    static int skip = -1;
    if (skip < 0) skip = getenv("C21CM_DIAG_SKIP_TABLES") != NULL;
    if (!(skip && c->tab_seq > 0))
#endif
    TRY(c21hip_window_tables(buf, s->hii_filter, 0.f, s->stars_filter, (float)s->mfp_meandens,
                             c->nx, c->ny, c->nz, s->box_len, s->box_len_z, (float)s->R[R_ct],
                             g_tab.aux));
    TRY(c21hip_event_record(g_tab.ev_table[buf], g_tab.aux));
done:
    return status;
}

static int eul_flush_pending(ion_ctx *c, int last) {
    if (c->eul_pend < 0) return 0;
    c21hip_ionize_args args;
    fill_args(&args, c->s, c->eul_pend);
    const int R = c->eul_pend;
    c->eul_pend = -1;
    int st = c21hip_eulerian_mask(&args, c->eul_pend_buf ? c->nion_dense2 : c->nion_dense, NULL,
                                  c->scalars + SC_MEANS + R, c->eul_pend_mask, c->stream);
    if (!st && last && c->eul_pend_buf)
        st = c21hip_d2d(c->nion_dense, c->nion_dense2, c->ntot * sizeof(float), c->stream);
    return st;
}

static int flush_deferred(ion_ctx *c) {
    {
        const int st_e = eul_flush_pending(c, 1);
        if (st_e) return st_e;
    }
    if (!c->def_partials || c->def_count == 0) return 0;
    const c21cm_ionize_spec *s = c->s;
    int st = c21hip_batched_means(c->def_partials, c->def_stride, (int)c->def_stride, c->def_first,
                                  c->def_count > 1 ? c->def_step : 1, c->def_count,
                                  (double)c->ntot, s->mass_dep_zeta, s->f_limit_acg,
                                  c->scalars + SC_SUMS, c->scalars + SC_MEANS, c->stream);
    c->def_count = 0;
    return st;
}

static int z_ionise_radius(ion_ctx *c, int R_ct, const float *dwork, const float *swork,
                           const float *xwork, unsigned char *first_cross) {
    int status = 0;
    const c21cm_ionize_spec *s = c->s;
    unsigned *plane = c->cross_bits ? c->cross_bits + (size_t)(R_ct - 1) * (c->ntot / 32) : NULL;
    if (c->fused_rc) {
        double *part = c->def_partials ? c->def_partials + (long)R_ct * c->def_stride : c->partials;
        if (c->def_partials) {
            if (c->def_count == 0)
                c->def_first = R_ct;
            else if (c->def_count == 1)
                c->def_step = c->def_first - R_ct;
            else if (R_ct != c->def_first - c->def_count * c->def_step)
                TRY(flush_deferred(c));
            if (c->def_count == 0) c->def_first = R_ct;
            c->def_count++;
        }
        if (c->x4_on)
            TRY(c21hip_split_z_ionise_recomb_xe_nrec(dwork, swork, c->cur_xe, c->cur_x4, c->G12, first_cross,
                                                     part, c->nx, c->ny, c->nz, R_ct, s->rhocrit_omb,
                                                     s->ion_eff_factor, s->mass_dep_zeta, s->f_limit_acg,
                                                     c->stream));
        else if (c->x3_nrec)
            TRY(c21hip_split_z_ionise_recomb_nrec(dwork, swork, c->cur_xe, c->G12, first_cross, part, c->nx,
                                                  c->ny, c->nz, R_ct, s->rhocrit_omb, s->ion_eff_factor,
                                                  s->mass_dep_zeta, s->f_limit_acg, c->stream));
        else
        TRY(c21hip_split_z_ionise_recomb_xe(dwork, swork, s->use_ts_fluct ? c->cur_xe : NULL,
                                            c->inhomo ? c->prev_nrec : NULL, c->rec0, c->G12, first_cross,
                                            part, c->nx, c->ny, c->nz, R_ct, s->rhocrit_omb,
                                            s->ion_eff_factor, s->mass_dep_zeta, s->f_limit_acg, c->stream));
        TRY(c21hip_split_z_sfr_gamma12(xwork, first_cross, c->G12, c->nx, c->ny, c->nz, R_ct,
                                       s->R[R_ct] * s->gamma_prefactor, c->stream));
        if (!c->def_partials) {
            double *sum_dev = c->scalars + SC_SUMS + R_ct;
            TRY(c21hip_reduce_sum(part, c21hip_z_ionise_partials(c->nx, c->ny, c->nz), sum_dev, c->stream));
            TRY(c21hip_finish_mean(sum_dev, (double)c->ntot, s->mass_dep_zeta, s->f_limit_acg,
                                   c->scalars + SC_MEANS + R_ct, c->stream));
        }
        goto done;
    }
    if (c->def_partials) {
        if (c->def_count == 0)
            c->def_first = R_ct;
        else if (c->def_count == 1)
            c->def_step = c->def_first - R_ct;
        else if (R_ct != c->def_first - c->def_count * c->def_step)
            TRY(flush_deferred(c));
        if (c->def_count == 0) c->def_first = R_ct;
        c->def_count++;
        if (plane)
            TRY(c21hip_split_z_ionise_stars_bits(dwork, swork, plane,
                                                 c->def_partials + (long)R_ct * c->def_stride, NULL,
                                                 c->nx, c->ny, c->nz, R_ct, s->rhocrit_omb,
                                                 s->ion_eff_factor, s->mass_dep_zeta, s->f_limit_acg,
                                                 c->stream));
        else
        TRY(c21hip_split_z_ionise_stars_xe(dwork, swork, xwork, first_cross,
                                           c->def_partials + (long)R_ct * c->def_stride, NULL,
                                           c->nx, c->ny, c->nz, R_ct, s->rhocrit_omb,
                                           s->ion_eff_factor, s->mass_dep_zeta, s->f_limit_acg,
                                           c->stream));
        goto done;
    }
    {
        double *sum_dev = c->scalars + SC_SUMS + R_ct;
        if (plane)
            TRY(c21hip_split_z_ionise_stars_bits(dwork, swork, plane, c->partials, sum_dev, c->nx, c->ny,
                                                 c->nz, R_ct, s->rhocrit_omb, s->ion_eff_factor,
                                                 s->mass_dep_zeta, s->f_limit_acg, c->stream));
        else
        TRY(c21hip_split_z_ionise_stars_xe(dwork, swork, xwork, first_cross, c->partials, sum_dev,
                                           c->nx, c->ny, c->nz, R_ct, s->rhocrit_omb,
                                           s->ion_eff_factor, s->mass_dep_zeta, s->f_limit_acg,
                                           c->stream));
        TRY(c21hip_finish_mean(sum_dev, (double)c->ntot, s->mass_dep_zeta, s->f_limit_acg,
                               c->scalars + SC_MEANS + R_ct, c->stream));
    }
done:
    return status;
}

static int fused_step(ion_ctx *c, int R_a, int R_b, unsigned char *first_cross, int next_a,
                      int next_b) {
    int status = 0;
    const c21cm_ionize_spec *s = c->s;
    const int set = c->tab_seq & 1;
    const int buf_a = 2 * set, buf_b = 2 * set + 1;
    tab_init();
    const int tab_async = !c->wev && g_tab.enabled && c->ntot >= ((size_t)1 << 26);
    if (tab_async) {
        if (c->tab_seq == 0) {
            TRY(c21hip_event_record(g_tab.ev_sync, c->stream));
            TRY(c21hip_stream_wait_event(g_tab.aux, g_tab.ev_sync));
            TRY(tab_build_async(c, R_a, buf_a));
            if (R_b >= 1) TRY(tab_build_async(c, R_b, buf_b));
        }
        if (next_a >= 1) TRY(tab_build_async(c, next_a, 2 * (set ^ 1)));
        if (next_b >= 1) TRY(tab_build_async(c, next_b, 2 * (set ^ 1) + 1));
        TRY(c21hip_stream_wait_event(c->stream, g_tab.ev_table[buf_a]));
        if (R_b >= 1) TRY(c21hip_stream_wait_event(c->stream, g_tab.ev_table[buf_b]));
    }
    if (R_b >= 1) {
        static int yy = -1;
        if (yy < 0) {
            const char *e = getenv("C21CM_PAIR_ORDER");
            yy = (e && e[0] == 'y') ? 1 : 0;
        }
        const float *xw[2] = {c->fused_rc ? c->sfr_work : (s->use_ts_fluct ? c->xe_work : NULL),
                              c->fused_rc ? c->sfr_work2 : (s->use_ts_fluct ? c->xe_work2 : NULL)};
        const float *xe_of[2] = {c->x3_on ? c->x3_work : NULL, c->x3_on ? c->x3_work2 : NULL};
        for (int ph = 0; ph < 3; ph++) {
            const int bits = ph == 0 ? (tab_async ? 2 : 3) : (4 << (ph - 1));
            TRY(c21hip_split_filter_xy2_pair(
                c->delta_unf, c->delta_work, c->delta_work2, s->hii_filter, 0.f, c->stars_unf,
                c->stars_work, c->stars_work2, s->stars_filter, (float)s->mfp_meandens, c->nx,
                c->ny, c->nz, s->box_len, s->box_len_z, (float)s->R[R_a], (float)s->R[R_b], buf_a,
                buf_b, bits, c->stream));
            static int merge34 = -1;
            if (merge34 < 0) {
                const char *e = getenv("C21CM_RECOMB_MERGE34");
                merge34 = (e && e[0] == '0') ? 0 : 1;
            }
            if (c->x3_on && c->fused_rc && c->wev && merge34) {
                TRY(c21hip_split_filter_xy2_pair(
                    c->x3_unf, c->x3_work, c->x3_work2, s->hii_filter, 0.f, c->sfr_unf, c->sfr_work,
                    c->sfr_work2, s->stars_filter, (float)s->mfp_meandens, c->nx, c->ny, c->nz,
                    s->box_len, s->box_len_z, (float)s->R[R_a], (float)s->R[R_b], buf_a, buf_b,
                    bits & ~1, c->stream));
            } else {
            if (c->x3_on)
                TRY(c21hip_split_filter_xy_shared_pair(
                    c->x3_unf, c->x3_work, c->x3_work2, s->hii_filter, c->nx, c->ny, c->nz,
                    s->box_len, s->box_len_z, (float)s->R[R_a], (float)s->R[R_b], buf_a, buf_b,
                    bits & ~1, c->stream));
            if (c->fused_rc)
                TRY(c21hip_split_filter_xy_single_pair(
                    c->sfr_unf, c->sfr_work, c->sfr_work2, s->stars_filter, (float)s->mfp_meandens,
                    c->nx, c->ny, c->nz, s->box_len, s->box_len_z, (float)s->R[R_a],
                    (float)s->R[R_b], bits & ~1, c->stream));
            }
            if (c->x4_on)
                TRY(c21hip_split_filter_xy_shared_pair(
                    c->x4_unf, c->x4_work, c->x4_work2, s->hii_filter, c->nx, c->ny, c->nz,
                    s->box_len, s->box_len_z, (float)s->R[R_a], (float)s->R[R_b], buf_a, buf_b,
                    bits & ~1, c->stream));
            if (ph == (yy ? 2 : 1) && tab_async) {
                TRY(c21hip_event_record(g_tab.ev_used[buf_a], c->stream));
                TRY(c21hip_event_record(g_tab.ev_used[buf_b], c->stream));
            }
            if (ph == 1 && !yy) {
                c->cur_xe = xe_of[0];
                c->cur_x4 = c->x4_work;
                TRY(z_ionise_radius(c, R_a, c->delta_work, c->stars_work, xw[0], first_cross));
            }
        }
        c->tab_seq++;
        if (yy) {
            c->cur_xe = xe_of[0];
            c->cur_x4 = c->x4_work;
            TRY(z_ionise_radius(c, R_a, c->delta_work, c->stars_work, xw[0], first_cross));
        }
        c->cur_xe = xe_of[1];
        c->cur_x4 = c->x4_work2;
        TRY(z_ionise_radius(c, R_b, c->delta_work2, c->stars_work2, xw[1], first_cross));
        goto done;
    } else {
        TRY(c21hip_split_filter_xy2(c->delta_unf, c->delta_work, s->hii_filter, 0.f, c->stars_unf,
                                    c->stars_work, s->stars_filter, (float)s->mfp_meandens, c->nx,
                                    c->ny, c->nz, s->box_len, s->box_len_z, (float)s->R[R_a], 1,
                                    buf_a, tab_async, c->stream));
        if (c->x3_on)
            TRY(c21hip_split_filter_xy_shared(c->x3_unf, c->x3_work, s->hii_filter, c->nx, c->ny,
                                              c->nz, s->box_len, s->box_len_z, (float)s->R[R_a], 1,
                                              buf_a, c->stream));
        if (c->fused_rc)
            TRY(c21hip_split_filter_xy(c->sfr_unf, c->sfr_work, c->nx, c->ny, c->nz, s->box_len,
                                       s->box_len_z, s->stars_filter, (float)s->R[R_a],
                                       (float)s->mfp_meandens, 1, c->stream));
        if (c->x4_on)
            TRY(c21hip_split_filter_xy_shared(c->x4_unf, c->x4_work, s->hii_filter, c->nx, c->ny,
                                              c->nz, s->box_len, s->box_len_z, (float)s->R[R_a], 1,
                                              buf_a, c->stream));
        if (tab_async) TRY(c21hip_event_record(g_tab.ev_used[buf_a], c->stream));
    }
    c->tab_seq++;
    c->cur_xe = c->x3_on ? c->x3_work : NULL;
    c->cur_x4 = c->x4_work;
    TRY(z_ionise_radius(c, R_a, c->delta_work, c->stars_work,
                        c->fused_rc ? c->sfr_work : (s->use_ts_fluct ? c->xe_work : NULL), first_cross));
done:
    return status;
}

static int fused_loop(ion_ctx *c, int first, int step, int lowest, unsigned char *first_cross) {
    int status = 0;
    if (lowest < 1) lowest = 1;
    if (first < lowest) return 0;
    c->wev = 0;
    {
        float radii[C21CM_MAX_RADII];
        int n = 0;
        for (int R = first; R >= lowest && n < C21CM_MAX_RADII; R -= step) radii[n++] = (float)c->s->R[R];
        if (n > 0)
            TRY(c21hip_wev_prepare(c->s->hii_filter, 0.f, c->s->stars_filter, (float)c->s->mfp_meandens,
                                   2, radii, n, c->nx, c->ny, c->nz, c->s->box_len, c->s->box_len_z,
                                   c->pair_radii, &c->wev, c->stream));
    }
    if (c->fused_rc) {
        if (!c->wev) {
            c21hip_set_error("ionize: the fused recombination loop needs the evaluated windows");
            status = C21CM_VALUE_ERROR;
            goto done;
        }
        c->rec0 = 0.;
        if (!c->inhomo) {
            float r0 = 0.f;
            if (c21hip_is_device_ptr(c->prev_nrec)) {
                TRY(c21hip_d2h(&r0, c->prev_nrec, sizeof(float), c->stream));
                TRY(c21hip_sync(c->stream));
            } else {
                r0 = c->prev_nrec[0];
            }
            c->rec0 = (double)r0;
        }
    }
    int R_a = first;
    while (R_a >= lowest) {
        const int want_b = c->pair_radii && R_a - step >= lowest;
        const int R_b = want_b ? R_a - step : -1;
        const int n_a = (want_b ? R_b : R_a) - step;
        const int next_a = n_a >= lowest ? n_a : -1;
        const int next_b = (c->pair_radii && next_a >= 1 && next_a - step >= lowest) ? next_a - step
                                                                                     : -1;
        TRY(fused_step(c, R_a, R_b, first_cross, next_a, next_b));
        R_a = n_a;
    }
done:
    c21hip_wev_release();
    c->wev = 0;
    return status;
}

static int eul_xe_buffers(ion_ctx *c) {
    if (c->eul_xe[0] && c->eul_xe[1]) return 0;
    c->eul_xe[0] = (float *)c21hip_ws(WS_EUL_XE0, c->ntot * sizeof(float));
    c->eul_xe[1] = (float *)c21hip_ws(WS_EUL_XE1, c->ntot * sizeof(float));
    return (c->eul_xe[0] && c->eul_xe[1]) ? 0 : C21CM_MEMORY_ALLOC_ERROR;
}

static int mini_radius(ion_ctx *c, int R_ct, const c21hip_ionize_args *args, int apply, float R) {
    int status = 0;
    const c21cm_ionize_spec *s = c->s;
    const size_t t2 = (size_t)C21CM_NDELTA_TABLE * C21CM_NMTURN_TABLE;
    const size_t roff = (size_t)R_ct * c->ntot;
    double mm[8];
    float *tables = (float *)malloc(sizeof(float) * 4 * t2);
    if (!tables) return C21CM_MEMORY_ALLOC_ERROR;
    TRY(filter_to_real(c, c->pd_unf, c->pd_work, c->pd_fil, s->hii_filter, R, 0.f, apply));
    TRY(filter_to_real(c, c->mtm_unf, c->mtm_work, c->mtm_fil, s->hii_filter, R, 0.f, apply));
    TRY(filter_to_real(c, c->mta_unf, c->mta_work, c->mta_fil, s->hii_filter, R, 0.f, apply));
    TRY(c21hip_clip_minmax(c->delta_fil, c->nx, c->ny, c->nz, c->partials, c->scalars + SC_MINMAX,
                           c->stream));
    TRY(c21hip_clip_minmax(c->pd_fil, c->nx, c->ny, c->nz, c->partials, c->scalars + SC_MINMAX_M,
                           c->stream));
    TRY(c21hip_clip_minmax(c->mta_fil, c->nx, c->ny, c->nz, c->partials,
                           c->scalars + SC_MINMAX_M + 2, c->stream));
    TRY(c21hip_clip_minmax(c->mtm_fil, c->nx, c->ny, c->nz, c->partials,
                           c->scalars + SC_MINMAX_M + 4, c->stream));
    TRY(c21hip_d2h(mm, c->scalars + SC_MINMAX, 2 * sizeof(double), c->stream));
    TRY(c21hip_d2h(mm + 2, c->scalars + SC_MINMAX_M, 6 * sizeof(double), c->stream));
    TRY(c21hip_sync(c->stream));
    {
        const double dmin = mm[0] - 0.001, dmax = mm[1] + 0.001;
        const double pmin = mm[2] - 0.001, pmax = mm[3] + 0.001;
        const double amin = mm[4] * 0.99, amax = mm[5] * 1.01;
        const double mmin = mm[6] * 0.99, mmax = mm[7] * 1.01;
        int tst = s->table2d_fn(R_ct, 0, dmin, dmax, amin, amax, mmin, mmax, tables, tables + t2,
                                s->table2d_user);
        if (!tst && s->need_prev_ion)
            tst = s->table2d_fn(R_ct, 1, pmin, pmax, amin, amax, mmin, mmax, tables + 2 * t2,
                                tables + 3 * t2, s->table2d_user);
        if (tst) {
            c21hip_set_error("ionize: table2d_fn failed with status %d at radius %d", tst, R_ct);
            status = tst;
            goto done;
        }
        const double ranges[8] = {dmin, (dmax - dmin) / (C21CM_NDELTA_TABLE - 1.),
                                  pmin, (pmax - pmin) / (C21CM_NDELTA_TABLE - 1.),
                                  amin, (amax - amin) / (C21CM_NMTURN_TABLE - 1.),
                                  mmin, (mmax - mmin) / (C21CM_NMTURN_TABLE - 1.)};
        TRY(c21hip_h2d(c->mini_tables, tables, sizeof(float) * (s->need_prev_ion ? 4 : 2) * t2,
                       c->stream));
        TRY(c21hip_sync(c->stream));
        TRY(c21hip_fcoll_mini(c->nx, c->ny, c->nz, s->need_prev_ion, ranges, c->delta_fil,
                              c->pd_fil, c->mta_fil, c->mtm_fil, c->mini_tables, c->hist_a + roff,
                              c->hist_m + roff, c->nion_all + roff, c->mini_all + roff, c->partials,
                              c->scalars + SC_PAIR, c->stream));
    }
    TRY(c21hip_d2d(c->scalars + SC_SUMS + R_ct, c->scalars + SC_PAIR, sizeof(double), c->stream));
    TRY(c21hip_d2d(c->scalars + SC_SUMS_M + R_ct, c->scalars + SC_PAIR + 1, sizeof(double),
                   c->stream));
    TRY(c21hip_finish_mean(c->scalars + SC_SUMS + R_ct, (double)c->ntot, s->mass_dep_zeta,
                           s->f_limit_acg, c->scalars + SC_MEANS + R_ct, c->stream));
    TRY(c21hip_finish_mean(c->scalars + SC_SUMS_M + R_ct, (double)c->ntot, s->mass_dep_zeta,
                           s->f_limit_mcg, c->scalars + SC_MEANS_M + R_ct, c->stream));
    TRY(c21hip_ionise_mini(args, 0, c->recomb, c->inhomo, s->cell_recomb, s->R[R_ct],
                           s->gamma_prefactor, s->gamma_prefactor_mini, s->ion_eff_factor_mini,
                           s->f_limit_mcg, s->mean_f_coll_mini, c->delta_fil,
                           c->nion_all + roff, c->mini_all + roff, c->xe_fil, c->nrec_fil,
                           c->prev_nrec, c->density, c->prev_zre, c->Tneutral,
                           c->scalars + SC_MEANS + R_ct, c->scalars + SC_MEANS_M + R_ct, c->xH,
                           c->zre, c->Tk, c->G12, c->mfp, c->partials, NULL, c->stream));
done:
    free(tables);
    return status;
}

static int fcoll_nodes(ion_ctx *c, int R_ct, double *partials, double *sum_dev) {
    int status = 0;
    const c21cm_ionize_spec *s = c->s;
    double nodes[C21CM_NODE_DOUBLES];
    const int tst = s->table_fn(R_ct, 0., 0., (float *)nodes, s->table_user);
    if (tst) {
        c21hip_set_error("ionize: table_fn (node data) failed with status %d at radius %d", tst, R_ct);
        return tst;
    }
    double *nodes_dev = (double *)(c->table_dev + 2 * C21CM_NDELTA_TABLE);
    TRY(c21hip_h2d(nodes_dev, nodes, sizeof(nodes), c->stream));
    TRY(c21hip_sync(c->stream));
    TRY(c21hip_fcoll_eulerian(c->delta_fil, c->nion_dense, c->nx, c->ny, c->nz, C21CM_FCOLL_NODES,
                              s->growth_factor, 0., 0., s->delta_c, 0., 1., (const float *)nodes_dev,
                              partials, sum_dev, c->stream));
done:
    return status;
}

static int eul_defer_ok(ion_ctx *c) {
    const char *e = getenv("C21CM_EUL_DEFER");
    if (!(e && e[0] == '1')) return 0;
    if (!c21hip_z_fcoll_erfc_mask_supported(c->nx, c->ny, c->nz)) return 0;
    if (!c->nion_dense2)
        c->nion_dense2 = (float *)c21hip_ws(WS_NION_DENSE2, c->ntot * sizeof(float));
    return c->nion_dense2 != NULL;
}

static int eul_band_ok(ion_ctx *c) {
    const char *e = getenv("C21CM_EUL_BAND");
    if ((e && e[0] == '0') || c->band_off || c->s->n_radii >= 255) return 0;
    return c21hip_z_fcoll_erfc_mask_supported(c->nx, c->ny, c->nz);
}

static int eul_band_flush(ion_ctx *c) {
    if (c->band_pend < 0) return 0;
    const int R = c->band_pend;
    c->band_pend = -1;
    if (c->band_mf)
        return c21hip_eul_resolve_pending_xe(R, c->nion_dense, c->band_xe_pend, c->scalars + SC_BANDX + R,
                                             c->s->mass_dep_zeta, c->s->f_limit_acg, c->s->ion_eff_factor,
                                             c->band_mask, c->ntot, c->stream);
    return c21hip_eul_resolve_pending(R, c->nion_dense, c->scalars + SC_BANDX + R, c->band_mask, c->ntot,
                                      c->stream);
}

static int eul_band_finish(ion_ctx *c, unsigned char *mask, int *redo) {
    *redo = 0;
    int st = eul_band_flush(c);
    if (st || !c->band_used) return st;
    double cell;
    int fail;
    if ((st = c21hip_d2h(&cell, c->scalars + SC_BANDFAIL, sizeof(cell), c->stream))) return st;
    if ((st = c21hip_sync(c->stream))) return st;
    memcpy(&fail, &cell, sizeof(int));
    if (getenv("C21CM_EUL_BAND_DEBUG")) {
        double b[2 * C21CM_MAX_RADII], t[C21CM_MAX_RADII], m[C21CM_MAX_RADII];
        if (!c21hip_d2h(b, c->scalars + SC_BAND, sizeof(b), c->stream) &&
            !c21hip_d2h(t, c->scalars + SC_BANDX, sizeof(t), c->stream) &&
            !c21hip_d2h(m, c->scalars + SC_MEANS, sizeof(m), c->stream) && !c21hip_sync(c->stream))
            for (int r = c->s->n_radii - 1; r >= 1; r--)
                fprintf(stderr, "band r=%3d mean=%.9e threshold=%.9e sure>=%.9e maybe>=%.9e rel=[%+.2e, %+.2e]\n",
                        r, m[r], t[r], b[2 * r], b[2 * r + 1], b[2 * r] / t[r] - 1., b[2 * r + 1] / t[r] - 1.);
        fprintf(stderr, "band fail=%d\n", fail);
    }
    c->band_used = 0;
    c->band_next = c->band_h1 = c->band_h2 = -1;
    c->band_hn = 0;
    if (fail > 0) {
        c->band_off = 1;
        *redo = fail;
        if ((st = c21hip_memset(c->scalars + SC_BANDFAIL, 0, sizeof(double), c->stream))) return st;
        return c21hip_eul_rewind(mask, fail, c->ntot, c->stream);
    }
    return 0;
// ... 759 lines not shown

static int paint_spheres(ion_ctx *c, const unsigned char *mask) {
    int status = 0;
    const c21cm_ionize_spec *s = c->s;
    float rsq[C21CM_MAX_RADII];
    for (int r = 0; r < s->n_radii; r++) rsq[r] = sphere_rsq(s, r);
    float *rsq_dev = (float *)c21hip_ws(WS_SPHERE_RSQ, sizeof(rsq));
    if (!rsq_dev) return C21CM_MEMORY_ALLOC_ERROR;
    TRY(c21hip_h2d(rsq_dev, rsq, sizeof(rsq), c->stream));
    TRY(c21hip_sync(c->stream));
    TRY(c21hip_paint_spheres(mask, rsq_dev, c->xH, c->nx, c->ny, c->nz, c->stream));
done:
    return status;
}

static int eul_r0_fused(const ion_ctx *c) {
    const char *e = getenv("C21CM_EUL_R0_FUSED");
    return c->eul_mask && !c->sphere && !c->recomb && c->s->r_lowest == 0 && !(e && e[0] == '0') &&
           (!c->s->use_ts_fluct || r0_direct());
}

static int native_wev_prepare(ion_ctx *c) {
    const c21cm_ionize_spec *spec = c->s;
    if (!c->native || c->fused) return 0;
    float radii[C21CM_MAX_RADII];
    int n = 0, on = 0;
    for (int R_ct = spec->n_radii - 1; R_ct >= 1 && R_ct >= spec->r_lowest && n < C21CM_MAX_RADII; R_ct--)
        radii[n++] = (float)spec->R[R_ct];
    if (n == 0) return 0;
    const char *ep = getenv("C21CM_EUL_PAIR");
    const int pair = c->eul_mask && !(ep && ep[0] == '0') && c21hip_pair_sweep_supported(c->nx);
    const int st = c21hip_wev_prepare(spec->hii_filter, 0.f, spec->hii_filter, 0.f, spec->use_ts_fluct ? 2 : 1,
                                      radii, n, c->nx, c->ny, c->nz, spec->box_len, spec->box_len_z, pair, &on,
                                      c->stream);
    c->wev_pair = !st && on && pair;
    return st;
}

typedef struct {
    void *ev[4];
    int n, marked;
} phase_clock;

static int clock_start(phase_clock *k, int n, void *stream) {
    for (k->n = 0; k->n < n; k->n++) k->ev[k->n] = c21hip_event_create();
    k->marked = 1;
    return c21hip_event_record(k->ev[0], stream);
}

static int clock_mark(phase_clock *k, void *stream) { return c21hip_event_record(k->ev[k->marked++], stream); }

static double clock_ms(const phase_clock *k, int i) { return c21hip_event_elapsed_ms(k->ev[i], k->ev[i + 1]); }

static void clock_free(phase_clock *k) {
    while (k->n > 0) c21hip_event_destroy(k->ev[--k->n]);
}

static int radii_ladder(ion_ctx *c, int first, int step, unsigned char *mask, int after) {
    int status = 0;
    const c21cm_ionize_spec *s = c->s;
    const int lowest = s->r_lowest > 1 ? s->r_lowest : 1;
    if (c->fused) return fused_loop(c, first, step, lowest, mask);
    if (c->eul_mask && s->fcoll_mode != C21CM_FCOLL_ERFC && s->fcoll_mode != C21CM_FCOLL_NODES) {
        int radii[C21CM_MAX_RADII], n = 0, redo = 0;
        for (int R_ct = first; R_ct >= lowest; R_ct -= step) radii[n++] = R_ct;
        TRY(eul_table_loop(c, radii, n, mask));
        TRY(eul_band_finish(c, mask, &redo));
        if (redo) {
            int m = 0;
            for (int i = 0; i < n; i++)
                if (radii[i] <= redo) radii[m++] = radii[i];
            TRY(eul_table_loop(c, radii, m, mask));
        }
        goto done;
    }
    for (int attempt = 0, from = first; attempt < 2; attempt++) {
        int redo = 0;
        for (int R_ct = first; R_ct >= lowest; R_ct -= step) {
            if (R_ct > from) continue;
            TRY(one_radius(c, R_ct, mask, R_ct - step >= lowest ? R_ct - step : after));
        }
        TRY(eul_flush_pending(c, after < 0));
        TRY(eul_band_finish(c, mask, &redo));
        if (!redo) break;
        from = redo;
    }
done:
    return status;
}

static int finish_first_cross(ion_ctx *c, const unsigned char *mask, int stars_ready) {
    int status = 0;
    const c21cm_ionize_spec *s = c->s;
    if (c->fused && s->r_lowest == 0 && !c->sphere) return final_step(c, mask, stars_ready);
    if (eul_r0_fused(c)) {
        c->r0_mask = mask;
        return one_radius(c, 0, NULL, -1);
    }
    TRY(c21hip_apply_first_cross(mask, c->prev_zre, s->first_snapshot, s->redshift, c->xH, c->zre, c->ntot,
                                 c->stream));
    if (c->sphere) TRY(paint_spheres(c, mask));
    if (s->r_lowest == 0) TRY(one_radius(c, 0, NULL, -1));
done:
    return status;
}

static int finish_first_cross_recomb(ion_ctx *c, const unsigned char *mask) {
    int status = 0;
    const c21cm_ionize_spec *s = c->s;
    float Rf[C21CM_MAX_RADII];
    for (int r = 0; r < C21CM_MAX_RADII; r++) Rf[r] = r < s->n_radii ? (float)s->R[r] : 0.f;
    float *R_dev = (float *)c21hip_ws(WS_R_DEV, sizeof(Rf));
    if (!R_dev) return C21CM_MEMORY_ALLOC_ERROR;
    TRY(c21hip_h2d(R_dev, Rf, sizeof(Rf), c->stream));
    TRY(c21hip_sync(c->stream));
    TRY(c21hip_apply_first_cross_recomb(mask, R_dev, c->prev_zre, s->first_snapshot, s->redshift, c->xH,
                                        c->zre, c->mfp, c->ntot, c->stream));
    TRY(one_radius(c, 0, NULL, -1));
done:
    return status;
}

static void cross_bits_begin(ion_ctx *c) {
    const c21cm_ionize_spec *s = c->s;
    c->cross_bits = NULL;
    if (!c->fused || c->fused_rc || s->use_ts_fluct || c->sphere || s->n_radii < 2 ||
        !c21hip_z_cross_bits_supported(c->nx, c->ny, c->nz))
        return;
    c->cross_bits = (unsigned *)c21hip_ws(WS_CROSS_BITS, (size_t)(s->n_radii - 1) * (c->ntot / 8));
}

int c21cm_ionize_grids(const c21cm_ionize_spec *spec, const PerturbedField *perturbed_field,
                       const IonizedBox *previous_ionize_box, const TsBox *spin_temp,
                       const HaloBox *halos, IonizedBox *box, c21cm_ionize_report *report,
                       void *stream) {
    int status = validate_spec(spec, perturbed_field, halos, spin_temp, box);
    if (status) return status;
    ion_ctx c;
    phase_clock clk = {{NULL}, 0, 0};
    unsigned char *mask = NULL;
    g_spectra.valid = 0;
    TRY(ctx_setup(&c, spec, perturbed_field, previous_ionize_box, spin_temp, halos, box, 1, 1, stream));
    TRY(clock_start(&clk, 4, stream));
    TRY(init_output_grids(&c, previous_ionize_box));
    TRY(preloop(&c));
    TRY(clock_mark(&clk, stream));
    if (c.fused || c.eul_mask || c.sphere) {
        mask = (unsigned char *)c21hip_ws(WS_FIRST_CROSS, c.ntot);
        if (!mask) {
            status = C21CM_MEMORY_ALLOC_ERROR;
            goto done;
        }
        cross_bits_begin(&c);
        if (!c.cross_bits)
            TRY(c21hip_memset(mask, 0, c.ntot, stream));
    }
    TRY(native_wev_prepare(&c));
    if (mask) {
        TRY(radii_ladder(&c, spec->n_radii - 1, 1, mask, spec->r_lowest == 0 ? 0 : -1));
        if (c.cross_bits) {
            TRY(c21hip_resolve_crossings(c.cross_bits, spec->n_radii - 1, spec->r_lowest > 1 ? spec->r_lowest : 1,
                                         mask, (size_t)c.nx * c.ny, stream));
            c.cross_bits = NULL;
        }
        TRY(flush_deferred(&c));
        TRY(c.fused_rc ? finish_first_cross_recomb(&c, mask) : finish_first_cross(&c, mask, 0));
    } else {
        for (int R_ct = spec->n_radii - 1; R_ct >= spec->r_lowest; R_ct--)
            TRY(one_radius(&c, R_ct, NULL, -1));
        TRY(flush_deferred(&c));
    }
    c21hip_wev_release();
    TRY(clock_mark(&clk, stream));
    TRY(postloop(&c, box, report));
    TRY(clock_mark(&clk, stream));
    if (report) {
        report->ms_preloop = clock_ms(&clk, 0);
        report->ms_rloop = clock_ms(&clk, 1);
        report->ms_postloop = clock_ms(&clk, 2);
    }
done:
    c21hip_wev_release();
    clock_free(&clk);
    return status;
}

static int no_mini_shards(void) {
    c21hip_set_error("ionize: the sharded R loop does not take USE_MINI_HALOS");
    return C21CM_VALUE_ERROR;
}

static struct {
    int valid, n;
    double means[C21CM_MAX_RADII];
} g_shard_means;

int c21cm_ionize_shard_set_means(const double *means, int n_radii) {
    if (!means || n_radii < 0 || n_radii > C21CM_MAX_RADII) {
        g_shard_means.valid = 0;
        return means ? C21CM_VALUE_ERROR : 0;
    }
    memset(g_shard_means.means, 0, sizeof(g_shard_means.means));
    memcpy(g_shard_means.means, means, sizeof(double) * (size_t)n_radii);
    g_shard_means.n = n_radii;
    g_shard_means.valid = 1;
    return 0;
}

static int shard_means_restore(ion_ctx *c) {
    int status = 0;
    if (g_shard_means.valid && g_shard_means.n == c->s->n_radii)
        status = c21hip_h2d(c->scalars + SC_MEANS, g_shard_means.means, sizeof(double) * (size_t)c->s->n_radii,
                            c->stream);
    g_shard_means.valid = 0;
    return status;
}

static int radii_phase_box(const c21cm_ionize_spec *spec, const PerturbedField *pf, const HaloBox *halos,
                           const TsBox *ts, int recomb, IonizedBox *dummy) {
    memset(dummy, 0, sizeof(*dummy));
    if (spec && spec->fcoll_mode != C21CM_FCOLL_STARS_GRID)
        dummy->unnormalised_nion = (float *)c21hip_ws(
            WS_NION_DENSE, (size_t)spec->hii_dim * spec->hii_dim * spec->hii_dim_z * sizeof(float));
    IonizedBox probe = *dummy;
    float sentinel;
    probe.neutral_fraction = probe.z_reion = probe.kinetic_temperature = &sentinel;
    if (recomb) probe.ionisation_rate_G12 = probe.cumulative_recombinations = &sentinel;
    int status = validate_spec(spec, pf, halos, ts, &probe);
    if (!status && spec->use_mini_halos) status = no_mini_shards();
    return status;
}

static int radii_phase_preloop(ion_ctx *c, const PerturbedField *pf, const HaloBox *halos, const TsBox *ts) {
    g_spectra.valid = 0;
    const int status = preloop(c);
    if (!status) spectra_remember(c, pf, halos, ts);
    return status;
}

static int spectra_reuse(ion_ctx *c, const PerturbedField *pf, const HaloBox *halos, const TsBox *ts,
                         int *stars_ready) {
    int status = 0;
    if (spectra_match(c, pf, halos, ts)) {
        if (stars_ready) *stars_ready = g_spectra.stars_r0_ready;
    } else {
        status = preloop(c);
    }
    g_spectra.valid = 0;
    return status;
}

static int radii_phase_report(ion_ctx *c, int world, const phase_clock *k, c21cm_ionize_report *report) {
    int status = 0;
    double means[C21CM_MAX_RADII];
    if (!report) return 0;
    TRY(c21hip_d2h(means, c->scalars + SC_MEANS, sizeof(means), c->stream));
    TRY(c21hip_sync(c->stream));
    report_grid_means(report, means, c->s->n_radii);
    if (world == 1) c21cm_ionize_shard_set_means(means, c->s->n_radii);
    report->ms_preloop = clock_ms(k, 0);
    report->ms_rloop = clock_ms(k, 1);
    report->ms_postloop = 0.;
done:
    return status;
}

static int finish_phase_postloop(ion_ctx *c, IonizedBox *box, c21cm_ionize_report *report, phase_clock *k) {
    int status = 0;
    TRY(clock_mark(k, c->stream));
    TRY(postloop(c, box, report));
    TRY(clock_mark(k, c->stream));
    if (report) {
        report->ms_preloop = 0.;
        report->ms_rloop = clock_ms(k, 0);
        report->ms_postloop = clock_ms(k, 1);
    }
done:
    return status;
}

int c21cm_ionize_shard_radii(const c21cm_ionize_spec *spec, int rank, int world,
                             const PerturbedField *perturbed_field,
                             const IonizedBox *previous_ionize_box, const TsBox *spin_temp,
                             const HaloBox *halos, unsigned char *first_cross,
                             c21cm_ionize_report *report, void *stream) {
    IonizedBox dummy;
    int status = 0;
    if (!first_cross || !c21hip_is_device_ptr(first_cross) || world < 1 || rank < 0 ||
        rank >= world) {
        c21hip_set_error("ionize shard: first_cross must be a device array, 0 <= rank < world");
        return C21CM_VALUE_ERROR;
    }
    if ((status = radii_phase_box(spec, perturbed_field, halos, spin_temp, 0, &dummy))) return status;
    ion_ctx c;
    phase_clock clk = {{NULL}, 0, 0};
    TRY(ctx_setup(&c, spec, perturbed_field, previous_ionize_box, spin_temp, halos, &dummy, 0, 0, stream));
    TRY(clock_start(&clk, 3, stream));
    TRY(c21hip_memset(first_cross, 0, c.ntot, stream));
    TRY(radii_phase_preloop(&c, perturbed_field, halos, spin_temp));
    TRY(clock_mark(&clk, stream));
    TRY(native_wev_prepare(&c));
    TRY(radii_ladder(&c, spec->n_radii - 1 - rank, world, first_cross, -1));
    TRY(flush_deferred(&c));
    if (c.fused && spec->r_lowest == 0 && rank == (spec->n_radii - 1) % world && !r0_direct()) {
        TRY(final_prepare(&c));
        g_spectra.stars_r0_ready = 1;
// ... 430 lines not shown
```

Measured before the change: 3.451 billion cells/s.

## Hoist Nyquist-plane filtering for all radii into one batched pass before the loop

Adds a batched line-pass mode that filters and transforms the kz-Nyquist planes of both grids for every radius up front, storing them in a stack buffer. Per-radius XY passes then skip the Nyquist geometry, and the Z ionise kernel reads the precomputed Nyquist planes. This removes the separate per-radius Nyquist-line work and its launch geometry. In exchange it needs an extra stack of n_R*4*nx*ny floats, a synchronous host-to-device upload of per-pair metadata, and per-pair window-node restaging in LDS inside the batch kernel.

```diff
diff --git a/21cmfast_amd/csrc/hip/c21hip.h b/21cmfast_amd/csrc/hip/c21hip.h
--- a/21cmfast_amd/csrc/hip/c21hip.h
+++ b/21cmfast_amd/csrc/hip/c21hip.h
@@ -199,6 +199,20 @@
                                      int mass_dep_zeta, double f_limit, void *stream);
 int c21hip_resolve_crossings(const unsigned *bits, int r_hi, int r_lo, unsigned char *first_cross,
                              size_t nlines, void *stream);
+int c21hip_nyq_hoist_supported(int nx, int ny, int nz);
+size_t c21hip_nyq_stack_floats(int nx, int ny, int n_R);
+int c21hip_nyq_hoist(const float *src_a, int filter_a, float R_param_a, const float *src_b, int filter_b,
+                     float R_param_b, int nx, int ny, int nz, double box_len, double box_len_z, const float *R,
+                     int n_R, float *stack, int phases, void *stream);
+int c21hip_split_filter_xy2_main(const float *src_a, float *work_a, int filter_a, float R_param_a,
+                                 const float *src_b, float *work_b, int filter_b, float R_param_b, int nx, int ny,
+                                 int nz, double box_len, double box_len_z, float R, int table_slot,
+                                 int tables_ready, void *stream);
+int c21hip_split_z_ionise_stars_nyq(const float *delta_work, const float *stars_work, const float *delta_nyq,
+                                    const float *stars_nyq, unsigned char *first_cross, unsigned *cross_plane,
+                                    double *partials, double *sum_out, int nx, int ny, int nz, int r_index,
+                                    double rhocrit_omb, double ion_eff, int mass_dep_zeta, double f_limit,
+                                    void *stream);
 int c21hip_split_filter_xy_shared(const float *src, float *work, int filter_type, int nx, int ny,
                                   int nz, double box_len, double box_len_z, float R, int apply,
                                   int table_slot, void *stream);
diff --git a/21cmfast_amd/csrc/hip/fft_native.hip b/21cmfast_amd/csrc/hip/fft_native.hip
--- a/21cmfast_amd/csrc/hip/fft_native.hip
+++ b/21cmfast_amd/csrc/hip/fft_native.hip
@@ -477,6 +477,14 @@
     int filter_axis;
 };
 
+struct NyqPair {
+    int tab[2][2];
+    int src[3];
+    int n_tabs;
+    float R[2];
+    int slice[2];
+};
+
 struct LinePassArgs {
     LineGeo g0, g1;
     int n_geo;
@@ -500,6 +508,10 @@
     float wev_mfp[2][4];
     double wev_dkx, wev_dky, wev_dkz;
     int item_order;
+    const NyqPair *nyq_pairs;
+    float2 *nyq_stack;
+    long nyq_plane;
+    int ktime;
 };
 
 static inline int geo_items(const LineGeo &g) {
@@ -514,7 +526,7 @@
 template <int N, int FMODE = 0>
 struct LineThreads {
     static constexpr int value =
-        ((FMODE == 5 || FMODE == 7 || FMODE == 9) && N == 512) ? C21X_XPAIR_THREADS
+        ((FMODE == 5 || FMODE == 7 || FMODE == 9 || FMODE == 10) && N == 512) ? C21X_XPAIR_THREADS
                                                  : ((N >= 128 && N != 192) ? 512 : 256);
 };
 
@@ -542,10 +554,11 @@
     constexpr int TZ = line_tile_cols(N);
     constexpr int CPAIR = TZ / 2;
     constexpr int RSTEP = kBlock / CPAIR;
-    constexpr bool WEVAL = (FMODE >= 6 && FMODE <= 9);
+    constexpr bool WEVAL = (FMODE >= 6 && FMODE <= 10);
+    constexpr bool BATCH = (FMODE == 10);
     constexpr bool WDIRECT = (FMODE == 8 || FMODE == 9);
     constexpr bool WIN = (FMODE == 3 || (FMODE == 5 && !C21X_XPAIR_NOWIN) || WEVAL);
-    constexpr bool PAIR = (FMODE == 5 || FMODE == 7 || FMODE == 9);
+    constexpr bool PAIR = (FMODE == 5 || FMODE == 7 || FMODE == 9 || FMODE == 10);
     constexpr int NR = PAIR ? 2 : 1;
     using LineItem = LineItemT<PAIR>;
     extern __shared__ float4 lds_raw[];
@@ -556,7 +569,7 @@
     for (int t = threadIdx.x; t < N; t += kBlock) tw[t] = tw_global[t];
     if (N >= 1024)
         for (int t = threadIdx.x; t < N / 2; t += kBlock) tw_half[t] = tw_global[2 * t];
-    if constexpr (WEVAL) {
+    if constexpr (WEVAL && !BATCH) {
         const int per = 3 * a.wev_n_nodes;
         for (int t = threadIdx.x; t < per; t += kBlock) {
             wnodes[t] = a.wev_src[0][t];
@@ -650,6 +663,13 @@
                     it.ct = v - it.og * m;
                 }
             }
+        }
+        if constexpr (BATCH) {
+            const int s0 = a.nyq_pairs[it.og].slice[0], s1 = a.nyq_pairs[it.og].slice[1];
+            it.dst0 = a.nyq_stack + (long)s0 * 2 * a.nyq_plane;
+            it.dst1 = it.dst0 + a.nyq_plane;
+            it.dst0b = s1 >= 0 ? a.nyq_stack + (long)s1 * 2 * a.nyq_plane : nullptr;
+            it.dst1b = s1 >= 0 ? it.dst0b + a.nyq_plane : nullptr;
         }
         it.npair = (po && it.og != 0 && 2 * it.og != it.n_outer) ? 2 : 1;
         return it;
@@ -749,7 +769,25 @@
         }
         wev_kx_half = (float)((double)(N / 2) * a.wev_dkx);
     }
+    int bt_pair = -1, bt_tab[2][2] = {{0, 0}, {0, 0}};
+    float bt_R[2] = {0.f, 0.f};
+    auto batch_stage = [&](int p) {
+        __syncthreads();
+        const NyqPair q = a.nyq_pairs[p];
+        const int per = 3 * a.wev_n_nodes;
+        for (int t = threadIdx.x; t < per; t += kBlock) {
+            wnodes[t] = a.wev_src[0][(size_t)q.src[0] * per + t];
+            if (q.n_tabs > 1) wnodes[per + t] = a.wev_src[0][(size_t)q.src[1] * per + t];
+            if (q.n_tabs > 2) wnodes[2 * per + t] = a.wev_src[0][(size_t)q.src[2] * per + t];
+        }
+        bt_pair = p;
+        bt_tab[0][0] = q.tab[0][0], bt_tab[0][1] = q.tab[0][1], bt_tab[1][0] = q.tab[1][0], bt_tab[1][1] = q.tab[1][1];
+        bt_R[0] = q.R[0], bt_R[1] = q.R[1];
+        __syncthreads();
+    };
     auto eval_windows = [&](const LineItem &it, int m) {
+        if constexpr (BATCH)
+            if (it.og != bt_pair) batch_stage(it.og);
         const int wsel = (a.dual && member_grid(it, m)) ? 1 : 0;
         const int type = wsel ? a.wev_type[1] : a.wev_type[0];
         const int per = 3 * a.wev_n_nodes;
@@ -767,6 +805,10 @@
         }
         const float *tab0 = wnodes + max(wsel ? a.wev_tab[0][1] : a.wev_tab[0][0], 0) * per;
         const float *tab1 = wnodes + max(wsel ? a.wev_tab[1][1] : a.wev_tab[1][0], 0) * per;
+        if constexpr (BATCH) {
+            tab0 = wnodes + max(wsel ? bt_tab[0][1] : bt_tab[0][0], 0) * per;
+            tab1 = wnodes + max(wsel ? bt_tab[1][1] : bt_tab[1][0], 0) * per;
+        }
 #pragma unroll
         for (int u = 0; u < NW; u++) {
             if (FUSED && u >= NP && !(u == NP && r0 == 0)) continue;
@@ -774,7 +816,7 @@
             const KAbs k1 = k_abs(wev_kx[WEVAL ? u : 0], kyc[1], kzc[1]);
 #pragma unroll
             for (int rr = 0; rr < NR; rr++) {
-                const float R = rr ? a.wev_R[1] : a.wev_R[0];
+                const float R = BATCH ? (rr ? bt_R[1] : bt_R[0]) : (rr ? a.wev_R[1] : a.wev_R[0]);
                 const float *tab = rr ? tab1 : tab0;
                 (WPRE ? wpre[rr][WPRE ? u : 0] : wcur[rr][u]) =
                     make_float2(weval_one(k0, R, type, tab, rr), weval_one(k1, R, type, tab, rr));
@@ -784,7 +826,7 @@
             const KAbs k0 = k_abs(wev_kx_half, kyc[0], kzc[0]), k1 = k_abs(wev_kx_half, kyc[1], kzc[1]);
 #pragma unroll
             for (int rr = 0; rr < NR; rr++) {
-                const float R = rr ? a.wev_R[1] : a.wev_R[0];
+                const float R = BATCH ? (rr ? bt_R[1] : bt_R[0]) : (rr ? a.wev_R[1] : a.wev_R[0]);
                 const float *tab = rr ? tab1 : tab0;
                 (WPRE ? wpre_half[rr] : wcur_half[rr]) =
                     make_float2(weval_one(k0, R, type, tab, rr), weval_one(k1, R, type, tab, rr));
@@ -1176,6 +1218,8 @@
 #pragma unroll
       for (int rr = 0; rr < NR; rr++) {
         float2 *const tile_r = tile + rr * N * TZ;
+        if constexpr (BATCH)
+            if (rr && !it.dst0b) continue;
         float2 *st_lo = member_grid(it, m) ? it.dst1 : it.dst0;
         if constexpr (PAIR)
             if (rr) st_lo = member_grid(it, m) ? it.dst1b : it.dst0b;
@@ -1786,7 +1830,8 @@
 };
 constexpr int ktime_kind(int sign, int fmode) {
     return sign < 0 ? 9 : (fmode == 0 ? 1 : fmode == 3 ? 0 : fmode == 5 ? 6 : (fmode == 6 || fmode == 8) ? 7
-                                                              : (fmode == 7 || fmode == 9) ? 8 : 10);
+                                                              : (fmode == 7 || fmode == 9) ? 8
+                                                              : fmode == 10 ? 15 : 10);
 }
 
 #ifndef C21X_XORDER_DEFAULT
@@ -1799,9 +1844,9 @@
         c21hip_set_error("native FFT: twiddle table allocation failed");
         return C21CM_MEMORY_ALLOC_ERROR;
     }
-    const size_t lds = sizeof(float2) * ((size_t)((FMODE == 5 || FMODE == 7 || FMODE == 9) ? 2 : 1) * N *
+    const size_t lds = sizeof(float2) * ((size_t)((FMODE == 5 || FMODE == 7 || FMODE == 9 || FMODE == 10) ? 2 : 1) * N *
                                              line_tile_cols(N) + N + (N >= 1024 ? N / 2 : 0)) +
-                       ((FMODE >= 6 && FMODE <= 9) ? sizeof(float) * 3 * (size_t)a.wev_n_nodes * a.wev_n_tabs : 0);
+                       ((FMODE >= 6 && FMODE <= 10) ? sizeof(float) * 3 * (size_t)a.wev_n_nodes * a.wev_n_tabs : 0);
     if (lds > 160 * 1024) {
         c21hip_set_error("native FFT: %zu bytes of LDS for a %d-point line pass (mode %d)", lds, N, FMODE);
         return C21CM_VALUE_ERROR;
@@ -1828,7 +1873,7 @@
         }
         ao.item_order = (FMODE == 0) ? yo : xo;
     }
-    KTimeScope kt(ktime_kind(SIGN, FMODE), stream);
+    KTimeScope kt(a.ktime ? a.ktime : ktime_kind(SIGN, FMODE), stream);
     hipLaunchKernelGGL((line_pass_kernel<N, SIGN, FMODE>), dim3((unsigned)nblocks),
                        dim3(LineThreads<N, FMODE>::value), lds, stream, ao, tw);
     LAUNCH_CHECK();
@@ -1847,9 +1892,10 @@
         if constexpr (N <= 512) {
             if (SIGN > 0 && fmode == 7) return launch_line_pass_mode<N, +1, 7>(a, stream);
             if (SIGN > 0 && fmode == 9) return launch_line_pass_mode<N, +1, 9>(a, stream);
-        }
-    }
-    if (fmode >= 6 && fmode <= 9) {
+            if (SIGN > 0 && fmode == 10) return launch_line_pass_mode<N, +1, 10>(a, stream);
+        }
+    }
+    if (fmode >= 6 && fmode <= 10) {
         c21hip_set_error("native FFT: evaluated windows are not built for %d-point lines", N);
         return C21CM_VALUE_ERROR;
     }
@@ -3360,7 +3406,7 @@
         a.dual = w.dual;
     }
     if (!(phases & 6)) return 0;
-    a.n_geo = 2;
+    a.n_geo = (phases & 16) ? 1 : 2;
     a.n_grids = n_grids;
     a.g0 = geo_x_main(ny, H, line_tile_cols(nx), split_xb_log2(nx));
     a.g1 = geo_x_nyq(ny, line_tile_cols(nx));
@@ -3454,7 +3500,7 @@
         }
         a.dual = w.dual;
     }
-    a.n_geo = 2;
+    a.n_geo = (phases & 16) ? 1 : 2;
     a.n_grids = n_grids;
     a.g0 = geo_x_main(ny, H, line_tile_cols(nx), split_xb_log2(nx));
     a.g1 = geo_x_nyq(ny, line_tile_cols(nx));
@@ -3497,6 +3543,119 @@
     return filter_xy_pair(src_a, work_a, work_a2, filter_a, R_param_a, src_b, work_b, work_b2,
                           filter_b, R_param_b, nx, ny, nz, box_len, box_len_z, R, R2, table_slot,
                           table_slot2, phases, stream_);
+}
+
+extern "C" int c21hip_split_filter_xy2_main(const float *src_a, float *work_a, int filter_a, float R_param_a,
+                                            const float *src_b, float *work_b, int filter_b, float R_param_b,
+                                            int nx, int ny, int nz, double box_len, double box_len_z, float R,
+                                            int table_slot, int tables_ready, void *stream_) {
+    const float *src[2] = {src_a, src_b};
+    float *work[2] = {work_a, work_b};
+    const int ft[2] = {filter_a, filter_b};
+    const float rp[2] = {R_param_a, R_param_b};
+    return filter_xy(src, work, 2, nx, ny, nz, box_len, box_len_z, ft, R, rp, 1, stream_,
+                     (tables_ready ? 6 : 7) | 16, table_slot);
+}
+
+extern "C" int c21hip_nyq_hoist_supported(int nx, int ny, int nz) {
+    const char *e = getenv("C21CM_NYQ_HOIST");
+    if (e && e[0] == '0') return 0;
+    const WevSet &w = g_wev;
+    return w.active && w.covers && w.nx == nx && w.ny == ny && w.nz == nz && nx >= 128 && nx <= 512 &&
+           (nx & (nx - 1)) == 0 && c21hip_pair_sweep_supported(nx);
+}
+extern "C" size_t c21hip_nyq_stack_floats(int nx, int ny, int n_R) {
+    return (size_t)n_R * 2 * 2 * (size_t)nx * ny;
+}
+extern "C" int c21hip_nyq_hoist(const float *src_a, int filter_a, float R_param_a, const float *src_b,
+                                int filter_b, float R_param_b, int nx, int ny, int nz, double box_len,
+                                double box_len_z, const float *R, int n_R, float *stack_, int phases,
+                                void *stream_) {
+    if (!c21hip_nyq_hoist_supported(nx, ny, nz) || n_R < 1 || !stack_) {
+        c21hip_set_error("Nyquist planes before the loop: no prepared window set covers this %dx%dx%d launch", nx,
+                         ny, nz);
+        return C21CM_VALUE_ERROR;
+    }
+    hipStream_t stream = (hipStream_t)stream_;
+    const int ft[2] = {filter_a, filter_b};
+    const float rp[2] = {R_param_a, R_param_b};
+    const long plane = (long)nx * ny;
+    const long nlines = plane;
+    const int H = nz / 2;
+    float2 *stack = reinterpret_cast<float2 *>(stack_);
+    int st = 0;
+    if (phases & 1) {
+        const int n_pairs = (n_R + 1) / 2;
+        static std::vector<NyqPair> host;
+        host.assign(n_pairs, NyqPair{});
+        LinePassArgs a{};
+        int max_tabs = 1;
+        for (int p = 0; p < n_pairs; p++) {
+            const bool single = 2 * p + 1 >= n_R;
+            LinePassArgs t{};
+            if (!wev_use(t, 2, ft, rp, R[2 * p], single ? R[2 * p] : R[2 * p + 1], true, nx, ny, nz, box_len,
+                         box_len_z)) {
+                c21hip_set_error("Nyquist planes before the loop: radii %g, %g are not in the prepared window set",
+                                 (double)R[2 * p], (double)(single ? R[2 * p] : R[2 * p + 1]));
+                return C21CM_VALUE_ERROR;
+            }
+            NyqPair &q = host[p];
+            const size_t per = 3 * (size_t)t.wev_n_nodes;
+            for (int m = 0; m < 2; m++) {
+                q.R[m] = t.wev_R[m];
+                for (int win = 0; win < 2; win++) q.tab[m][win] = t.wev_tab[m][win];
+            }
+            for (int i = 0; i < 3; i++) q.src[i] = (int)((size_t)(t.wev_src[i] - g_wev.nodes) / per);
+            q.n_tabs = t.wev_n_tabs;
+            q.slice[0] = 2 * p;
+            q.slice[1] = single ? -1 : 2 * p + 1;
+            if (q.n_tabs > max_tabs) max_tabs = q.n_tabs;
+            if (p == 0) a = t;
+        }
+        NyqPair *dev = (NyqPair *)c21hip_ws(WS_NYQ_PAIRS, sizeof(NyqPair) * (size_t)n_pairs);
+        if (!dev) return C21CM_MEMORY_ALLOC_ERROR;
+        if (hipMemcpyAsync(dev, host.data(), sizeof(NyqPair) * (size_t)n_pairs, hipMemcpyHostToDevice, stream) !=
+            hipSuccess)
+            return C21CM_IO_ERROR;
+        if (hipStreamSynchronize(stream) != hipSuccess) return C21CM_IO_ERROR;
+        a.fp.type = -1;
+        a.n_y = ny;
+        a.n_z = nz;
+        a.out_scale = 1.0f;
+        a.wev_src[0] = a.wev_src[1] = a.wev_src[2] = g_wev.nodes;
+        a.wev_n_tabs = max_tabs;
+        a.n_geo = 1;
+        a.n_grids = 2;
+        a.g0 = geo_x_nyq(ny, line_tile_cols(nx));
+        a.g0.n_outer = n_pairs;
+        geo_ptrs(a.g0, 0, reinterpret_cast<const float2 *>(src_a) + nlines * H, nullptr);
+        geo_ptrs(a.g0, 1, reinterpret_cast<const float2 *>(src_b) + nlines * H, nullptr);
+        a.nyq_pairs = dev;
+        a.nyq_stack = stack;
+        a.nyq_plane = plane;
+        if ((st = dispatch_line_pass<+1>(nx, a, 10, stream))) return st;
+    }
+    if (phases & 2) {
+        LinePassArgs a{};
+        a.fp.type = -1;
+        a.n_y = ny;
+        a.n_z = nz;
+        a.out_scale = 1.0f;
+        a.n_geo = 2;
+        a.n_grids = 2;
+        a.g0 = geo_y_main(nx, ny, H, line_tile_cols(ny), split_xb_log2(nx));
+        a.g0.n_outer = 0;
+        a.g0.n_ctiles = 0;
+        a.g1 = geo_y_nyq(nx, ny, line_tile_cols(ny));
+        a.g1.n_outer = n_R;
+        a.g1.outer_bstride = 2 * plane;
+        a.g1_strided = 1;
+        geo_ptrs(a.g1, 0, stack, stack);
+        geo_ptrs(a.g1, 1, stack + plane, stack + plane);
+        a.ktime = 16;
+        if ((st = dispatch_line_pass<+1>(ny, a, 0, stream))) return st;
+    }
+    return 0;
 }
 
 extern "C" int c21hip_split_filter_xy_shared_pair(const float *src, float *work, float *work2,
@@ -4054,15 +4213,16 @@
 static int z_ionise_stars(const float *delta_work, const float *stars_work, const float *xe_work,
                           unsigned char *first_cross, unsigned *cross_bits, double *partials,
                           double *sum_out, int nx, int ny, int nz, int r_index, double rhocrit_omb,
-                          double ion_eff, int mass_dep_zeta, double f_limit, void *stream) {
+                          double ion_eff, int mass_dep_zeta, double f_limit, void *stream,
+                          const float *delta_nyq = nullptr, const float *stars_nyq = nullptr) {
     const long nlines = (long)nx * ny;
     ZFusedArgs a{};
     a.ny = ny;
     a.lb = split_xb_log2(nx);
     a.d_main = reinterpret_cast<const float2 *>(delta_work);
-    a.d_nyq = a.d_main + nlines * (nz / 2);
+    a.d_nyq = delta_nyq ? reinterpret_cast<const float2 *>(delta_nyq) : a.d_main + nlines * (nz / 2);
     a.s_main = reinterpret_cast<const float2 *>(stars_work);
-    a.s_nyq = a.s_main + nlines * (nz / 2);
+    a.s_nyq = stars_nyq ? reinterpret_cast<const float2 *>(stars_nyq) : a.s_main + nlines * (nz / 2);
     if (xe_work) {
         a.x_main = reinterpret_cast<const float2 *>(xe_work);
         a.x_nyq = a.x_main + nlines * (nz / 2);
@@ -4121,6 +4281,21 @@
     }
     return z_ionise_stars(delta_work, stars_work, nullptr, nullptr, cross_plane, partials, sum_out, nx,
                           ny, nz, r_index, rhocrit_omb, ion_eff, mass_dep_zeta, f_limit, stream);
+}
+
+extern "C" int c21hip_split_z_ionise_stars_nyq(const float *delta_work, const float *stars_work,
+                                               const float *delta_nyq, const float *stars_nyq,
+                                               unsigned char *first_cross, unsigned *cross_plane,
+                                               double *partials, double *sum_out, int nx, int ny, int nz,
+                                               int r_index, double rhocrit_omb, double ion_eff,
+                                               int mass_dep_zeta, double f_limit, void *stream) {
+    if (!delta_nyq || !stars_nyq || (cross_plane && !c21hip_z_cross_bits_supported(nx, ny, nz))) {
+        c21hip_set_error("fused pass Z: Nyquist planes or crossing bits are not available for this grid");
+        return C21CM_VALUE_ERROR;
+    }
+    return z_ionise_stars(delta_work, stars_work, nullptr, cross_plane ? nullptr : first_cross, cross_plane,
+                          partials, sum_out, nx, ny, nz, r_index, rhocrit_omb, ion_eff, mass_dep_zeta, f_limit,
+                          stream, delta_nyq, stars_nyq);
 }
 
 extern "C" int c21hip_split_z_ionise_recomb_xe(const float *delta_work, const float *stars_work,
diff --git a/21cmfast_amd/csrc/hip/ws_slots.h b/21cmfast_amd/csrc/hip/ws_slots.h
--- a/21cmfast_amd/csrc/hip/ws_slots.h
+++ b/21cmfast_amd/csrc/hip/ws_slots.h
@@ -278,6 +278,9 @@
     WS_PH_OUT,
     WS_PH_GRIDS,
 
+    WS_NYQ_STACK,
+    WS_NYQ_PAIRS,
+
     WS_COUNT
 };
 
diff --git a/21cmfast_amd/csrc/host/ionize_driver.c b/21cmfast_amd/csrc/host/ionize_driver.c
--- a/21cmfast_amd/csrc/host/ionize_driver.c
+++ b/21cmfast_amd/csrc/host/ionize_driver.c
@@ -233,6 +233,8 @@
     float *x4_unf, *x4_work, *x4_work2;
     const float *cur_x4;
     unsigned *cross_bits;
+    int nyq_ok, nyq_first, nyq_step;
+    float *nyq_stack;
     float *sfr_work2;
     double rec0;
     int finalised;
@@ -666,6 +668,10 @@
     int status = 0;
     const c21cm_ionize_spec *s = c->s;
     unsigned *plane = c->cross_bits ? c->cross_bits + (size_t)(R_ct - 1) * (c->ntot / 32) : NULL;
+    const float *nyq_d = c->nyq_stack ? c->nyq_stack + (size_t)((c->nyq_first - R_ct) / c->nyq_step) *
+                                                           c21hip_nyq_stack_floats(c->nx, c->ny, 1)
+                                      : NULL;
+    const float *nyq_s = nyq_d ? nyq_d + 2 * (size_t)c->nx * c->ny : NULL;
     if (c->fused_rc) {
         double *part = c->def_partials ? c->def_partials + (long)R_ct * c->def_stride : c->partials;
         if (c->def_partials) {
@@ -711,7 +717,12 @@
             TRY(flush_deferred(c));
         if (c->def_count == 0) c->def_first = R_ct;
         c->def_count++;
-        if (plane)
+        if (nyq_d)
+            TRY(c21hip_split_z_ionise_stars_nyq(dwork, swork, nyq_d, nyq_s, first_cross, plane,
+                                                c->def_partials + (long)R_ct * c->def_stride, NULL, c->nx,
+                                                c->ny, c->nz, R_ct, s->rhocrit_omb, s->ion_eff_factor,
+                                                s->mass_dep_zeta, s->f_limit_acg, c->stream));
+        else if (plane)
             TRY(c21hip_split_z_ionise_stars_bits(dwork, swork, plane,
                                                  c->def_partials + (long)R_ct * c->def_stride, NULL,
                                                  c->nx, c->ny, c->nz, R_ct, s->rhocrit_omb,
@@ -727,7 +738,11 @@
     }
     {
         double *sum_dev = c->scalars + SC_SUMS + R_ct;
-        if (plane)
+        if (nyq_d)
+            TRY(c21hip_split_z_ionise_stars_nyq(dwork, swork, nyq_d, nyq_s, first_cross, plane, c->partials,
+                                                sum_dev, c->nx, c->ny, c->nz, R_ct, s->rhocrit_omb,
+                                                s->ion_eff_factor, s->mass_dep_zeta, s->f_limit_acg, c->stream));
+        else if (plane)
             TRY(c21hip_split_z_ionise_stars_bits(dwork, swork, plane, c->partials, sum_dev, c->nx, c->ny,
                                                  c->nz, R_ct, s->rhocrit_omb, s->ion_eff_factor,
                                                  s->mass_dep_zeta, s->f_limit_acg, c->stream));
@@ -778,7 +793,7 @@
                 c->delta_unf, c->delta_work, c->delta_work2, s->hii_filter, 0.f, c->stars_unf,
                 c->stars_work, c->stars_work2, s->stars_filter, (float)s->mfp_meandens, c->nx,
                 c->ny, c->nz, s->box_len, s->box_len_z, (float)s->R[R_a], (float)s->R[R_b], buf_a,
-                buf_b, bits, c->stream));
+                buf_b, bits | (c->nyq_stack ? 16 : 0) , c->stream));
             static int merge34 = -1;
             if (merge34 < 0) {
                 const char *e = getenv("C21CM_RECOMB_MERGE34");
@@ -828,6 +843,12 @@
         TRY(z_ionise_radius(c, R_b, c->delta_work2, c->stars_work2, xw[1], first_cross));
         goto done;
     } else {
+        if (c->nyq_stack)
+            TRY(c21hip_split_filter_xy2_main(c->delta_unf, c->delta_work, s->hii_filter, 0.f, c->stars_unf,
+                                             c->stars_work, s->stars_filter, (float)s->mfp_meandens, c->nx,
+                                             c->ny, c->nz, s->box_len, s->box_len_z, (float)s->R[R_a], buf_a,
+                                             tab_async, c->stream));
+        else
         TRY(c21hip_split_filter_xy2(c->delta_unf, c->delta_work, s->hii_filter, 0.f, c->stars_unf,
                                     c->stars_work, s->stars_filter, (float)s->mfp_meandens, c->nx,
                                     c->ny, c->nz, s->box_len, s->box_len_z, (float)s->R[R_a], 1,
@@ -860,6 +881,7 @@
     if (lowest < 1) lowest = 1;
     if (first < lowest) return 0;
     c->wev = 0;
+    c->nyq_stack = NULL;
     {
         float radii[C21CM_MAX_RADII];
         int n = 0;
@@ -868,6 +890,19 @@
             TRY(c21hip_wev_prepare(c->s->hii_filter, 0.f, c->s->stars_filter, (float)c->s->mfp_meandens,
                                    2, radii, n, c->nx, c->ny, c->nz, c->s->box_len, c->s->box_len_z,
                                    c->pair_radii, &c->wev, c->stream));
+        if (c->nyq_ok && c->wev && c->pair_radii && n > 0 && (first - lowest) / step + 1 == n && !c->fused_rc &&
+            !c->s->use_ts_fluct && !c->x3_on && !c->x4_on && !c->sphere &&
+            c21hip_nyq_hoist_supported(c->nx, c->ny, c->nz)) {
+            float *stack = (float *)c21hip_ws(WS_NYQ_STACK, c21hip_nyq_stack_floats(c->nx, c->ny, n) * sizeof(float));
+            if (stack) {
+                TRY(c21hip_nyq_hoist(c->delta_unf, c->s->hii_filter, 0.f, c->stars_unf, c->s->stars_filter,
+                                     (float)c->s->mfp_meandens, c->nx, c->ny, c->nz, c->s->box_len,
+                                     c->s->box_len_z, radii, n, stack, 3, c->stream));
+                c->nyq_stack = stack;
+                c->nyq_first = first;
+                c->nyq_step = step;
+            }
+        }
     }
     if (c->fused_rc) {
         if (!c->wev) {
@@ -901,6 +936,7 @@
 done:
     c21hip_wev_release();
     c->wev = 0;
+    c->nyq_stack = NULL;
     return status;
 }
 
@@ -1966,6 +2002,7 @@
             goto done;
         }
         cross_bits_begin(&c);
+        c.nyq_ok = 1;
         if (!c.cross_bits)
             TRY(c21hip_memset(mask, 0, c.ntot, stream));
     }
```

Result: faster. 3.497 billion cells/s (median of 6 runs) (+1.3%).
